# KogarashiNetwork/Kogarashi

Hardware: AMD Instinct MI355X
Metric: bn254_g1_msm_pairs_per_sec (higher is better)
Workload: dtype u32x9 (29-bit limbs)

## Files before the change

### kogarashi_amd/csrc/common.h

```cpp
#pragma once
#include <hip/hip_runtime.h>
#include <cstdint>
#include <atomic>
#include <future>
#include <cstdio>
#include <string>
#include <memory>
#include <map>
#include <unordered_map>
#include <vector>
#include <thread>
#include <new>
#include "../../include/kogarashi_amd.h"
#include "curve.h"
#include "tuning.h"
#include "worker_pool.h"

struct kg_tw_cache;

struct kg_ctx {
  int device = 0;
  hipStream_t own_stream = nullptr;
  hipStream_t stream = nullptr;
  std::string last_error;
  kg_tuning tune;
  int msm_window = 0;
  bool sort_alone = false;
  int msm_groups = 0;
  void* ws_sort[2] = {nullptr, nullptr};
  size_t ws_sort_bytes[2] = {0, 0};
  unsigned sort_seq = 0;
  bool queues_placed = false, sort_events = false;
  int placement = 0;
  hipStream_t sort_stream = nullptr;
  static constexpr int MAX_GROUPS = 4;
  hipEvent_t ev_sorted[2][MAX_GROUPS] = {};
  hipStream_t acc_stream[MAX_GROUPS] = {};
  void* ws_pb = nullptr;
  size_t ws_pb_bytes = 0;
  hipEvent_t ev_pb = nullptr;
  hipEvent_t ev_prep = nullptr;
  static constexpr int IDLE_EVS = 8;
  hipEvent_t ev_ws_idle[2][IDLE_EVS] = {};
  int ws_idle_n[2] = {0, 0};
  hipEvent_t ev_bases = nullptr;
  hipEvent_t ev_order = nullptr;
  unsigned small_glv_off = 0;
  bool inputs_complete = false;

  std::multimap<size_t, void*> pool_free;
  size_t pool_cached = 0;
  void* ws_vec = nullptr;
  size_t ws_vec_bytes = 0;
  void* ws2 = nullptr;
  size_t ws2_bytes = 0;
  void* ws3[2] = {nullptr, nullptr};
  size_t ws3_bytes[2] = {0, 0};
  static constexpr int RUN_SETS = 8;
  void* ws_run[RUN_SETS] = {};
  size_t ws_run_bytes[RUN_SETS] = {};
  hipStream_t side_stream = nullptr;
  hipStream_t side2_stream = nullptr;
  hipEvent_t ev_fork = nullptr, ev_join[3] = {nullptr, nullptr, nullptr};
  hipEvent_t ev_acc[RUN_SETS] = {};
  hipEvent_t ev_info[MAX_GROUPS] = {};
  struct Slot { void* host = nullptr; void* host_dev = nullptr; size_t bytes = 0; hipEvent_t done = nullptr; int W = 0, c = 0, w0 = 0; bool busy = false;
                bool combined = false; };
  static constexpr int NSLOTS = 24;
  Slot slots[NSLOTS];
  void* ws_small[NSLOTS] = {};
  size_t ws_small_bytes[NSLOTS] = {};
  std::unique_ptr<kg::WorkerPool> workers;
  std::shared_ptr<void> prover_jobs;
  size_t ticket_n[4] = {0, 0, 0, 0};
  std::future<int> ticket_fut[4];
  uint64_t ticket_out[4][24] = {};
  struct Registered { const uint64_t* base; const uint8_t* inf; size_t n; int curve; uint32_t* packed; uint32_t* table = nullptr; int table_c = 0, table_W = 0; bool fmt64 = false, table64 = false; };
  std::vector<Registered> registered;
  void* up_buf[3] = {nullptr, nullptr, nullptr};
  size_t up_bytes[3] = {0, 0, 0};
  hipStream_t up_stream = nullptr;
  static constexpr int UP_SLICES = 8;
  hipEvent_t ev_up_s[UP_SLICES] = {}, ev_up_b[UP_SLICES] = {};
  void* ws_points = nullptr;
  void* fb_tmp = nullptr;
  size_t fb_tmp_bytes = 0;
  uint32_t* fb_table[3] = {nullptr, nullptr, nullptr};
  void* h_pinned = nullptr;
  void* h_pinned_dev = nullptr;
  size_t h_pinned_bytes = 0;
  std::vector<kg_tw_cache*> tw;
  bool tw_fresh = false;
  bool prof = false;
  struct Phase { const char* name; hipEvent_t e0, e1; };
  std::vector<Phase> phases;
  std::vector<hipEvent_t> event_pool;
  size_t event_next = 0;
  std::atomic<long long> host_finish_us{0};
  std::atomic<int> host_finish_calls{0};
};

namespace kg {

inline WorkerPool& pool(kg_ctx* c) {
  if (!c->workers) c->workers.reset(new WorkerPool(c->tune.pool_max_threads));
  return *c->workers;
}
inline int set_err(kg_ctx* c, int code, const char* what, hipError_t e = hipSuccess) {
  if (c) {
    c->last_error = what;
    if (e != hipSuccess) { c->last_error += ": "; c->last_error += hipGetErrorString(e); }
  }
  if (e != hipSuccess) (void)hipGetLastError();
  return code;
}
template <class Fn>
inline int kg_guarded(kg_ctx* c, Fn&& fn) noexcept {
  try { return fn(); }
  catch (const std::bad_alloc&) { return set_err(c, KG_ERR_OOM, "host allocation failed"); }
  catch (...) { return set_err(c, KG_ERR_HIP, "host runtime failure (a worker thread could not be started?)"); }
}
struct JoinGuard {
  std::thread& t;
  ~JoinGuard() { if (t.joinable()) t.join(); }
};
#define KG_HIP(ctx, call)                                                        \
  do {                                                                           \
    hipError_t e__ = (call);                                                     \
    if (e__ != hipSuccess) return kg::set_err(ctx, e__ == hipErrorOutOfMemory ? KG_ERR_OOM : KG_ERR_HIP, #call, e__); \
  } while (0)
#define KG_TRY(call)            \
  do {                          \
    int s__ = (call);           \
    if (s__ != KG_OK) return s__; \
  } while (0)

hipError_t dev_alloc(kg_ctx* c, void** p, size_t bytes);
void pool_trim(kg_ctx* c);
int ensure_ws_sort(kg_ctx* c, int set, size_t bytes);
int make_sort_stream(kg_ctx* c);
hipError_t create_stream(kg_ctx* c, hipStream_t* out, bool service);
int ensure_ws2(kg_ctx* c, size_t bytes);
int ensure_ws_vec(kg_ctx* c, size_t bytes);
int ensure_ws3(kg_ctx* c, int which, size_t bytes);
int ensure_ws_run(kg_ctx* c, int which, size_t bytes);
int ensure_slot(kg_ctx* c, int slot, size_t bytes);
int ensure_pinned(kg_ctx* c, size_t bytes);
int make_side_stream(kg_ctx* c);
int slice_table_window(const kg_ctx* ctx, int curve, const uint64_t* d_bases, const uint8_t* d_inf, size_t cnt);
void sync_all(kg_ctx* c);

struct PhaseScope {
  kg_ctx* c; int idx = -1; hipStream_t s;
  PhaseScope(kg_ctx* ctx, const char* name, hipStream_t stream = nullptr);
  void end();
};
void prof_reset(kg_ctx* c);

#if defined(__HIP_DEVICE_COMPILE__)
#ifndef KG_PRIO_LEVEL
#define KG_PRIO_LEVEL 3
#endif
#define KG_SERVICE_PRIO() __builtin_amdgcn_s_setprio(KG_PRIO_LEVEL)
#ifndef KG_REDUCE_LEVEL
#define KG_REDUCE_LEVEL 1
#endif
#define KG_REDUCE_PRIO() __builtin_amdgcn_s_setprio(KG_REDUCE_LEVEL)
#else
#define KG_SERVICE_PRIO() ((void)0)
#define KG_REDUCE_PRIO() ((void)0)
#endif

struct alignas(16) Words8 { uint32_t w[8]; };

__device__ __forceinline__ void load_words(const uint64_t* base, size_t elem, uint32_t w[8]) {
  const uint4* p = reinterpret_cast<const uint4*>(base) + 2 * elem;
  uint4 a = p[0], b = p[1];
  w[0] = a.x; w[1] = a.y; w[2] = a.z; w[3] = a.w; w[4] = b.x; w[5] = b.y; w[6] = b.z; w[7] = b.w;
}
__device__ __forceinline__ void store_words(uint64_t* base, size_t elem, const uint32_t w[8]) {
  uint4* p = reinterpret_cast<uint4*>(base) + 2 * elem;
  p[0] = make_uint4(w[0], w[1], w[2], w[3]);
  p[1] = make_uint4(w[4], w[5], w[6], w[7]);
}

template <class F> struct RawIO;
template <class P> struct RawIO<Fp<P>> {
  static constexpr int NW = 9;
  static __device__ __forceinline__ Fp<P> load(const uint32_t* base, size_t stride, size_t i) {
    Fp<P> r;
#pragma unroll
    for (int k = 0; k < 9; ++k) r.l[k] = base[(size_t)k * stride + i];
    return r;
  }
  static __device__ __forceinline__ void store(uint32_t* base, size_t stride, size_t i, const Fp<P>& a) {
#pragma unroll
    for (int k = 0; k < 9; ++k) base[(size_t)k * stride + i] = a.l[k];
  }
};
template <class F> struct RawIO<Fp2<F>> {
  static constexpr int NW = 18;
  static __device__ __forceinline__ Fp2<F> load(const uint32_t* base, size_t stride, size_t i) {
    return {RawIO<F>::load(base, stride, i), RawIO<F>::load(base + 9 * stride, stride, i)};
  }
  static __device__ __forceinline__ void store(uint32_t* base, size_t stride, size_t i, const Fp2<F>& a) {
    RawIO<F>::store(base, stride, i, a.c0);
    RawIO<F>::store(base + 9 * stride, stride, i, a.c1);
  }
};
template <class F>
struct PointIO {
  static constexpr int NW = 4 * RawIO<F>::NW;
  static __device__ __forceinline__ XYZZ<F> load(const uint32_t* base, size_t stride, size_t i) {
    constexpr int E = RawIO<F>::NW;
    return {RawIO<F>::load(base, stride, i), RawIO<F>::load(base + (size_t)E * stride, stride, i),
            RawIO<F>::load(base + (size_t)2 * E * stride, stride, i), RawIO<F>::load(base + (size_t)3 * E * stride, stride, i)};
  }
  static __device__ __forceinline__ void store(uint32_t* base, size_t stride, size_t i, const XYZZ<F>& p) {
    constexpr int E = RawIO<F>::NW;
    RawIO<F>::store(base, stride, i, p.x);
    RawIO<F>::store(base + (size_t)E * stride, stride, i, p.y);
    RawIO<F>::store(base + (size_t)2 * E * stride, stride, i, p.zz);
    RawIO<F>::store(base + (size_t)3 * E * stride, stride, i, p.zzz);
  }
};

template <class F> struct RefIO;
template <class P> struct RefIO<Fp<P>> {
  static constexpr int W64 = 4;
  static __device__ __forceinline__ Fp<P> load(const uint64_t* p) {
    uint32_t w[8];
    load_words(p, 0, w);
    return from_ref<P>(w);
  }
};
template <class F> struct RefIO<Fp2<F>> {
  static constexpr int W64 = 8;
  static __device__ __forceinline__ Fp2<F> load(const uint64_t* p) { return {RefIO<F>::load(p), RefIO<F>::load(p + 4)}; }
};


struct MsmSorted {
  size_t n = 0;
  int c = 0, W = 0, B = 0;
  uint32_t T = 0, T2 = 16, T_top = 0, nhot = 0;
  int top_w = -1;
  uint32_t* hot_list = nullptr;
  size_t npts = 0, part_cap = 0;
  uint32_t ntasks = 0, max_cnt = 0;
  uint32_t *sorted = nullptr, *bsize = nullptr, *bstart = nullptr, *lcnt = nullptr, *lrel = nullptr, *lbase = nullptr;
  uint32_t *task_bkt = nullptr, *task_id = nullptr;
  int set = 0;
  hipEvent_t ready = nullptr;
  int w0 = 0, group = 0;
  hipStream_t acc_stream = nullptr;
  bool reduce_inline = false;
  bool tail_alone = false;
  hipStream_t sorted_on = nullptr;
  int merged_shift = 0, windows = 0;
};
int r1cs_prod_enqueue(kg_ctx* c, hipStream_t st, int field, const uint64_t* row_ptr, const uint64_t* col, const uint64_t* val, size_t m,
                      const uint64_t* z, uint64_t* out, uint32_t* scratch);
int ntt_prepare(kg_ctx* ctx, uint32_t log_n, int inverse);
int ntt_enqueue(kg_ctx* ctx, hipStream_t st, uint64_t* tmp, uint64_t* d_data, uint32_t log_n, int inverse, int coset);
struct NttTables;
int ntt_tables(kg_ctx* ctx, uint32_t log_n, int inverse, NttTables* out, const uint32_t** zinv);
int msm_sort(kg_ctx* ctx, int scalar_field, const uint64_t* d_scalars, size_t n, MsmSorted* S, bool ordered = false, int merged_c = 0, int lane_mult = 1,
             bool wait_info = true, int info_idx = 0);
int msm_sort_wait(kg_ctx* ctx, MsmSorted* S);
struct MsmSortPlan {
  size_t n = 0, chunk_len = 0, nv = 0;
  int c = 0, W = 0, B = 0, Wb = 0, G = 0, nch = 0, maxseg = 0, mshift = 0, set = 0, ngroups = 1, info_base = 0, fb = 7;
  bool alone = false;
  bool merged = false, two_pass = false;
  uint32_t T = 0, T_top = 0;
  int gw0[kg_ctx::MAX_GROUPS] = {}, gW[kg_ctx::MAX_GROUPS] = {};
  char* ws = nullptr;
  size_t o_kt = 0, o_cnt = 0, o_bsize = 0, o_bstart = 0, o_tmp = 0, o_gsize = 0, o_gstart = 0, o_segbase = 0, o_segcnt = 0, o_segoff = 0, o_sorted = 0,
         o_lcnt = 0, o_lrel = 0, o_rowtot = 0, o_bpart = 0, o_woff = 0, o_gsize_m = 0, o_gstart_m = 0, o_segbase_m = 0;
  size_t o_lbase[kg_ctx::MAX_GROUPS] = {}, o_misc[kg_ctx::MAX_GROUPS] = {}, o_lenh[kg_ctx::MAX_GROUPS] = {}, o_tbkt[kg_ctx::MAX_GROUPS] = {},
         o_tid[kg_ctx::MAX_GROUPS] = {}, o_hot[kg_ctx::MAX_GROUPS] = {}, part_cap[kg_ctx::MAX_GROUPS] = {};
};
int msm_sort_begin(kg_ctx* ctx, int scalar_field, const uint64_t* d_scalars, size_t n, MsmSortPlan* P, bool ordered, int merged_c, int lane_mult,
                   int ngroups = 1, const int* gw = nullptr, bool on_main = false);
int msm_sort_group(kg_ctx* ctx, const MsmSortPlan& P, int g, MsmSorted* S, bool on_main = false);
int msm_group_plan(const kg_ctx* ctx, size_t n, int* gw);
int merged_window(const kg_ctx* ctx, size_t n);
bool has_window_table(const kg_ctx* ctx, int curve, const uint64_t* d_bases, const uint8_t* d_inf, size_t nbases, size_t msm_len);
int scalar_queue(kg_ctx* ctx, hipStream_t* out);
struct MsmRunJob { const uint64_t* d_bases; const uint8_t* d_inf; size_t nbases; uint32_t idx_off; int slot; bool bases_complete = false;
                   const uint32_t* packed = nullptr; bool packed64 = false; };
int msm_run_multi(kg_ctx* ctx, const MsmSorted& S, int curve, const MsmRunJob* jobs, int njobs);
int msm_run(kg_ctx* ctx, const MsmSorted& S, int curve, const uint64_t* d_bases, const uint8_t* d_inf, size_t nbases, uint32_t idx_off, int slot);
int msm_finish(kg_ctx* ctx, int curve, int slot, uint64_t* out_xyz);
bool msm_small_plan(const kg_ctx* ctx, int curve, size_t n, int* c, int* r);
bool msm_small_glv(const kg_ctx* ctx, int curve, size_t n);
bool msm_small_kt(const kg_ctx* ctx, size_t n);
int msm_small_enqueue(kg_ctx* ctx, hipStream_t st, int curve, const uint64_t* d_bases, const uint8_t* d_inf, const uint64_t* d_scalars, size_t n, int slot,
                      int c, int r);
int msm_finish_groups(kg_ctx* ctx, int curve, const int* slots, int nslots, uint64_t* out_xyz);
void msm_identity(int curve, uint64_t* out_xyz);

}
```

### kogarashi_amd/csrc/msm_bases.h

```cpp
#pragma once
#include "msm_common.h"

namespace kg {
namespace msm {
namespace {

template <class F> struct FieldOf;
template <class Q> struct FieldOf<Fp<Q>> { using P = Q; };
template <class G> struct FieldOf<Fp2<G>> { using P = typename G::Params; };
template <class F> struct BaseIO;
template <class P> struct BaseIO<Fp<P>> {
  static constexpr int W = 8;
  static constexpr int PE = 9;
  static __device__ __forceinline__ void convert(const uint64_t* src, uint32_t* dst) {
    uint32_t w[8];
    load_words(src, 0, w);
    const Fp<P> v = from_ref<P>(w);
#pragma unroll
    for (int j = 0; j < 9; ++j) dst[j] = v.l[j];
  }
  static __device__ __forceinline__ Fp<P> from_words(const uint32_t* w) {
    Fp<P> r;
#pragma unroll
    for (int j = 0; j < 9; ++j) r.l[j] = w[j];
    return r;
  }
  static constexpr int PK = 8;
  static __device__ __forceinline__ void pack(const Fp<P>& v, uint32_t* dst) { words_from_limbs(v, dst); }
  static __device__ __forceinline__ bool load_point64(const uint32_t* src, Fp<P>& x, Fp<P>& y) {
    uint32_t w[16];
    const uint4* p = reinterpret_cast<const uint4*>(src);
#pragma unroll
    for (int j = 0; j < 4; ++j) { const uint4 v = p[j]; w[4 * j] = v.x; w[4 * j + 1] = v.y; w[4 * j + 2] = v.z; w[4 * j + 3] = v.w; }
    const bool inf = (w[7] & INF_BIT) != 0;
    w[7] &= ~INF_BIT;
    x = limbs_from_words<P>(w); y = limbs_from_words<P>(w + 8);
    return inf;
  }
  static __device__ __forceinline__ bool point64_from_words(uint32_t (&w)[16], Fp<P>& x, Fp<P>& y) {
    const bool inf = (w[7] & INF_BIT) != 0;
    w[7] &= ~INF_BIT;
    x = limbs_from_words<P>(w); y = limbs_from_words<P>(w + 8);
    return inf;
  }
  static __device__ __forceinline__ bool load_point(const uint32_t* src, Fp<P>& x, Fp<P>& y) {
    uint32_t w[18];
    const uint2* p = reinterpret_cast<const uint2*>(src);
#pragma unroll
    for (int j = 0; j < 9; ++j) { const uint2 v = p[j]; w[2 * j] = v.x; w[2 * j + 1] = v.y; }
    const bool inf = (w[8] & INF_BIT) != 0;
    w[8] &= ~INF_BIT;
    x = from_words(w); y = from_words(w + 9);
    return inf;
  }
};
template <class F> struct BaseIO<Fp2<F>> {
  static constexpr int W = 16;
  static constexpr int PE = 18;
  static __device__ __forceinline__ void convert(const uint64_t* src, uint32_t* dst) {
    BaseIO<F>::convert(src, dst);
    BaseIO<F>::convert(src + 4, dst + 9);
  }
  static constexpr int PK = 16;
  static __device__ __forceinline__ void pack(const Fp2<F>& v, uint32_t* dst) { BaseIO<F>::pack(v.c0, dst); BaseIO<F>::pack(v.c1, dst + 8); }
  static __device__ __forceinline__ bool load_point64(const uint32_t* src, Fp2<F>& x, Fp2<F>& y) {
    uint32_t w[32];
    const uint4* p = reinterpret_cast<const uint4*>(src);
#pragma unroll
    for (int j = 0; j < 8; ++j) { const uint4 v = p[j]; w[4 * j] = v.x; w[4 * j + 1] = v.y; w[4 * j + 2] = v.z; w[4 * j + 3] = v.w; }
    const bool inf = (w[7] & INF_BIT) != 0;
    w[7] &= ~INF_BIT;
    using P = typename F::Params;
    x = {limbs_from_words<P>(w), limbs_from_words<P>(w + 8)};
    y = {limbs_from_words<P>(w + 16), limbs_from_words<P>(w + 24)};
    return inf;
  }
  static __device__ __forceinline__ bool load_point(const uint32_t* src, Fp2<F>& x, Fp2<F>& y) {
    uint32_t w[36];
    const uint4* p = reinterpret_cast<const uint4*>(src);
#pragma unroll
    for (int j = 0; j < 9; ++j) { const uint4 v = p[j]; w[4 * j] = v.x; w[4 * j + 1] = v.y; w[4 * j + 2] = v.z; w[4 * j + 3] = v.w; }
    const bool inf = (w[8] & INF_BIT) != 0;
    w[8] &= ~INF_BIT;
    x = {BaseIO<F>::from_words(w), BaseIO<F>::from_words(w + 9)};
    y = {BaseIO<F>::from_words(w + 18), BaseIO<F>::from_words(w + 27)};
    return inf;
  }
};


}
}
template <class F> struct RawIO<Fp2S<F>> {
  static constexpr int NW = 18;
  static __device__ __forceinline__ Fp2S<F> load(const uint32_t* base, size_t stride, size_t i) {
    return {RawIO<F>::load(base + (size_t)(9 * Fp2S<F>::half()) * stride, stride, i)};
  }
  static __device__ __forceinline__ void store(uint32_t* base, size_t stride, size_t i, const Fp2S<F>& a) {
    RawIO<F>::store(base + (size_t)(9 * Fp2S<F>::half()) * stride, stride, i, a.v);
  }
};
namespace msm {
namespace {

template <class G> struct BaseIO<Fp2S<G>> {
  static constexpr int W = 16, PE = 18, PK = 16;
  using P = typename G::Params;
  static __device__ __forceinline__ bool load_point64(const uint32_t* src, Fp2S<G>& x, Fp2S<G>& y) {
    const int h = Fp2S<G>::half();
    const uint4* p = reinterpret_cast<const uint4*>(src);
    uint32_t w[16];
    const uint4 a0 = p[2 * h], a1 = p[2 * h + 1], b0 = p[4 + 2 * h], b1 = p[5 + 2 * h];
    w[0] = a0.x; w[1] = a0.y; w[2] = a0.z; w[3] = a0.w; w[4] = a1.x; w[5] = a1.y; w[6] = a1.z; w[7] = a1.w;
    w[8] = b0.x; w[9] = b0.y; w[10] = b0.z; w[11] = b0.w; w[12] = b1.x; w[13] = b1.y; w[14] = b1.z; w[15] = b1.w;
    int flag = (h == 0 && (w[7] & INF_BIT) != 0) ? 1 : 0;
    flag |= __shfl_xor(flag, 1);
    if (h == 0) w[7] &= ~INF_BIT;
    x.v = limbs_from_words<P>(w); y.v = limbs_from_words<P>(w + 8);
    return flag != 0;
  }
  static __device__ __forceinline__ bool load_point(const uint32_t* src, Fp2S<G>& x, Fp2S<G>& y) {
    const int h = Fp2S<G>::half();
    uint32_t wx[9], wy[9];
#pragma unroll
    for (int k = 0; k < 9; ++k) { wx[k] = src[9 * h + k]; wy[k] = src[18 + 9 * h + k]; }
    int flag = (h == 0 && (wx[8] & INF_BIT) != 0) ? 1 : 0;
    flag |= __shfl_xor(flag, 1);
    if (h == 0) wx[8] &= ~INF_BIT;
    x.v = BaseIO<G>::from_words(wx); y.v = BaseIO<G>::from_words(wy);
    return flag != 0;
  }
};

template <class F>
__device__ __forceinline__ void store_resident(uint32_t* out, size_t i, uint32_t* buf , int fmt64) {
  constexpr int PE = BaseIO<F>::PE, PK = BaseIO<F>::PK;
  if (fmt64) {
    const bool inf = (buf[8] & INF_BIT) != 0;
    buf[8] &= ~INF_BIT;
    uint32_t pk[2 * PK];
#pragma unroll
    for (int e = 0; e < PE / 9; ++e) {
      Fp<typename FieldOf<F>::P> vx, vy;
#pragma unroll
      for (int k = 0; k < 9; ++k) { vx.l[k] = buf[9 * e + k]; vy.l[k] = buf[PE + 9 * e + k]; }
      words_from_limbs(vx, pk + 8 * e);
      words_from_limbs(vy, pk + PK + 8 * e);
    }
    if (inf) pk[7] |= INF_BIT;
    uint4* dst = reinterpret_cast<uint4*>(out + i * 2 * PK);
#pragma unroll
    for (int j = 0; j < PK / 2; ++j) dst[j] = make_uint4(pk[4 * j], pk[4 * j + 1], pk[4 * j + 2], pk[4 * j + 3]);
    return;
  }
  uint2* dst = reinterpret_cast<uint2*>(out + i * 2 * PE);
#pragma unroll
  for (int j = 0; j < PE; ++j) dst[j] = make_uint2(buf[2 * j], buf[2 * j + 1]);
}
template <class F, bool P64>
__global__ void __launch_bounds__(256) k_prep_bases(const uint64_t* __restrict__ bases, const uint8_t* __restrict__ inf, size_t n,
                                                    uint32_t* __restrict__ out) {
  KG_SERVICE_PRIO();
  size_t i = (size_t)blockIdx.x * blockDim.x + threadIdx.x;
  if (i >= n) return;
  constexpr int W = BaseIO<F>::W, PE = BaseIO<F>::PE;
  uint32_t buf[2 * PE];
  BaseIO<F>::convert(bases + (size_t)i * W, buf);
  BaseIO<F>::convert(bases + (size_t)i * W + W / 2, buf + PE);
  if (inf && inf[i]) buf[8] |= INF_BIT;
  store_resident<F>(out, i, buf, P64 ? 1 : 0);
}

template <class F>
static void launch_prep_bases(hipStream_t st, const uint64_t* bases, const uint8_t* inf, size_t n, uint32_t* out, bool fmt64) {
  const dim3 grid((unsigned)((n + 255) / 256));
  if (fmt64) hipLaunchKernelGGL((k_prep_bases<F, true>), grid, dim3(256), 0, st, bases, inf, n, out);
  else hipLaunchKernelGGL((k_prep_bases<F, false>), grid, dim3(256), 0, st, bases, inf, n, out);
}

template <class P> __device__ __forceinline__ void put_limbs(const Fp<P>& a, uint32_t* w) {
#pragma unroll
  for (int j = 0; j < 9; ++j) w[j] = a.l[j];
}
template <class F> __device__ __forceinline__ void put_limbs(const Fp2<F>& a, uint32_t* w) { put_limbs(a.c0, w); put_limbs(a.c1, w + 9); }
template <class F>
__global__ void __launch_bounds__(64) k_table_next(const uint32_t* __restrict__ prev, size_t n, int c, uint32_t* __restrict__ next, int fmt64) {
  const size_t i = (size_t)blockIdx.x * blockDim.x + threadIdx.x;
  if (i >= n) return;
  constexpr int PE = BaseIO<F>::PE, PK = BaseIO<F>::PK;
  Affine<F> a;
  bool inf = fmt64 ? BaseIO<F>::load_point64(prev + i * 2 * PK, a.x, a.y) : BaseIO<F>::load_point(prev + i * 2 * PE, a.x, a.y);
  uint32_t buf[2 * PE];
#pragma unroll
  for (int j = 0; j < 2 * PE; ++j) buf[j] = 0;
  if (!inf) {
    XYZZ<F> p = double_affine(a);
    for (int k = 1; k < c; ++k) p = double_xyzz(p);
    Affine<F> o;
    inf = !to_affine(p, o);
    if (!inf) { put_limbs(reduce(o.x), buf); put_limbs(reduce(o.y), buf + PE); }
  }
  if (inf) buf[8] |= INF_BIT;
  store_resident<F>(next, i, buf, fmt64);
}


}
}
}
```

### kogarashi_amd/csrc/msm_digits.h

```cpp
#pragma once
#include <cstdint>
#include "fp29.h"
#include "glv_consts.h"

namespace kg {

KG_HD void small_bias(int c, int W, uint32_t H[8]) {
  for (int j = 0; j < 8; ++j) H[j] = 0;
  for (int w = 0; w < W - 1; ++w) {
    const int bit = w * c + c - 1;
    H[bit >> 5] |= 1u << (bit & 31);
  }
}

KG_HD uint32_t small_window_digit(const uint32_t kb[8], int w, int c, int W, bool& negative) {
  const int o = w * c;
  const int j = o >> 5, sh = o & 31;
  uint64_t v = kb[j];
  if (j + 1 < 8) v |= (uint64_t)kb[j + 1] << 32;
  const uint32_t e = (uint32_t)(v >> sh);
  if (w == W - 1) {
    negative = false;
    return e;
  }
  const int32_t d = (int32_t)(e & ((1u << c) - 1u)) - (int32_t)(1u << (c - 1));
  negative = d < 0;
  return (uint32_t)(d < 0 ? -d : d);
}

template <int NA, int NB, int LO, int NR>
KG_HD void glv_mul_words(const uint32_t* a, const uint32_t* b, uint32_t* r) {
  uint64_t carry = 0;
  uint64_t carry_hi = 0;
#pragma unroll
  for (int col = 0; col < LO + NR; ++col) {
    uint64_t lo = carry, hi = carry_hi;
#pragma unroll
    for (int i = 0; i < NA; ++i) {
      const int j = col - i;
      if (j < 0 || j >= NB) continue;
      const uint64_t pr = (uint64_t)a[i] * b[j];
      lo += pr & 0xffffffffu;
      hi += pr >> 32;
    }
    if (col >= LO) r[col - LO] = (uint32_t)lo;
    carry = (lo >> 32) + (hi & 0xffffffffu);
    carry_hi = hi >> 32;
  }
}
template <class L>
KG_HD void glv_decompose_with(const uint32_t k[8], uint32_t k1[4], bool& neg1, uint32_t k2[4], bool& neg2) {
  uint32_t c1[3], c2[5];
  {
    uint32_t t[6];
    glv_mul_words<8, 3, 7, 4>(k, L::G1, t);
    uint64_t cy = ((uint64_t)t[0] + 0x80000000u) >> 32;
#pragma unroll
    for (int i = 0; i < 3; ++i) { const uint64_t v = (uint64_t)t[1 + i] + cy; c1[i] = (uint32_t)v; cy = v >> 32; }
    glv_mul_words<8, 5, 7, 6>(k, L::G2, t);
    cy = ((uint64_t)t[0] + 0x80000000u) >> 32;
#pragma unroll
    for (int i = 0; i < 5; ++i) { const uint64_t v = (uint64_t)t[1 + i] + cy; c2[i] = (uint32_t)v; cy = v >> 32; }
  }
  uint32_t t1[5], t2[5], r1[5], r2[5];
  glv_mul_words<3, 5, 0, 5>(c1, L::A1, t1);
  glv_mul_words<5, 5, 0, 5>(c2, L::A2, t2);
  {
    int64_t br = 0;
#pragma unroll
    for (int i = 0; i < 5; ++i) {
      const int64_t d = (int64_t)k[i] - (int64_t)t1[i] - (int64_t)t2[i] + br;
      r1[i] = (uint32_t)d;
      br = d >> 32;
    }
  }
  glv_mul_words<3, 5, 0, 5>(c1, L::B1, t1);
  glv_mul_words<5, 5, 0, 5>(c2, L::B2, t2);
  {
    int64_t br = 0;
#pragma unroll
    for (int i = 0; i < 5; ++i) {
      const int64_t d = -(int64_t)t1[i] - (int64_t)t2[i] + br;
      r2[i] = (uint32_t)d;
      br = d >> 32;
    }
  }
  neg1 = (r1[4] >> 31) != 0;
  neg2 = (r2[4] >> 31) != 0;
  uint64_t cy1 = neg1 ? 1 : 0, cy2 = neg2 ? 1 : 0;
#pragma unroll
  for (int i = 0; i < 4; ++i) {
    const uint64_t s1 = (uint64_t)(neg1 ? ~r1[i] : r1[i]) + cy1;
    k1[i] = (uint32_t)s1; cy1 = s1 >> 32;
    const uint64_t s2 = (uint64_t)(neg2 ? ~r2[i] : r2[i]) + cy2;
    k2[i] = (uint32_t)s2; cy2 = s2 >> 32;
  }
}

}
```

### kogarashi_amd/csrc/msm_host.cpp

```cpp
#include "common.h"
#include "host_fp.h"
#include "msm_internal.h"
#include <algorithm>
#include <chrono>
#include <cstdlib>
#include <cstring>
#include <condition_variable>
#include <mutex>
#include <thread>

using namespace kg;

namespace {

struct G1Cfg { using HF = HostFq; static constexpr int E64 = 4; static constexpr int ID = KG_G1; };
struct GkCfg { using HF = HostFr; static constexpr int E64 = 4; static constexpr int ID = KG_GRUMPKIN; };
struct G2Cfg { using HF = HostFq2; static constexpr int E64 = 8; static constexpr int ID = KG_G2; };

template <class HF> struct HostIO;
template <class P> struct HostIO<HostFp<P>> {
  static HostFp<P> load(const uint64_t* w) { return HostFp<P>::from_words(w); }
  static void store(const HostFp<P>& a, uint64_t* w) { a.to_words(w); }
};
template <class F> struct HostIO<Fp2<F>> {
  static Fp2<F> load(const uint64_t* w) { return {HostIO<F>::load(w), HostIO<F>::load(w + 4)}; }
  static void store(const Fp2<F>& a, uint64_t* w) { HostIO<F>::store(a.c0, w); HostIO<F>::store(a.c1, w + 4); }
};

template <class Cfg>
XYZZ<typename Cfg::HF> host_load_point(const uint64_t* p) {
  using HF = typename Cfg::HF;
  constexpr int E = Cfg::E64;
  return {HostIO<HF>::load(p), HostIO<HF>::load(p + E), HostIO<HF>::load(p + 2 * E), HostIO<HF>::load(p + 3 * E)};
}

template <class Cfg>
void store_projective(const XYZZ<typename Cfg::HF>& p, uint64_t* out_xyz) {
  using HF = typename Cfg::HF;
  constexpr int E = Cfg::E64;
  Affine<HF> a;
  if (!to_affine(p, a)) {
    HostIO<HF>::store(HF::zero(), out_xyz);
    HostIO<HF>::store(HF::one(), out_xyz + E);
    HostIO<HF>::store(HF::zero(), out_xyz + 2 * E);
    return;
  }
  HostIO<HF>::store(a.x, out_xyz);
  HostIO<HF>::store(a.y, out_xyz + E);
  HostIO<HF>::store(HF::one(), out_xyz + 2 * E);
}

}

namespace kg {

template <class Cfg>
int msm_finish_t(kg_ctx* ctx, const int* slots, int nslots, uint64_t* out_xyz) {
  using HF = typename Cfg::HF;
  hipSetDevice(ctx->device);
  host_trace("finish: enter");
  constexpr int PE = 4 * Cfg::E64;
  XYZZ<HF> acc = XYZZ<HF>::identity();
  long long busy_us = 0;
  for (int s = 0; s < nslots; ++s) {
    kg_ctx::Slot& sl = ctx->slots[slots[s]];
    if (hipEventSynchronize(sl.done) != hipSuccess) return KG_ERR_HIP;
    host_trace("finish: slot ready");
    const auto t0 = std::chrono::steady_clock::now();
    const uint64_t* hp = (const uint64_t*)sl.host;
    const int W = sl.W, c = sl.c, w0 = sl.w0;
    if (sl.combined) {
      for (int w = W - 1; w >= 0; --w) {
        for (int l = 0; l < c; ++l) acc = double_xyzz(acc);
        acc = add_xyzz(acc, host_load_point<Cfg>(hp + (size_t)w * PE));
      }
    } else
    for (int bit = (w0 + W) * c - 1; bit >= w0 * c; --bit) {
      acc = double_xyzz(acc);
      const int w = bit / c - w0, l = bit % c;
      if (c > 1 && l < c - 1) acc = add_xyzz(acc, host_load_point<Cfg>(hp + ((size_t)w * c + 1 + l) * PE));
      if (l == 0) acc = add_xyzz(acc, host_load_point<Cfg>(hp + ((size_t)w * c) * PE));
    }
    if (s == nslots - 1) store_projective<Cfg>(acc, out_xyz);
    busy_us += std::chrono::duration_cast<std::chrono::microseconds>(std::chrono::steady_clock::now() - t0).count();
  }
  host_trace("finish: done");
  if (ctx->prof) {
    ctx->host_finish_us += busy_us;
    ctx->host_finish_calls += 1;
  }
  return KG_OK;
}

int msm_finish_groups(kg_ctx* ctx, int curve, const int* slots, int nslots, uint64_t* out_xyz) {
  if (nslots < 1) return KG_ERR_BAD_ARG;
  switch (curve) {
    case KG_G1: return msm_finish_t<G1Cfg>(ctx, slots, nslots, out_xyz);
    case KG_GRUMPKIN: return msm_finish_t<GkCfg>(ctx, slots, nslots, out_xyz);
    case KG_G2: return msm_finish_t<G2Cfg>(ctx, slots, nslots, out_xyz);
    default: return KG_ERR_BAD_ARG;
  }
}
int msm_finish(kg_ctx* ctx, int curve, int slot, uint64_t* out_xyz) { return msm_finish_groups(ctx, curve, &slot, 1, out_xyz); }
void msm_identity(int curve, uint64_t* out_xyz) {
  if (curve == KG_G2) store_projective<G2Cfg>(XYZZ<HostFq2>::identity(), out_xyz);
  else if (curve == KG_GRUMPKIN) store_projective<GkCfg>(XYZZ<HostFr>::identity(), out_xyz);
  else store_projective<G1Cfg>(XYZZ<HostFq>::identity(), out_xyz);
}

}

namespace {

template <class Cfg>
int sum_affine_impl(const uint64_t* pts, const uint8_t* inf, size_t count, uint64_t* out_xy, uint8_t* out_inf) {
  using HF = typename Cfg::HF;
  constexpr int E = Cfg::E64;
  XYZZ<HF> acc = XYZZ<HF>::identity();
  for (size_t i = 0; i < count; ++i) {
    if (inf && inf[i]) continue;
    Affine<HF> a{HostIO<HF>::load(pts + i * 2 * E), HostIO<HF>::load(pts + i * 2 * E + E)};
    acc = add_mixed(acc, a);
  }
  uint64_t xyz[3 * 8];
  store_projective<Cfg>(acc, xyz);
  std::memcpy(out_xy, xyz, 2 * E * 8);
  *out_inf = is_identity(acc) ? 1 : 0;
  return KG_OK;
}

}

extern "C" {

static int sum_slices(kg_ctx* ctx, int curve, const uint64_t (*part)[24], int K, uint64_t* out_xyz) {
  const int E = curve == KG_G2 ? 8 : 4;
  if (K == 1) { std::memcpy(out_xyz, part[0], (size_t)3 * E * 8); return KG_OK; }
  uint64_t pts[kg_ctx::UP_SLICES * 16];
  uint8_t pinf[kg_ctx::UP_SLICES];
  for (int j = 0; j < K; ++j) {
    bool z0 = true;
    for (int k = 0; k < E; ++k) z0 = z0 && part[j][2 * E + k] == 0;
    pinf[j] = z0 ? 1 : 0;
    std::memcpy(pts + (size_t)j * 2 * E, part[j], (size_t)2 * E * 8);
  }
  uint64_t xy[16];
  uint8_t inf = 0;
  KG_TRY(kg_points_sum_affine(ctx, curve, pts, pinf, (size_t)K, xy, &inf));
  kg::msm_identity(curve, out_xyz);
  if (!inf) {
    for (int k = 0; k < E; ++k) out_xyz[2 * E + k] = out_xyz[E + k];
    std::memcpy(out_xyz, xy, (size_t)2 * E * 8);
  }
  return KG_OK;
}

static int msm_sliced(kg_ctx* ctx, int curve, const uint64_t* d_bases, const uint8_t* d_inf, const uint64_t* d_scalars, size_t n, uint64_t* out_xyz) {
  constexpr int K = 4;
  const size_t pw = curve == KG_G2 ? 16 : 8;
  size_t lo[K + 1];
  for (int j = 0; j <= K; ++j) lo[j] = n / K * j + (j == K ? n % K : 0);
  const int saved_window = ctx->msm_window;
  struct Restore { kg_ctx* c; int w; ~Restore() { c->msm_window = w; } } restore_window{ctx, saved_window};
  if (!saved_window) { const int cw = pick_window(n, 0), cs = pick_window(n / K, 0); ctx->msm_window = cw > cs ? cw : cs; }
  uint64_t part[K][24];
  std::future<int> fin[K];
  kg::WaitAll fin_done{fin, K};
  int rc = KG_OK;
  const int sfield = curve == KG_GRUMPKIN ? KG_FQ : KG_FR;
  for (int j = 0; j < K && rc == KG_OK; ++j) {
    const size_t a = lo[j], cnt = lo[j + 1] - lo[j];
    kg::MsmSorted S;
    rc = kg::msm_sort(ctx, sfield, d_scalars + 4 * a, cnt, &S, j > 0);
    if (rc != KG_OK) break;
    rc = kg::msm_run(ctx, S, curve, d_bases + a * pw, d_inf ? d_inf + a : nullptr, cnt, 0, 16 + j);
    if (rc != KG_OK) break;
    uint64_t* out = part[j];
    fin[j] = kg::pool(ctx).submit([ctx, curve, j, out] { return kg::msm_finish(ctx, curve, 16 + j, out); });
  }
  ctx->msm_window = saved_window;
  for (int j = 0; j < K; ++j)
    if (fin[j].valid()) { const int r2 = fin[j].get(); if (rc == KG_OK) rc = r2; }
  if (rc != KG_OK) { kg_ctx_sync(ctx); return rc; }
  return sum_slices(ctx, curve, part, K, out_xyz);
}

static int msm_grouped(kg_ctx* ctx, int curve, const uint64_t* d_bases, const uint8_t* d_inf, const uint64_t* d_scalars, size_t n, const int* gw, int NG,
                       uint64_t* out_xyz) {
  KG_HIP(ctx, hipSetDevice(ctx->device));
  if (!ctx->side_stream) KG_TRY(make_side_stream(ctx));
  KG_TRY(make_sort_stream(ctx));
  for (int g = 1; g < NG && g < ctx->tune.group_accq; ++g)
    if (!ctx->acc_stream[g]) KG_HIP(ctx, create_stream(ctx, &ctx->acc_stream[g], false));
  kg::MsmSortPlan Q;
  const int main_first = ctx->tune.group_main_first;
  KG_TRY(kg::msm_sort_begin(ctx, curve == KG_GRUMPKIN ? KG_FQ : KG_FR, d_scalars, n, &Q, false, 0, 1, NG, gw, main_first != 0));
  if (main_first == 1) {
    KG_HIP(ctx, hipEventRecord(ctx->ev_prep, ctx->stream));
    KG_HIP(ctx, hipStreamWaitEvent(ctx->sort_stream, ctx->ev_prep, 0));
  }
  const size_t pw64 = curve == KG_G2 ? 16 : 8;
  bool resident = false;
  for (const auto& r : ctx->registered) {
    if (r.curve != curve || d_bases < r.base) continue;
    const size_t off64 = (size_t)(d_bases - r.base);
    if (off64 % pw64 != 0 || off64 / pw64 + n > r.n) continue;
    if (d_inf != (r.inf ? r.inf + off64 / pw64 : nullptr)) continue;
    resident = true;
    break;
  }
  const bool f64 = resident_fmt64(n);
  if (!resident) {
    const size_t bytes = n * (f64 ? (curve == KG_G2 ? 128 : 64) : (curve == KG_G2 ? 144 : 72));
    if (bytes > ctx->ws_pb_bytes) {
      if (ctx->ws_pb) { sync_all(ctx); hipFree(ctx->ws_pb); ctx->ws_pb = nullptr; ctx->ws_pb_bytes = 0; }
      const hipError_t e = dev_alloc(ctx, &ctx->ws_pb, bytes + bytes / 8);
      if (e != hipSuccess) return set_err(ctx, KG_ERR_OOM, "resident-bases allocation", e);
      ctx->ws_pb_bytes = bytes + bytes / 8;
    }
    hipStream_t cq = ctx->side_stream;
    if (!ctx->inputs_complete) {
      KG_HIP(ctx, hipEventRecord(ctx->ev_order, ctx->stream));
      KG_HIP(ctx, hipStreamWaitEvent(cq, ctx->ev_order, 0));
    }
    PhaseScope ph(ctx, "prep_bases", cq);
    prep_bases_enqueue(curve, cq, d_bases, d_inf, n, (uint32_t*)ctx->ws_pb, f64);
    ph.end();
    KG_HIP(ctx, hipGetLastError());
    KG_HIP(ctx, hipEventRecord(ctx->ev_pb, cq));
  }
  kg::MsmSorted S[kg_ctx::MAX_GROUPS];
  int slots[kg_ctx::MAX_GROUPS];
  int rc = kg::msm_sort_group(ctx, Q, 0, &S[0], main_first != 0);
  if (rc == KG_OK && main_first == 2) KG_HIP(ctx, hipStreamWaitEvent(ctx->sort_stream, S[0].ready, 0));
  if (rc == KG_OK && NG > 1) rc = kg::msm_sort_group(ctx, Q, 1, &S[1]);
  int launched = 0;
  for (int g = 0; g < NG && rc == KG_OK; ++g) {
    rc = kg::msm_sort_wait(ctx, &S[g]);
    if (rc != KG_OK) break;
    const int accq = ctx->tune.group_accq;
    S[g].acc_stream = (accq > 1 && g % accq) ? ctx->acc_stream[g % accq] : nullptr;
    const int rinl = ctx->tune.group_reduce_inline;
    S[g].reduce_inline = rinl && g == NG - 1;
    S[g].tail_alone = g == NG - 1;
    const int one_side = ctx->tune.group_one_side;
    slots[g] = one_side ? 16 + 2 * g : 16 + g;
    kg::MsmRunJob job{d_bases, d_inf, n, 0u, slots[g], false, resident ? nullptr : (const uint32_t*)ctx->ws_pb, f64};
    rc = kg::msm_run_multi(ctx, S[g], curve, &job, 1);
    if (rc != KG_OK) break;
    ++launched;
    if (g + 2 < NG) rc = kg::msm_sort_group(ctx, Q, g + 2, &S[g + 2]);
  }
  if (rc != KG_OK) { sync_all(ctx); return rc; }
  (void)launched;
  return kg::msm_finish_groups(ctx, curve, slots, NG, out_xyz);
}

static int msm_blocking(kg_ctx* ctx, int curve, const uint64_t* d_bases, const uint8_t* d_inf, const uint64_t* d_scalars, size_t n, uint64_t* out_xyz);

int kg_msm(kg_ctx* ctx, int curve, const uint64_t* d_bases, const uint8_t* d_inf, const uint64_t* d_scalars, size_t n, uint64_t* out_xyz) {
  return kg::kg_guarded(ctx, [&]() -> int {
  if (!ctx || !out_xyz || (n && (!d_bases || !d_scalars)) || curve < 0 || curve > KG_G2) return KG_ERR_BAD_ARG;
  if (n == 0) { kg::msm_identity(curve, out_xyz); return KG_OK; }
  return msm_blocking(ctx, curve, d_bases, d_inf, d_scalars, n, out_xyz);
  });
}

static int msm_blocking(kg_ctx* ctx, int curve, const uint64_t* d_bases, const uint8_t* d_inf, const uint64_t* d_scalars, size_t n, uint64_t* out_xyz) {
  int sc = 0, sr = 0;
  if (kg::msm_small_plan(ctx, curve, n, &sc, &sr)) {
    KG_TRY(kg::msm_small_enqueue(ctx, ctx->stream, curve, d_bases, d_inf, d_scalars, n, 0, sc, sr));
    return kg::msm_finish(ctx, curve, 0, out_xyz);
  }
  const bool sliced_ok = ctx->tune.msm_sliced != 0;
  if (n >= ((size_t)1 << 23) && sliced_ok && pick_window(n, ctx->msm_window) < 19) return msm_sliced(ctx, curve, d_bases, d_inf, d_scalars, n, out_xyz);
  kg::MsmSorted S;
  const bool tables_ok = n <= ((size_t)1 << ctx->tune.blocking_tables_log);
  const int mc = tables_ok && kg::has_window_table(ctx, curve, d_bases, d_inf, n, n) ? kg::merged_window(ctx, n) : 0;
  if (!mc) {
    int gw[kg_ctx::MAX_GROUPS];
    const int NG = kg::msm_group_plan(ctx, n, gw);
    if (NG > 1) return msm_grouped(ctx, curve, d_bases, d_inf, d_scalars, n, gw, NG, out_xyz);
  }
  ctx->sort_alone = true;
  const int rs = kg::msm_sort(ctx, curve == KG_GRUMPKIN ? KG_FQ : KG_FR, d_scalars, n, &S, false, mc);
  ctx->sort_alone = false;
  KG_TRY(rs);
  S.tail_alone = true;
  S.reduce_inline = ctx->tune.blocking_reduce_inline != 0;
  KG_TRY(kg::msm_run(ctx, S, curve, d_bases, d_inf, n, 0, 0));
  return kg::msm_finish(ctx, curve, 0, out_xyz);
}

int kg_msm_pick_window(size_t n) { return pick_window(n ? n : 1, 0); }
int kg_msm_table_window(size_t msm_len) { return kg::merged_window(nullptr, msm_len); }

int kg_bases_register(kg_ctx* ctx, int curve, const uint64_t* d_bases, const uint8_t* d_inf, size_t n) {
  return kg::kg_guarded(ctx, [&]() -> int {
  if (!ctx || curve < 0 || curve > KG_G2) return KG_ERR_BAD_ARG;
  if (n == 0) return KG_OK;
  if (!d_bases) return KG_ERR_BAD_ARG;
  KG_HIP(ctx, hipSetDevice(ctx->device));
  kg_bases_unregister(ctx, d_bases);
  const bool fmt64 = resident_fmt64(n);
  const size_t pw = fmt64 ? (curve == KG_G2 ? 32 : 16) : (curve == KG_G2 ? 36 : 18);
  uint32_t* packed = nullptr;
  KG_HIP(ctx, dev_alloc(ctx, (void**)&packed, n * pw * 4));
  prep_bases_enqueue(curve, ctx->stream, d_bases, d_inf, n, packed, fmt64);
  if (hipError_t e = hipGetLastError(); e != hipSuccess) {
    hipFree(packed);
    return set_err(ctx, KG_ERR_HIP, "k_prep_bases launch", e);
  }
  kg_ctx::Registered reg{d_bases, d_inf, n, curve, packed};
  reg.fmt64 = fmt64;
  ctx->registered.push_back(reg);
  return KG_OK;
  });
}

int kg_bases_unregister(kg_ctx* ctx, const uint64_t* d_bases) {
  return kg::kg_guarded(ctx, [&]() -> int {
  if (!ctx) return KG_ERR_BAD_ARG;
  for (size_t i = 0; i < ctx->registered.size(); ++i) {
    if (ctx->registered[i].base == d_bases) {
      kg_ctx_sync(ctx);
      hipFree(ctx->registered[i].packed);
      if (ctx->registered[i].table) hipFree(ctx->registered[i].table);
      ctx->registered.erase(ctx->registered.begin() + i);
      return KG_OK;
    }
  }
  return KG_OK;
  });
}

int kg_bases_precompute(kg_ctx* ctx, const uint64_t* d_bases, size_t msm_len) {
  return kg::kg_guarded(ctx, [&]() -> int {
  if (!ctx || !d_bases) return KG_ERR_BAD_ARG;
  KG_HIP(ctx, hipSetDevice(ctx->device));
  kg_ctx::Registered* r = nullptr;
  for (auto& e : ctx->registered) if (e.base == d_bases) r = &e;
  if (!r) return set_err(ctx, KG_ERR_BAD_ARG, "kg_bases_precompute: the array is not registered");
  if (msm_len == 0) msm_len = r->n;
  if (msm_len < r->n) return set_err(ctx, KG_ERR_BAD_ARG, "kg_bases_precompute: msm_len is shorter than the array");
  const int c = kg::merged_window(ctx, msm_len);
  if (!c) return set_err(ctx, KG_ERR_BAD_ARG, "kg_bases_precompute: window tables are offered for MSMs of 2^16 .. 2^20 scalars");
  if (r->table && r->table_c == c) return KG_OK;
  if (r->table) { kg_ctx_sync(ctx); hipFree(r->table); r->table = nullptr; r->table_c = r->table_W = 0; }
  const int W = (255 + c - 1) / c;
  const bool t64 = table_fmt64();
  const size_t pw = t64 ? (r->curve == KG_G2 ? 32 : 16) : (r->curve == KG_G2 ? 36 : 18), row = r->n * pw;
  uint32_t* table = nullptr;
  if (hipError_t e = dev_alloc(ctx, (void**)&table, (size_t)W * row * 4); e != hipSuccess) {
    (void)hipGetLastError();
    return set_err(ctx, KG_ERR_OOM, "window table allocation", e);
  }
  hipStream_t st = ctx->stream;
  prep_bases_enqueue(r->curve, st, r->base, r->inf, r->n, table, t64);
  hipError_t e = hipGetLastError();
  for (int w = 1; w < W && e == hipSuccess; ++w) {
    table_next_enqueue(r->curve, st, table + (size_t)(w - 1) * row, r->n, c, table + (size_t)w * row, t64);
    e = hipGetLastError();
  }
  if (e != hipSuccess) { hipFree(table); return set_err(ctx, KG_ERR_HIP, "window table build", e); }
  r->table = table; r->table_c = c; r->table_W = W; r->table64 = t64;
  return KG_OK;
  });
}

int kg_msm_begin(kg_ctx* ctx, int curve, const uint64_t* d_bases, const uint8_t* d_inf, const uint64_t* d_scalars, size_t n, int ticket) {
  return kg::kg_guarded(ctx, [&]() -> int {
  if (!ctx || (n && (!d_bases || !d_scalars)) || curve < 0 || curve > KG_G2 || ticket < 0 || ticket > 3) return KG_ERR_BAD_ARG;
  ctx->ticket_n[ticket] = n;
  if (n == 0) return KG_OK;
  int sc = 0, sr = 0;
  struct GlvGuard { kg_ctx* c; unsigned old; ~GlvGuard() { c->small_glv_off = old; } } glv_guard{ctx, ctx->small_glv_off};
  ctx->small_glv_off |= (1u << KG_G1) | (1u << KG_GRUMPKIN);
  if (n <= (size_t)(curve == KG_G2 ? ctx->tune.small_max_flight / 2 : ctx->tune.small_max_flight) && kg::msm_small_plan(ctx, curve, n, &sc, &sr)) {
    if (ctx->ticket_fut[ticket].valid()) ctx->ticket_fut[ticket].wait();
    KG_TRY(kg::msm_small_enqueue(ctx, ctx->stream, curve, d_bases, d_inf, d_scalars, n, 1 + ticket, sc, sr));
    uint64_t* out = ctx->ticket_out[ticket];
    ctx->ticket_fut[ticket] = kg::pool(ctx).submit([ctx, curve, ticket, out] { return kg::msm_finish(ctx, curve, 1 + ticket, out); });
    return KG_OK;
  }
  kg::MsmSorted S;
  const int mc = kg::has_window_table(ctx, curve, d_bases, d_inf, n, n) ? kg::merged_window(ctx, n) : 0;
  KG_TRY(kg::msm_sort(ctx, curve == KG_GRUMPKIN ? KG_FQ : KG_FR, d_scalars, n, &S, false, mc));
  const int pipe_accq = ctx->tune.pipe_accq;
  if (pipe_accq > 1 && (ticket & 1) && ctx->acc_stream[1]) S.acc_stream = ctx->acc_stream[1];
  if (ctx->ticket_fut[ticket].valid()) ctx->ticket_fut[ticket].wait();
  KG_TRY(kg::msm_run(ctx, S, curve, d_bases, d_inf, n, 0, 1 + ticket));
  uint64_t* out = ctx->ticket_out[ticket];
  ctx->ticket_fut[ticket] = kg::pool(ctx).submit([ctx, curve, ticket, out] { return kg::msm_finish(ctx, curve, 1 + ticket, out); });
  return KG_OK;
  });
}

int kg_msm_end(kg_ctx* ctx, int curve, int ticket, uint64_t* out_xyz) {
  return kg::kg_guarded(ctx, [&]() -> int {
  if (!ctx || !out_xyz || curve < 0 || curve > KG_G2 || ticket < 0 || ticket > 3) return KG_ERR_BAD_ARG;
  if (ctx->ticket_n[ticket] == 0) { kg::msm_identity(curve, out_xyz); return KG_OK; }
  if (!ctx->ticket_fut[ticket].valid()) return kg::set_err(ctx, KG_ERR_BAD_ARG, "kg_msm_end without a matching kg_msm_begin");
  const int rc = ctx->ticket_fut[ticket].get();
  if (rc != KG_OK) return rc;
  std::memcpy(out_xyz, ctx->ticket_out[ticket], (curve == KG_G2 ? 24 : 12) * 8);
  return KG_OK;
  });
}

static int grow_device(kg_ctx* ctx, int which, size_t bytes) {
  if (bytes <= ctx->up_bytes[which]) return KG_OK;
  if (ctx->up_buf[which]) { sync_all(ctx); hipFree(ctx->up_buf[which]); ctx->up_buf[which] = nullptr; ctx->up_bytes[which] = 0; }
  const hipError_t e = dev_alloc(ctx, &ctx->up_buf[which], bytes + bytes / 8);
  if (e != hipSuccess) { (void)hipGetLastError(); return set_err(ctx, KG_ERR_OOM, "upload buffer allocation", e); }
  ctx->up_bytes[which] = bytes + bytes / 8;
  return KG_OK;
}

static int msm_host_plan(const kg_tuning& tune, size_t n, bool scalars_only, size_t* lo) {
  int K = n >= ((size_t)1 << 20) ? 4 : (n >= ((size_t)1 << 18) ? 2 : 1);
  int first_div = 1;
  if (scalars_only) {
    int lg = 0;
    while (((size_t)1 << (lg + 1)) <= n) ++lg;
    K = lg >= 24 ? 8 : (lg == 23 ? 6 : (lg == 22 ? 4 : (lg == 21 ? 3 : (lg >= 19 ? 2 : 1))));
    first_div = K > 1 ? 2 : 1;
  }
  if (tune.host_slices >= 1 && tune.host_slices <= kg_ctx::UP_SLICES) K = tune.host_slices;
  if (tune.host_first_div >= 1 && tune.host_first_div <= 16) first_div = tune.host_first_div;
  if ((size_t)K > n) K = (int)n;
  if (K <= 1) { lo[0] = 0; lo[1] = n; return 1; }
  const size_t units = 1 + (size_t)(K - 1) * first_div;
  size_t first = n / units;
  if (first < 1) first = 1;
  first &= ~(size_t)255;
  if (first == 0) first = n / units ? n / units : 1;
  lo[0] = 0; lo[1] = first;
  const size_t rest = n - first;
  for (int j = 2; j <= K; ++j) lo[j] = first + rest / (K - 1) * (j - 1) + (j == K ? rest % (K - 1) : 0);
  return K;
}

static int msm_host_impl(kg_ctx* ctx, int curve, const uint64_t* bases, const uint8_t* inf, bool bases_on_device, const uint64_t* h_scalars, size_t n,
                         uint64_t* out_xyz) {
  KG_HIP(ctx, hipSetDevice(ctx->device));
  host_trace("host: enter");
  const size_t pb = curve == KG_G2 ? 128 : 64;
  if (!bases_on_device) {
    KG_TRY(grow_device(ctx, 0, n * pb));
    if (inf) KG_TRY(grow_device(ctx, 2, n));
  }
  KG_TRY(grow_device(ctx, 1, n * 32));
  if (!ctx->ev_up_s[0]) {
    KG_TRY(make_sort_stream(ctx));
    if (!ctx->up_stream) KG_HIP(ctx, hipStreamCreateWithFlags(&ctx->up_stream, hipStreamNonBlocking));
    for (int i = 0; i < kg_ctx::UP_SLICES; ++i) {
      KG_HIP(ctx, hipEventCreateWithFlags(&ctx->ev_up_s[i], hipEventDisableTiming));
      KG_HIP(ctx, hipEventCreateWithFlags(&ctx->ev_up_b[i], hipEventDisableTiming));
    }
  }
  hipStream_t sq;
  KG_TRY(kg::scalar_queue(ctx, &sq));
  if (bases_on_device && !ctx->inputs_complete) {
    KG_HIP(ctx, hipEventRecord(ctx->ev_order, ctx->stream));
    KG_HIP(ctx, hipStreamWaitEvent(sq, ctx->ev_order, 0));
  }
  const char* d_b = bases_on_device ? (const char*)bases : (const char*)ctx->up_buf[0];
  uint64_t* d_s = (uint64_t*)ctx->up_buf[1];
  const uint8_t* d_i = bases_on_device ? inf : (inf ? (const uint8_t*)ctx->up_buf[2] : nullptr);
  int sc = 0, sr = 0;
  if (kg::msm_small_plan(ctx, curve, n, &sc, &sr)) {
    KG_HIP(ctx, hipMemcpyAsync(d_s, h_scalars, n * 32, hipMemcpyHostToDevice, ctx->stream));
    if (!bases_on_device) {
      KG_HIP(ctx, hipMemcpyAsync(ctx->up_buf[0], bases, n * pb, hipMemcpyHostToDevice, ctx->stream));
      if (inf) KG_HIP(ctx, hipMemcpyAsync(ctx->up_buf[2], inf, n, hipMemcpyHostToDevice, ctx->stream));
    }
    KG_TRY(kg::msm_small_enqueue(ctx, ctx->stream, curve, (const uint64_t*)d_b, d_i, d_s, n, 0, sc, sr));
    return kg::msm_finish(ctx, curve, 0, out_xyz);
  }
  size_t lo[kg_ctx::UP_SLICES + 1];
  const int K = msm_host_plan(ctx->tune, n, bases_on_device, lo);
  std::atomic<int> up_s{0}, up_b{0}, up_rc{(int)hipSuccess};
  std::mutex up_mu;
  std::condition_variable up_cv;
  auto upload_scalars = [&](int j) {
    const size_t a = lo[j], cnt = lo[j + 1] - lo[j];
    hipError_t e = hipMemcpyAsync(d_s + 4 * a, h_scalars + 4 * a, cnt * 32, hipMemcpyHostToDevice, ctx->up_stream);
    if (e == hipSuccess) e = hipEventRecord(ctx->ev_up_s[j], ctx->up_stream);
    if (e != hipSuccess) up_rc = (int)e;
    { std::lock_guard<std::mutex> lk(up_mu); up_s = j + 1; }
    up_cv.notify_all();
    host_trace("upload: scalars");
  };
  auto upload_bases = [&](int j) {
    if (!bases_on_device) {
      const size_t a = lo[j], cnt = lo[j + 1] - lo[j];
      hipError_t e = hipMemcpyAsync((char*)ctx->up_buf[0] + a * pb, (const char*)bases + a * pb, cnt * pb, hipMemcpyHostToDevice, ctx->up_stream);
      if (e == hipSuccess && inf) e = hipMemcpyAsync((uint8_t*)ctx->up_buf[2] + a, inf + a, cnt, hipMemcpyHostToDevice, ctx->up_stream);
      if (e == hipSuccess) e = hipEventRecord(ctx->ev_up_b[j], ctx->up_stream);
      if (e != hipSuccess) up_rc = (int)e;
      host_trace("upload: bases");
    }
    { std::lock_guard<std::mutex> lk(up_mu); up_b = j + 1; }
    up_cv.notify_all();
  };
  upload_scalars(0);
  if (K == 1 && bases_on_device) {
    if (up_rc != (int)hipSuccess) return set_err(ctx, KG_ERR_HIP, "host-to-device upload", (hipError_t)up_rc.load());
    KG_HIP(ctx, hipStreamWaitEvent(ctx->stream, ctx->ev_up_s[0], 0));
    KG_HIP(ctx, hipStreamWaitEvent(sq, ctx->ev_up_s[0], 0));
    return msm_blocking(ctx, curve, bases, inf, d_s, n, out_xyz);
  }
  if (K > 1 && !ctx->acc_stream[1]) { if (create_stream(ctx, &ctx->acc_stream[1], false) != hipSuccess) return set_err(ctx, KG_ERR_HIP, "queue creation"); }
  std::future<int> uploader = kg::pool(ctx).submit([&]() -> int {
    hipSetDevice(ctx->device);
    upload_bases(0);
    for (int j = 1; j < K; ++j) { upload_scalars(j); upload_bases(j); }
    return KG_OK;
  });
  struct WaitGuard { std::future<int>& f; ~WaitGuard() { if (f.valid()) f.wait(); } } uploader_done{uploader};
  uint64_t part[kg_ctx::UP_SLICES][24];
  std::future<int> fin[kg_ctx::UP_SLICES];
  kg::WaitAll fin_done{fin, kg_ctx::UP_SLICES};
  int rc = KG_OK;
  const int sfield = curve == KG_GRUMPKIN ? KG_FQ : KG_FR;
  const bool was_alone = ctx->sort_alone;
  for (int j = 0; j < K && rc == KG_OK; ++j) {
    const size_t a = lo[j], cnt = lo[j + 1] - lo[j];
    { std::unique_lock<std::mutex> lk(up_mu); up_cv.wait(lk, [&] { return up_s.load() > j; }); }
    if (up_rc != (int)hipSuccess) { rc = set_err(ctx, KG_ERR_HIP, "host-to-device upload", (hipError_t)up_rc.load()); break; }
    if (hipStreamWaitEvent(sq, ctx->ev_up_s[j], 0) != hipSuccess) { rc = KG_ERR_HIP; break; }
    kg::MsmSorted S;
    ctx->sort_alone = j == 0;
    const int mc = (bases_on_device && ctx->tune.host_slice_tables) ? kg::slice_table_window(ctx, curve, (const uint64_t*)(d_b + a * pb), d_i ? d_i + a : nullptr, cnt) : 0;
    rc = kg::msm_sort(ctx, sfield, d_s + 4 * a, cnt, &S, true, mc);
    ctx->sort_alone = was_alone;
    if (rc != KG_OK) break;
    if (bases_on_device) {
      if (ctx->tune.host_accq > 1 && (j & 1)) S.acc_stream = ctx->acc_stream[1];
      S.reduce_inline = ctx->tune.group_reduce_inline && K > 1 && j == K - 1;
      S.tail_alone = j == K - 1;
    }
    if (!bases_on_device) {
      { std::unique_lock<std::mutex> lk(up_mu); up_cv.wait(lk, [&] { return up_b.load() > j; }); }
      if (up_rc != (int)hipSuccess) { rc = set_err(ctx, KG_ERR_HIP, "host-to-device upload", (hipError_t)up_rc.load()); break; }
      if (hipStreamWaitEvent(sq, ctx->ev_up_b[j], 0) != hipSuccess) { rc = KG_ERR_HIP; break; }
    }
    const kg::MsmRunJob job{(const uint64_t*)(d_b + a * pb), d_i ? d_i + a : nullptr, cnt, 0u, 16 + j, true};
    rc = kg::msm_run_multi(ctx, S, curve, &job, 1);
    if (rc != KG_OK) break;
    uint64_t* out = part[j];
    fin[j] = kg::pool(ctx).submit([ctx, curve, j, out] { return kg::msm_finish(ctx, curve, 16 + j, out); });
  }
  if (uploader.valid()) uploader.wait();
  hipStreamSynchronize(ctx->up_stream);
  host_trace("host: uploads synced");
  for (int j = 0; j < K; ++j)
    if (fin[j].valid()) { const int r2 = fin[j].get(); if (rc == KG_OK) rc = r2; }
  if (rc != KG_OK) { kg_ctx_sync(ctx); return rc; }
  return sum_slices(ctx, curve, part, K, out_xyz);
}

int kg_msm_host_slices(size_t n, int scalars_only, size_t* lo) {
  if (!lo) return KG_ERR_BAD_ARG;
  if (n == 0) { lo[0] = 0; return 0; }
  return msm_host_plan(tuning(), n, scalars_only != 0, lo);
}

int kg_msm_host(kg_ctx* ctx, int curve, const uint64_t* h_bases, const uint8_t* h_inf, const uint64_t* h_scalars, size_t n, uint64_t* out_xyz) {
  return kg::kg_guarded(ctx, [&]() -> int {
  if (!ctx || !out_xyz || (n && (!h_bases || !h_scalars)) || curve < 0 || curve > KG_G2) return KG_ERR_BAD_ARG;
  if (n == 0) return kg_msm(ctx, curve, nullptr, nullptr, nullptr, 0, out_xyz);
  return msm_host_impl(ctx, curve, h_bases, h_inf, false, h_scalars, n, out_xyz);
  });
}

int kg_msm_host_scalars(kg_ctx* ctx, int curve, const uint64_t* d_bases, const uint8_t* d_inf, const uint64_t* h_scalars, size_t n, uint64_t* out_xyz) {
  return kg::kg_guarded(ctx, [&]() -> int {
  if (!ctx || !out_xyz || (n && (!d_bases || !h_scalars)) || curve < 0 || curve > KG_G2) return KG_ERR_BAD_ARG;
  if (n == 0) return kg_msm(ctx, curve, nullptr, nullptr, nullptr, 0, out_xyz);
  return msm_host_impl(ctx, curve, d_bases, d_inf, true, h_scalars, n, out_xyz);
  });
}

static void xyz_to_commit(int curve, const uint64_t* xyz, uint64_t* out_xy, uint8_t* out_inf) {
  const int E = curve == KG_G2 ? 8 : 4;
  std::memcpy(out_xy, xyz, 2 * E * 8);
  bool z0 = true;
  for (int i = 0; i < E; ++i) z0 = z0 && xyz[2 * E + i] == 0;
  *out_inf = z0 ? 1 : 0;
}

int kg_commit_host_scalars(kg_ctx* ctx, int curve, const uint64_t* d_bases, const uint8_t* d_inf, const uint64_t* h_scalars, size_t n,
                           uint64_t* out_xy, uint8_t* out_inf) {
  return kg::kg_guarded(ctx, [&]() -> int {
  if (!ctx || !out_xy || !out_inf || curve < 0 || curve > KG_G2) return KG_ERR_BAD_ARG;
  uint64_t xyz[24];
  KG_TRY(kg_msm_host_scalars(ctx, curve, d_bases, d_inf, h_scalars, n, xyz));
  xyz_to_commit(curve, xyz, out_xy, out_inf);
  return KG_OK;
  });
}

int kg_commit(kg_ctx* ctx, int curve, const uint64_t* d_bases, const uint8_t* d_inf, const uint64_t* d_scalars, size_t n,
              uint64_t* out_xy, uint8_t* out_inf) {
  return kg::kg_guarded(ctx, [&]() -> int {
  if (!ctx || !out_xy || !out_inf || curve < 0 || curve > KG_G2) return KG_ERR_BAD_ARG;
  uint64_t xyz[24];
  KG_TRY(kg_msm(ctx, curve, d_bases, d_inf, d_scalars, n, xyz));
  xyz_to_commit(curve, xyz, out_xy, out_inf);
  return KG_OK;
  });
}

int kg_points_sum_affine(kg_ctx* ctx, int curve, const uint64_t* pts, const uint8_t* inf, size_t count, uint64_t* out_xy, uint8_t* out_inf) {
  (void)ctx;
  if (!out_xy || !out_inf || (count && !pts)) return KG_ERR_BAD_ARG;
  switch (curve) {
    case KG_G1: return sum_affine_impl<G1Cfg>(pts, inf, count, out_xy, out_inf);
    case KG_GRUMPKIN: return sum_affine_impl<GkCfg>(pts, inf, count, out_xy, out_inf);
    case KG_G2: return sum_affine_impl<G2Cfg>(pts, inf, count, out_xy, out_inf);
    default: return KG_ERR_BAD_ARG;
  }
}

}
```

### kogarashi_amd/csrc/msm_internal.h

```cpp
#pragma once
#include "common.h"

namespace kg {

int pick_window(size_t n, int forced);
bool resident_fmt64(size_t n);
bool table_fmt64();
void prep_bases_enqueue(int curve, hipStream_t st, const uint64_t* d_bases, const uint8_t* d_inf, size_t n, uint32_t* out, bool fmt64);
void table_next_enqueue(int curve, hipStream_t st, const uint32_t* prev, size_t n, int c, uint32_t* next, bool fmt64);
void host_trace(const char* what);

}
```

### kogarashi_amd/csrc/msm_run.hip

```cpp
#include "msm_reduce_kernels.h"
#include <cstdlib>
#include <cstring>

using namespace kg;
using namespace kg::msm;

namespace kg {
void prep_bases_enqueue(int curve, hipStream_t st, const uint64_t* d_bases, const uint8_t* d_inf, size_t n, uint32_t* out, bool fmt64) {
  if (curve == KG_G1) launch_prep_bases<Fq>(st, d_bases, d_inf, n, out, fmt64);
  else if (curve == KG_GRUMPKIN) launch_prep_bases<Fr>(st, d_bases, d_inf, n, out, fmt64);
  else launch_prep_bases<Fq2>(st, d_bases, d_inf, n, out, fmt64);
}
void table_next_enqueue(int curve, hipStream_t st, const uint32_t* prev, size_t n, int c, uint32_t* next, bool fmt64) {
  const dim3 grid((unsigned)((n + 63) / 64));
  if (curve == KG_G1) hipLaunchKernelGGL(k_table_next<Fq>, grid, dim3(64), 0, st, prev, n, c, next, fmt64 ? 1 : 0);
  else if (curve == KG_GRUMPKIN) hipLaunchKernelGGL(k_table_next<Fr>, grid, dim3(64), 0, st, prev, n, c, next, fmt64 ? 1 : 0);
  else hipLaunchKernelGGL(k_table_next<Fq2>, grid, dim3(64), 0, st, prev, n, c, next, fmt64 ? 1 : 0);
}
}

namespace kg {

struct RunJob { const uint64_t* d_bases; const uint8_t* d_inf; size_t nbases; uint32_t idx_off; int slot; bool bases_complete; const uint32_t* packed; bool packed64; };

template <class Cfg>
int msm_run_multi_t(kg_ctx* ctx, const MsmSorted& S, const RunJob* jobs, int njobs) {
  using F = typename Cfg::F;
  using KF = typename Cfg::KF;
  constexpr unsigned LPT = Lanes<KF>::N;
  constexpr int PW = 2 * BaseIO<F>::PE;
  constexpr int NW = PointIO<F>::NW;
  if (njobs < 1 || njobs > MAX_FUSED) return set_err(ctx, KG_ERR_BAD_ARG, "bad number of fused base arrays");
  const int W = S.W, B = S.B, c = S.c;
  const size_t npts = S.npts, part_cap = S.part_cap, nexp = (size_t)W * c;
  const size_t exp_bytes = nexp * 4 * Cfg::E64 * 8;
  hipStream_t st = S.acc_stream ? S.acc_stream : ctx->stream, sq;
  KG_TRY(scalar_queue(ctx, &sq));
  bool ordered_bases = false, converted = false, shared_pb = false;
  if (!ctx->side_stream) KG_TRY(make_side_stream(ctx));
  if (st != ctx->stream && !ctx->inputs_complete) {
    KG_HIP(ctx, hipEventRecord(ctx->ev_order, ctx->stream));
    KG_HIP(ctx, hipStreamWaitEvent(st, ctx->ev_order, 0));
  }
  struct Lay { size_t o_pb, o_lc[2], o_lr[2], o_lb[2], o_part[2], o_pbuf[2], o_rowtot, o_misc, o_hot; char* ws; const uint32_t* pb; int set; };
  Lay lay[MAX_FUSED];
  AccSets A;
  A.nsets = njobs;
  for (int k = 0; k < MAX_FUSED; ++k) { A.pb[k] = nullptr; A.idx_off[k] = 0; A.partial[k] = nullptr; A.tab_n[k] = 0; A.fmt64[k] = 0; }
  for (int k = 0; k < njobs; ++k) {
    const RunJob& J = jobs[k];
    Lay& Y = lay[k];
    Carver cv;
    const uint32_t* reg_pb = nullptr;
    if (J.packed) {
      if (S.merged_shift) return set_err(ctx, KG_ERR_BAD_ARG, "merged sort against caller-converted bases");
      reg_pb = J.packed; A.fmt64[k] = J.packed64 ? 1 : 0; shared_pb = true;
    }
    for (const auto& r : ctx->registered) {
      if (reg_pb) break;
      if (r.curve != Cfg::ID || J.d_bases < r.base) continue;
      const size_t off64 = (size_t)(J.d_bases - r.base);
      if (off64 % (size_t)BaseIO<F>::W != 0 || off64 / BaseIO<F>::W + J.nbases > r.n) continue;
      const size_t off = off64 / BaseIO<F>::W;
      if (J.d_inf != (r.inf ? r.inf + off : nullptr)) continue;
      if (S.merged_shift) {
        if (!r.table || r.table_c != c || r.table_W != S.windows) continue;
        reg_pb = r.table + off * (r.table64 ? 2 * BaseIO<F>::PK : PW);
        A.tab_n[k] = (uint32_t)r.n;
        A.fmt64[k] = r.table64 ? 1 : 0;
      } else {
        reg_pb = r.packed + off * (r.fmt64 ? 2 * BaseIO<F>::PK : PW);
        A.fmt64[k] = r.fmt64 ? 1 : 0;
      }
      break;
    }
    if (S.merged_shift && !reg_pb) return set_err(ctx, KG_ERR_BAD_ARG, "merged sort against bases without a matching window table");
    const bool conv64 = !reg_pb && resident_fmt64(J.nbases);
    if (conv64) A.fmt64[k] = 1;
    Y.o_pb = cv.take(reg_pb ? 256 : J.nbases * (conv64 ? 2 * BaseIO<F>::PK : PW) * 4);
    for (int i = 0; i < 2; ++i) {
      Y.o_lc[i] = cv.take(npts * 4); Y.o_lr[i] = cv.take(npts * 4); Y.o_lb[i] = cv.take((size_t)(W + 1) * 4);
      Y.o_part[i] = cv.take(part_cap * NW * 4); Y.o_pbuf[i] = cv.take(npts * NW * 4);
    }
    Y.o_rowtot = cv.take((size_t)W * 4); Y.o_misc = cv.take(64);
    Y.o_hot = cv.take(S.nhot ? (size_t)(S.nhot < HOT_MAX ? S.nhot : HOT_MAX) * hot_split<KF>(S.max_cnt) * NW * 4 : 0);
    Y.set = J.slot % kg_ctx::RUN_SETS;
    for (int k2 = 0; k2 < k; ++k2)
      if (lay[k2].set == Y.set) return set_err(ctx, KG_ERR_BAD_ARG, "fused MSMs need result slots in different run-space sets");
    KG_TRY(ensure_ws_run(ctx, Y.set, cv.off));
    KG_TRY(ensure_slot(ctx, J.slot, exp_bytes));
    if (!ctx->ev_acc[Y.set]) KG_HIP(ctx, hipEventCreateWithFlags(&ctx->ev_acc[Y.set], hipEventDisableTiming));
    Y.ws = (char*)ctx->ws_run[Y.set];
    Y.pb = reg_pb ? reg_pb : (uint32_t*)(Y.ws + Y.o_pb);
    for (int s2 = 0; s2 < kg_ctx::NSLOTS; ++s2)
      if (s2 % kg_ctx::RUN_SETS == Y.set && ctx->slots[s2].done && ctx->slots[s2].busy) {
        KG_HIP(ctx, hipStreamWaitEvent(st, ctx->slots[s2].done, 0));
        if (!reg_pb) KG_HIP(ctx, hipStreamWaitEvent(sq, ctx->slots[s2].done, 0));
        ctx->slots[s2].busy = false;
      }
    if (!reg_pb) {
      if (!ctx->inputs_complete && !ordered_bases && !J.bases_complete) {
        KG_HIP(ctx, hipEventRecord(ctx->ev_order, st));
        KG_HIP(ctx, hipStreamWaitEvent(sq, ctx->ev_order, 0));
        ordered_bases = true;
      }
      PhaseScope ph(ctx, "prep_bases", sq);
      launch_prep_bases<F>(sq, J.d_bases, J.d_inf, J.nbases, (uint32_t*)(Y.ws + Y.o_pb), conv64);
      ph.end();
      converted = true;
    }
    A.pb[k] = Y.pb; A.idx_off[k] = J.idx_off; A.partial[k] = (uint32_t*)(Y.ws + Y.o_part[0]);
  }
  const Level L0{S.lcnt, S.lrel, S.lbase};
  if (converted) {
    KG_HIP(ctx, hipEventRecord(ctx->ev_bases, sq));
    KG_HIP(ctx, hipStreamWaitEvent(st, ctx->ev_bases, 0));
  } else if (S.ready && S.sorted_on != st) KG_HIP(ctx, hipStreamWaitEvent(st, S.ready, 0));
  if (shared_pb) KG_HIP(ctx, hipStreamWaitEvent(st, ctx->ev_pb, 0));
  if (S.ntasks) {
    PhaseScope ph(ctx, "accumulate", st);
#ifdef KG_EXPERIMENTS
    if (LPT > 1 && ctx->tune.g2_pair_acc)
      hipLaunchKernelGGL(k_acc_tasks<KF>, dim3((unsigned)(((size_t)S.ntasks * LPT + 63) / 64) * (unsigned)njobs), dim3(64), 0, st, A, S.sorted, S.bstart, S.bsize, L0,
                         S.task_bkt, S.task_id, S.n, W, B, S.T, part_cap, S.merged_shift, S.T_top, S.top_w);
    else if (acc_prefetch<F>(A, njobs, jobs[0].nbases))
      hipLaunchKernelGGL(k_acc_tasks_q<typename PfField<F>::T>, dim3(((S.ntasks + 63) / 64) * (unsigned)njobs), dim3(64), 0, st, A, S.sorted, S.bstart, S.bsize, L0, S.task_bkt,
                         S.task_id, S.n, W, B, S.T, part_cap, S.merged_shift, S.T_top, S.top_w);
    else
#endif
    hipLaunchKernelGGL(k_acc_tasks<F>, dim3(((S.ntasks + 63) / 64) * (unsigned)njobs), dim3(64), 0, st, A, S.sorted, S.bstart, S.bsize, L0, S.task_bkt, S.task_id,
                       S.n, W, B, S.T, part_cap, S.merged_shift, S.T_top, S.top_w);
    ph.end();
  }
  for (int k = 0; k < njobs; ++k) {
    const RunJob& J = jobs[k];
    const Lay& Y = lay[k];
    const int slot = J.slot, set = Y.set;
    char* ws = Y.ws;
    const size_t* o_lc = Y.o_lc; const size_t* o_lr = Y.o_lr; const size_t* o_lb = Y.o_lb;
    uint32_t* part[2] = {(uint32_t*)(ws + Y.o_part[0]), (uint32_t*)(ws + Y.o_part[1])};
    uint32_t* pbuf[2] = {(uint32_t*)(ws + Y.o_pbuf[0]), (uint32_t*)(ws + Y.o_pbuf[1])};
    uint32_t* rowtot = (uint32_t*)(ws + Y.o_rowtot);
    uint32_t* misc = (uint32_t*)(ws + Y.o_misc);
    kg_ctx::Slot& sl = ctx->slots[slot];
    hipStream_t side = S.reduce_inline ? st : ((slot & 1) ? ctx->side2_stream : ctx->side_stream);
    if (side != st) {
      KG_HIP(ctx, hipEventRecord(ctx->ev_acc[set], st));
      KG_HIP(ctx, hipStreamWaitEvent(side, ctx->ev_acc[set], 0));
    }
    Level L = L0;
    int pcur = 0;
    bool fused_first = false;
    {
      PhaseScope ph(ctx, "partial_sums", side);
      uint32_t max_cnt = S.max_cnt;
      int lv = -1;
      const unsigned g1024 = (unsigned)((npts + 1023) / 1024);
      const bool hot_ok = ctx->tune.hot_sum != 0;
      if (max_cnt > GATHER_SUM_MAX && hot_ok && S.nhot >= 1 && S.nhot <= HOT_MAX && (size_t)part_cap * NW * 4 < ((size_t)1 << 32)) {
        PhaseScope ph2(ctx, "hot_sum", side);
        uint32_t* hot_scratch = (uint32_t*)(ws + Y.o_hot);
        const uint32_t split = hot_split<KF>(S.max_cnt);
        hipLaunchKernelGGL(k_hot_sum<KF>, dim3(S.nhot, split), dim3(256), 36 * 256 * 4, side, part[pcur], L, B, S.hot_list, hot_scratch, split);
        hipLaunchKernelGGL(k_hot_fold<KF>, dim3(S.nhot), dim3(256), 36 * 256 * 4, side, part[pcur], L, B, S.hot_list, hot_scratch, split);
        ph2.end();
        max_cnt = GATHER_SUM_MAX;
      }
      while (max_cnt > GATHER_SUM_MAX) {
        const int nx = lv < 0 ? 0 : (lv ^ 1);
        PhaseScope pr(ctx, "partial_round", side);
        uint32_t* ncnt = (uint32_t*)(ws + o_lc[nx]);
        uint32_t* nrel = (uint32_t*)(ws + o_lr[nx]);
        uint32_t* nbase = (uint32_t*)(ws + o_lb[nx]);
        KG_HIP(ctx, hipMemsetAsync(misc, 0, 64, side));
        hipLaunchKernelGGL(k_task_count, dim3(g1024), dim3(1024), 0, side, L.cnt, npts, S.T2, ncnt, misc + 8);
        hipLaunchKernelGGL(k_scan_rows, dim3(W), dim3(1024), 0, side, ncnt, B, nrel, rowtot);
        hipLaunchKernelGGL(k_row_bases, dim3(1), dim3(64), 0, side, rowtot, W, nbase, (const uint32_t*)nullptr, misc + 4);
        Level Lout{ncnt, nrel, nbase};
        const uint32_t bound = lv < 0 ? S.ntasks : (uint32_t)part_cap;
        hipLaunchKernelGGL(k_sum_tasks<KF>, dim3((unsigned)(((size_t)bound * LPT + 63) / 64)), dim3(64), 0, side, part[pcur], L, Lout, W, B, S.T2, part[pcur ^ 1]);
        pr.end();
        pcur ^= 1;
        L = Lout;
        lv = nx;
        max_cnt = (max_cnt + S.T2 - 1) / S.T2;
      }
      ph.end();
      PhaseScope pg(ctx, "gather", side);
      const bool fuse_ok = ctx->tune.gather_fuse != 0;
      fused_first = fuse_ok && max_cnt <= 1 && (uint32_t)B > (uint32_t)TailCfg<KF>::L && (size_t)part_cap * NW * 4 < ((size_t)1 << 32);
      if (max_cnt > 1)
        hipLaunchKernelGGL((k_gather_sum<F, KF>), dim3((unsigned)((npts * LPT + 63) / 64)), dim3(64), 0, side, part[pcur], L, W, B, pbuf[0]);
      else if (fused_first)
        hipLaunchKernelGGL(k_gather_halve<KF>, dim3((unsigned)((npts / 2 * LPT + 63) / 64)), dim3(64), 0, side, part[pcur], L, W, B, pbuf[0], (size_t)W * 2 * (B / 2));
      else
        hipLaunchKernelGGL(k_gather_buckets<F>, dim3((unsigned)((npts + 255) / 256)), dim3(256), 0, side, part[pcur], part_cap, L, W, B, pbuf[0]);
      pg.end();
    }
    if (ctx->ws_idle_n[S.set] < kg_ctx::IDLE_EVS) {
      KG_HIP(ctx, hipEventRecord(ctx->ev_ws_idle[S.set][ctx->ws_idle_n[S.set]], side));
      ctx->ws_idle_n[S.set] += 1;
    } else KG_HIP(ctx, hipStreamSynchronize(side));
    int cur = 0;
    {
      PhaseScope ph(ctx, "reduce", side);
      size_t in_stride = npts;
      int narr = 1;
      uint32_t len = (uint32_t)B;
      if (fused_first) { narr = 2; len = (uint32_t)B / 2; in_stride = (size_t)W * 2 * len; }
      constexpr uint32_t TL = (uint32_t)TailCfg<KF>::L;
      for (; len > TL; len /= 2) {
        const uint32_t n_out = len / 2;
        const size_t tasks = (size_t)W * narr * n_out;
        const size_t out_stride = (size_t)W * (narr + 1) * n_out;
        hipLaunchKernelGGL(k_halve<KF>, dim3((unsigned)((tasks * LPT + 63) / 64)), dim3(64), 0, side, pbuf[cur], in_stride, pbuf[cur ^ 1], out_stride,
                           W, narr, n_out);
        cur ^= 1;
        in_stride = out_stride;
        ++narr;
      }
      const size_t tail_lds = tail_lds_bytes(len, (int)LPT);
      const unsigned tail_threads = (unsigned)(len / 2 * LPT) < 64u ? 64u : (unsigned)(len / 2 * LPT);
      if (S.tail_alone && ctx->tune.coop_tail && len >= 2) {
        const size_t lds = tail_coop_lds_bytes<F>(len);
        static std::atomic<uint64_t> attr_devs{0};
        const uint64_t bit = (uint64_t)1 << (ctx->device & 63);
        if (!(attr_devs.load() & bit)) { KG_HIP(ctx, hipFuncSetAttribute((const void*)(k_reduce_tail_coop<F, Cfg::E64>), hipFuncAttributeMaxDynamicSharedMemorySize, 160 * 1024)); attr_devs |= bit; }
        hipLaunchKernelGGL((k_reduce_tail_coop<F, Cfg::E64>), dim3((unsigned)(W * narr)), dim3(TailCoopNT<F>::NT), lds, side, pbuf[cur], in_stride, narr, len, c, (uint64_t*)sl.host_dev);
      } else
      if (len == TL) {
        KG_HIP(ctx, hipFuncSetAttribute((const void*)(k_reduce_tail<KF, Cfg::E64, (int)TL>), hipFuncAttributeMaxDynamicSharedMemorySize, (int)tail_lds));
        hipLaunchKernelGGL((k_reduce_tail<KF, Cfg::E64, (int)TL>), dim3((unsigned)(W * narr)), dim3(tail_threads), tail_lds, side, pbuf[cur], in_stride, narr, len, c, (uint64_t*)sl.host_dev);
      } else {
        if (len > TL / 2) return set_err(ctx, KG_ERR_UNSUPPORTED, "reduction tail: array length");
        const size_t lds0 = tail_lds_bytes(TL / 2, (int)LPT);
        KG_HIP(ctx, hipFuncSetAttribute((const void*)(k_reduce_tail<KF, Cfg::E64, 0>), hipFuncAttributeMaxDynamicSharedMemorySize, (int)lds0));
        hipLaunchKernelGGL((k_reduce_tail<KF, Cfg::E64, 0>), dim3((unsigned)(W * narr)), dim3(tail_threads), lds0, side, pbuf[cur], in_stride, narr, len, c, (uint64_t*)sl.host_dev);
      }
      ph.end();
    }
    KG_HIP(ctx, hipGetLastError());
    KG_HIP(ctx, hipEventRecord(sl.done, side));
    sl.W = W; sl.c = c; sl.w0 = S.w0; sl.busy = true; sl.combined = false;
  }
  host_trace("run: enqueued");
  return KG_OK;
}

bool has_window_table(const kg_ctx* ctx, int curve, const uint64_t* d_bases, const uint8_t* d_inf, size_t nbases, size_t msm_len) {
  const int c = merged_window(ctx, msm_len);
  if (!c) return false;
  for (const auto& r : ctx->registered)
    if (r.base == d_bases && r.curve == curve && r.n == nbases && r.inf == d_inf && r.table && r.table_c == c) return true;
  return false;
}

int slice_table_window(const kg_ctx* ctx, int curve, const uint64_t* d_bases, const uint8_t* d_inf, size_t cnt) {
  const size_t pw64 = curve == KG_G2 ? 16 : 8;
  if (cnt < ((size_t)1 << 16)) return 0;
  int s = 0;
// ... 37 lines not shown
```

### kogarashi_amd/csrc/msm_sort.hip

```cpp
#include "msm_sort_kernels.h"
#include "msm_task_kernels.h"
#include <chrono>
#include <cstdlib>
#include <cstring>

using namespace kg;
using namespace kg::msm;

namespace kg {
void host_trace(const char* what) {
  if (!tuning().trace_host) return;
  static const auto t0 = std::chrono::steady_clock::now();
  fprintf(stderr, "[host] %-18s %10.1f us\n", what, std::chrono::duration<double, std::micro>(std::chrono::steady_clock::now() - t0).count());
}

int pick_window(size_t n, int forced) {
  const int wide_from = tuning().wide_window;
  if (forced) return forced;
  int lg = 0;
  while (((size_t)1 << (lg + 1)) <= n) ++lg;
  if (wide_from > 0 && lg >= wide_from && n <= ((size_t)1 << 24)) return 20;
  if (lg >= 21 && n <= ((size_t)1 << 24)) return 17;
  if (lg >= 19) return 16;
  if (lg >= 10) return 15;
  return lg >= 7 ? 8 : 5;
}

bool resident_fmt64(size_t n) { return n >= ((size_t)1 << tuning().fmt64_min_log); }
bool table_fmt64() { return tuning().table64 != 0; }
}

namespace kg {

int merged_window(const kg_ctx* ctx, size_t n) {
  if (n < ((size_t)1 << 16) || n > ((size_t)1 << 20)) return 0;
  int c = n >= ((size_t)1 << 17) ? 17 : 16;
  if (ctx && ctx->msm_window >= 15 && ctx->msm_window <= 18) c = ctx->msm_window;
  int s = 0;
  while (((size_t)1 << s) < n) ++s;
  const int W = (255 + c - 1) / c;
  if (((size_t)W << s) > ((size_t)1 << 24)) return 0;
  return c;
}

int msm_group_plan(const kg_ctx* ctx, size_t n, int* gw) {
  if (n < ((size_t)1 << 16) || n > ((size_t)1 << 24)) return 0;
  const int c = pick_window(n, ctx ? ctx->msm_window : 0);
  if (c - 1 < FINE_BITS + 4) return 0;
  const int W = (255 + c - 1) / c;
  int NG = n >= ((size_t)1 << 22) ? 3 : (n >= ((size_t)1 << 17) ? 2 : 0);
  if (c >= 19) NG = 4;
  if (ctx && ctx->msm_groups) NG = ctx->msm_groups;
  const kg_tuning& tn = ctx ? ctx->tune : tuning();
  if (!tn.msm_groups_list.empty() || tn.msm_groups >= 0) {
    if (!tn.msm_groups_list.empty()) {
      int k = 0, sum = 0;
      const char* p = tn.msm_groups_list.c_str();
      while (*p && k < kg_ctx::MAX_GROUPS) {
        const int v = atoi(p);
        if (v < 1) return 0;
        gw[k++] = v; sum += v;
        while (*p && *p != ',') ++p;
        if (*p == ',') ++p;
      }
      if (sum == W && !*p) return k;
    } else NG = tn.msm_groups;
  }
  if (NG > kg_ctx::MAX_GROUPS) NG = kg_ctx::MAX_GROUPS;
  if (NG > W) NG = W;
  if (NG < 2) return 0;
  for (int g = 0; g < NG; ++g) gw[g] = W / NG + (c >= 19 ? (g >= NG - W % NG ? 1 : 0) : (g < W % NG ? 1 : 0));
  return NG;
}

int msm_sort_begin(kg_ctx* ctx, int scalar_field, const uint64_t* d_scalars, size_t n, MsmSortPlan* P, bool ordered, int merged_c, int lane_mult,
                   int ngroups, const int* gw, bool on_main) {
  if (n == 0 || n >= ((size_t)1 << 31)) return set_err(ctx, KG_ERR_BAD_ARG, "msm length must be in [1, 2^31)");
  host_trace("sort: enter");
  KG_HIP(ctx, hipSetDevice(ctx->device));
  const bool merged = merged_c != 0;
  int c = merged ? merged_c : pick_window(n, ctx->msm_window);
  if (!merged && c > 16 && !(n >= ((size_t)1 << 16) && n <= ((size_t)1 << 24))) c = 16;
  const int W = (255 + c - 1) / c;
  const int B = 1 << (c - 1);
  int mshift = 0;
  if (merged) {
    while (((size_t)1 << mshift) < n) ++mshift;
    if (c < 15 || c > 18 || n < ((size_t)1 << 16) || ((size_t)W << mshift) > ((size_t)1 << 24))
      return set_err(ctx, KG_ERR_BAD_ARG, "merged sort not offered for this length / window");
  }
  const int Wb = merged ? 1 : W;
  const size_t nv = merged ? (size_t)W * n : n;
  int nch = (int)((n + 16383) / 16384);
  const int nch_cap = ctx->tune.sort_nch >= 1 && ctx->tune.sort_nch <= 1024 ? ctx->tune.sort_nch : 64;
  if (nch > nch_cap) nch = nch_cap;
  if (nch < 1) nch = 1;
  size_t chunk_len = (n + nch - 1) / nch;
  uint32_t T = (uint32_t)(2 * (n / B) + 16);
  if (ctx->tune.msm_t >= 4 && ctx->tune.msm_t <= 4096) T = (uint32_t)ctx->tune.msm_t;
  if (T < 32) T = 32;
  if (T > 2048) T = 2048;
  if (merged) {
    const size_t lanes = (size_t)(lane_mult < 1 ? 1 : lane_mult);
    size_t t = nv * lanes / ((size_t)4096 * 64);
    T = 16;
    while (T < 128 && 2 * (size_t)T <= t) T *= 2;
    if (ctx->tune.merged_t >= 4 && ctx->tune.merged_t <= 4096) T = (uint32_t)ctx->tune.merged_t;
  }
  const bool two_pass = merged || (c - 1 >= FINE_BITS + 4 && n >= ((size_t)1 << 16) && n <= ((size_t)1 << 24));
  const bool alone_ok = ctx->tune.sort_alone != 0;
  const bool alone = alone_ok && (ctx->sort_alone || ngroups > 1);
  if (c >= 19 && (!two_pass || merged)) return set_err(ctx, KG_ERR_BAD_ARG, "windows of 19 and 20 bits need the two-pass sort (2^16 .. 2^24 scalars)");
  const int fb = fine_bits_for(c);
  const uint32_t FINE = 1u << fb;
  const int G = two_pass ? B >> fb : 0;
  const uint32_t seg = seg_len_for(fb);
  const int maxseg = two_pass ? G + (int)((nv + seg - 1) / seg) : 0;
  if (two_pass) chunk_len = (chunk_len + PREP_CH - 1) / PREP_CH * PREP_CH;
  if (ngroups < 1 || ngroups > kg_ctx::MAX_GROUPS) return set_err(ctx, KG_ERR_BAD_ARG, "bad number of window groups");
  if (ngroups > 1 && (!two_pass || merged || !gw)) return set_err(ctx, KG_ERR_BAD_ARG, "window groups need the two-pass, unmerged sort");
  MsmSortPlan& Q = *P;
  Q = MsmSortPlan();
  {
    int top = Wb, sum = 0;
    for (int g = 0; g < ngroups; ++g) {
      const int wg = ngroups == 1 ? Wb : gw[g];
      if (wg < 1) return set_err(ctx, KG_ERR_BAD_ARG, "empty window group");
      top -= wg; sum += wg;
      Q.gw0[g] = top; Q.gW[g] = wg;
    }
    if (sum != Wb) return set_err(ctx, KG_ERR_BAD_ARG, "window groups do not add up to the window count");
  }
  Carver cv;
  Q.o_kt = cv.take(n * 32); Q.o_cnt = cv.take((size_t)W * nch * (two_pass ? G : B) * 4); Q.o_bsize = cv.take((size_t)W * B * 4);
  Q.o_bstart = cv.take((size_t)Wb * B * 4);
  Q.o_tmp = cv.take(two_pass ? (size_t)W * n * (fb == 9 ? 8 : 4) : 0); Q.o_gsize = cv.take((size_t)W * G * 4); Q.o_gstart = cv.take((size_t)W * G * 4);
  Q.o_segbase = cv.take((size_t)W * (G + 1) * 4); Q.o_segcnt = cv.take((size_t)Wb * maxseg * FINE * 4); Q.o_segoff = cv.take((size_t)Wb * maxseg * FINE * 4);
  Q.o_sorted = cv.take((size_t)W * n * 4); Q.o_lcnt = cv.take((size_t)Wb * B * 4); Q.o_lrel = cv.take((size_t)Wb * B * 4);
  Q.o_rowtot = cv.take((size_t)W * 4);
  Q.o_woff = cv.take(merged ? (size_t)W * G * 4 : 0); Q.o_gsize_m = cv.take(merged ? (size_t)G * 4 : 0); Q.o_gstart_m = cv.take(merged ? (size_t)G * 4 : 0);
  Q.o_segbase_m = cv.take(merged ? (size_t)(G + 1) * 4 : 0);
  Q.o_bpart = cv.take((size_t)W * (B / 4096 + 32) * 2 * 4);
  for (int g = 0; g < ngroups; ++g) {
    Q.part_cap[g] = (size_t)Q.gW[g] * (4 * ((nv + T - 1) / T)) + (size_t)Q.gW[g] * B;
    Q.o_lbase[g] = cv.take((size_t)(Q.gW[g] + 1) * 4);
    Q.o_misc[g] = cv.take(64); Q.o_lenh[g] = cv.take(2 * LEN_BINS * 4);
    Q.o_tbkt[g] = cv.take(Q.part_cap[g] * 4); Q.o_tid[g] = cv.take(Q.part_cap[g] * 4);
    Q.o_hot[g] = cv.take((size_t)HOT_MAX * 4);
  }
  const int set = (int)(ctx->sort_seq++ & 1u);
  KG_TRY(ensure_ws_sort(ctx, set, cv.off));
  KG_TRY(ensure_pinned(ctx, 4096));
  KG_TRY(make_sort_stream(ctx));
  char* ws = (char*)ctx->ws_sort[set];
  hipStream_t st = on_main ? ctx->stream : ctx->sort_stream;
  if (!on_main && !ordered && !ctx->inputs_complete) {
    KG_HIP(ctx, hipEventRecord(ctx->ev_order, ctx->stream));
    KG_HIP(ctx, hipStreamWaitEvent(st, ctx->ev_order, 0));
  }
  for (int j = 0; j < ctx->ws_idle_n[set]; ++j) KG_HIP(ctx, hipStreamWaitEvent(st, ctx->ev_ws_idle[set][j], 0));
  ctx->ws_idle_n[set] = 0;
  Q.n = n; Q.chunk_len = chunk_len; Q.nv = nv; Q.c = c; Q.W = W; Q.B = B; Q.Wb = Wb; Q.G = G; Q.nch = nch; Q.maxseg = maxseg; Q.mshift = mshift;
  Q.set = set; Q.ngroups = ngroups; Q.merged = merged; Q.two_pass = two_pass; Q.T = T; Q.ws = ws;
  Q.alone = alone;
  Q.T_top = merged ? T : 2 * T;
  Q.fb = fb;
  uint32_t* kt = (uint32_t*)(ws + Q.o_kt);
  uint32_t* cnt = (uint32_t*)(ws + Q.o_cnt);

  Words8 H;
  for (int j = 0; j < 8; ++j) H.w[j] = 0;
  for (int w = 0; w < W - 1; ++w) {
    int bit = w * c + c - 1;
    H.w[bit >> 5] |= 1u << (bit & 31);
  }
  {
    PhaseScope ph(ctx, "prep_scalars", st);
    if (two_pass) {
      const size_t hl = (size_t)W * G * 4;
      zero_fill(st, cnt, (size_t)W * nch * G * 4);
      const int per_wg = (alone && n < ((size_t)1 << 22) && fb == FINE_BITS) ? PREP_CH / 4 : PREP_CH;
      const dim3 grid((unsigned)((n + per_wg - 1) / per_wg));
      if (scalar_field == KG_FR) {
        if (hl > 48 * 1024) KG_HIP(ctx, hipFuncSetAttribute((const void*)k_prep_scalars_count<FrParams>, hipFuncAttributeMaxDynamicSharedMemorySize, (int)hl));
        hipLaunchKernelGGL(k_prep_scalars_count<FrParams>, grid, dim3(PREP_NT), hl, st, d_scalars, n, H, kt, c, W, fb, G, nch, chunk_len, cnt, per_wg);
      } else {
        if (hl > 48 * 1024) KG_HIP(ctx, hipFuncSetAttribute((const void*)k_prep_scalars_count<FqParams>, hipFuncAttributeMaxDynamicSharedMemorySize, (int)hl));
        hipLaunchKernelGGL(k_prep_scalars_count<FqParams>, grid, dim3(PREP_NT), hl, st, d_scalars, n, H, kt, c, W, fb, G, nch, chunk_len, cnt, per_wg);
      }
    } else if (scalar_field == KG_FR) hipLaunchKernelGGL(k_prep_scalars<FrParams>, dim3((unsigned)((n + 255) / 256)), dim3(256), 0, st, d_scalars, n, H, kt);
    else hipLaunchKernelGGL(k_prep_scalars<FqParams>, dim3((unsigned)((n + 255) / 256)), dim3(256), 0, st, d_scalars, n, H, kt);
    ph.end();
  }
  KG_HIP(ctx, hipGetLastError());
  return KG_OK;
}

int msm_sort_group(kg_ctx* ctx, const MsmSortPlan& Q, int g, MsmSorted* S, bool on_main) {
  if (g < 0 || g >= Q.ngroups) return set_err(ctx, KG_ERR_BAD_ARG, "bad window group");
  KG_HIP(ctx, hipSetDevice(ctx->device));
  const size_t n = Q.n, nv = Q.nv;
  const int c = Q.c, W = Q.W, B = Q.B, G = Q.G, nch = Q.nch, maxseg = Q.maxseg;
  const bool merged = Q.merged, two_pass = Q.two_pass;
  const int w0 = Q.gw0[g], Wg = Q.gW[g];
  const int sw0 = merged ? 0 : w0, sWg = merged ? W : Wg;
  const int hot_shift_env = ctx->tune.hot_shift;
  const uint32_t hot_shift = hot_shift_env >= 0 && hot_shift_env <= 2 ? (uint32_t)hot_shift_env : (Q.merged ? 0u : 2u);
  const uint32_t T = Q.T | (hot_shift << 30);
  char* ws = Q.ws;
  hipStream_t st = on_main ? ctx->stream : ctx->sort_stream;
  const size_t npts = (size_t)Wg * B;
  uint32_t* kt = (uint32_t*)(ws + Q.o_kt);
  uint32_t* cnt = (uint32_t*)(ws + Q.o_cnt);
  uint32_t* rowtot = (uint32_t*)(ws + Q.o_rowtot) + w0;
  uint32_t* misc = (uint32_t*)(ws + Q.o_misc[g]);
  uint32_t* lenh = (uint32_t*)(ws + Q.o_lenh[g]);
  S->set = Q.set; S->ready = ctx->ev_sorted[Q.set][g];
  S->n = n; S->c = c; S->W = Wg; S->B = B; S->T = T; S->npts = npts; S->part_cap = Q.part_cap[g];
  const int gi = Q.info_base + g;
  if (gi >= kg_ctx::MAX_GROUPS) return set_err(ctx, KG_ERR_BAD_ARG, "bad read-back index");
  S->merged_shift = Q.mshift; S->windows = W; S->w0 = w0; S->group = gi; S->acc_stream = nullptr; S->sorted_on = st;
  S->sorted = (uint32_t*)(ws + Q.o_sorted) + (size_t)w0 * n; S->bsize = (uint32_t*)(ws + Q.o_bsize) + (size_t)w0 * B;
  S->bstart = (uint32_t*)(ws + Q.o_bstart) + (size_t)w0 * B;
  S->lcnt = (uint32_t*)(ws + Q.o_lcnt) + (size_t)w0 * B; S->lrel = (uint32_t*)(ws + Q.o_lrel) + (size_t)w0 * B; S->lbase = (uint32_t*)(ws + Q.o_lbase[g]);
  S->task_bkt = (uint32_t*)(ws + Q.o_tbkt[g]); S->task_id = (uint32_t*)(ws + Q.o_tid[g]);
  S->hot_list = (uint32_t*)(ws + Q.o_hot[g]);
  S->T_top = Q.T_top | (hot_shift << 30);
  S->top_w = (!merged && w0 + Wg == W) ? Wg - 1 : -1;
  const uint32_t T_top = S->T_top;
  const int top_w = S->top_w;
  {
    PhaseScope ph(ctx, "sort", st);
    const size_t lds = (size_t)(two_pass ? G : B) * 4;
    if (lds > 48 * 1024) {
      KG_HIP(ctx, hipFuncSetAttribute((const void*)k_count, hipFuncAttributeMaxDynamicSharedMemorySize, (int)lds));
      KG_HIP(ctx, hipFuncSetAttribute((const void*)k_scatter, hipFuncAttributeMaxDynamicSharedMemorySize, (int)lds));
    }
    const int fb = Q.fb;
    const uint32_t FINE = 1u << fb;
    uint32_t* tmp = (uint32_t*)(ws + Q.o_tmp);
    uint64_t* tmp8 = (uint64_t*)(ws + Q.o_tmp);
    uint32_t* gsize = (uint32_t*)(ws + Q.o_gsize);
    uint32_t* gstart = (uint32_t*)(ws + Q.o_gstart);
    uint32_t* segbase = (uint32_t*)(ws + Q.o_segbase);
    uint32_t* segcnt = (uint32_t*)(ws + Q.o_segcnt) + (size_t)w0 * maxseg * FINE;
    uint32_t* segoff = (uint32_t*)(ws + Q.o_segoff) + (size_t)w0 * maxseg * FINE;
    const size_t zbytes = (Q.o_lenh[g] - Q.o_misc[g]) + 2 * LEN_BINS * 4;
    if (!two_pass) zero_fill(st, misc, zbytes);
    uint32_t* woff = merged ? (uint32_t*)(ws + Q.o_woff) : nullptr;
    const uint32_t* f_gstart = merged ? (uint32_t*)(ws + Q.o_gstart_m) : gstart + (size_t)w0 * G;
    const uint32_t* f_gsize = merged ? (uint32_t*)(ws + Q.o_gsize_m) : gsize + (size_t)w0 * G;
    const uint32_t* f_segbase = merged ? (uint32_t*)(ws + Q.o_segbase_m) : segbase + (size_t)w0 * (G + 1);
    const uint32_t* f_tmp = merged ? tmp : tmp + (size_t)w0 * n;
    const uint64_t* f_tmp8 = tmp8 + (size_t)w0 * n;
    const int gs_tile_env = ctx->tune.gs_tile;
    const int gs_nt_set = ctx->tune.gs_nt;
    const int gs_nt_env = gs_nt_set ? gs_nt_set : (fb == 9 ? 512 : 256);
    const int gs_nt0_env = ctx->tune.gs_nt0;
#ifdef KG_EXPERIMENTS
    const int gs_tile = gs_tile_env >= 0 ? gs_tile_env : (fb == 9 ? 8192 : 4096);
#else
    const int gs_tile = gs_tile_env > 0 ? gs_tile_env : (fb == 9 ? 8192 : 4096);
#endif
    const int gs_nt = (Q.alone && g == 0) ? gs_nt0_env : gs_nt_env;
    if (two_pass) {
      hipLaunchKernelGGL(k_group_scan, dim3(sWg), dim3(G > 256 ? 512 : GS_NT), 0, st, cnt + (size_t)sw0 * nch * G, nch, G, B, gsize + (size_t)sw0 * G, gstart + (size_t)sw0 * G,
                         segbase + (size_t)sw0 * (G + 1), (uint32_t*)(ws + Q.o_bsize) + (size_t)sw0 * B, misc, (int)(zbytes / 4), seg_len_for(fb));
      if (merged)
        hipLaunchKernelGGL(k_merge_groups, dim3(1), dim3(GS_NT), 0, st, gsize, W, G, woff, (uint32_t*)(ws + Q.o_gsize_m), (uint32_t*)(ws + Q.o_gstart_m),
                           (uint32_t*)(ws + Q.o_segbase_m));
      if (fb == 9) {
#ifdef KG_EXPERIMENTS
        if (!gs_tile) hipLaunchKernelGGL(k_group_scatter<9>, dim3(sWg, nch), dim3(GS_NT), 0, st, kt, n, c, W, Q.chunk_len, G, cnt, gstart, tmp8, woff, Q.mshift, sw0);
        else
#endif
        KG_HIP(ctx, launch_gs_big_any<9>(gs_tile, gs_nt, dim3(sWg, nch), st, kt, n, c, W, Q.chunk_len, G, cnt, gstart, tmp8, woff, Q.mshift, sw0));
        KG_HIP(ctx, hipFuncSetAttribute((const void*)k_fine_local<9>, hipFuncAttributeMaxDynamicSharedMemorySize, (int)fine_local_lds<9>()));
        hipLaunchKernelGGL(k_fine_local<9>, dim3(Wg, maxseg), dim3(512), fine_local_lds<9>(), st, f_tmp8, n, G, B, maxseg, f_gstart, f_gsize, f_segbase, S->bsize, segcnt, segoff, S->sorted);
      } else {
#ifdef KG_EXPERIMENTS
        if (!gs_tile) hipLaunchKernelGGL(k_group_scatter<7>, dim3(sWg, nch), dim3(GS_NT), 0, st, kt, n, c, W, Q.chunk_len, G, cnt, merged ? f_gstart : gstart, tmp, woff, Q.mshift, sw0);
        else
#endif
        KG_HIP(ctx, launch_gs_big_any<7>(gs_tile, gs_nt, dim3(sWg, nch), st, kt, n, c, W, Q.chunk_len, G, cnt, merged ? f_gstart : gstart, tmp, woff, Q.mshift, sw0));
        hipLaunchKernelGGL(k_fine_local<7>, dim3(Wg, maxseg), dim3(512), fine_local_lds<7>(), st, f_tmp, n, G, B, maxseg, f_gstart, f_gsize, f_segbase, S->bsize, segcnt, segoff, S->sorted);
      }
    } else {
      hipLaunchKernelGGL(k_count, dim3(W, nch), dim3(1024), lds, st, kt, n, c, W, Q.chunk_len, 0, cnt);
      hipLaunchKernelGGL(k_scan_chunks, dim3((unsigned)((npts + 255) / 256)), dim3(256), 0, st, cnt, W, nch, B, S->bsize);
    }
    const unsigned g1024 = (unsigned)((npts + 1023) / 1024);
    if (B >= 8192) {
      const int nsplit = B / 4096;
      uint32_t* bpart = (uint32_t*)(ws + Q.o_bpart) + (size_t)w0 * nsplit * 2;
      hipLaunchKernelGGL(k_bucket_part, dim3(Wg, nsplit), dim3(BR_NT), 0, st, S->bsize, B, T, nsplit, bpart, misc, lenh, T_top, top_w, S->hot_list, HOT_MAX);
      hipLaunchKernelGGL(k_bucket_fill, dim3(Wg, nsplit), dim3(BR_NT), 0, st, S->bsize, B, T, nsplit, bpart, S->bstart, S->lcnt, S->lrel, rowtot, T_top, top_w);
    } else
      hipLaunchKernelGGL(k_bucket_rows, dim3(Wg), dim3(BR_NT), 0, st, S->bsize, B, T, S->bstart, S->lcnt, S->lrel, rowtot, misc, lenh, T_top, top_w, S->hot_list, HOT_MAX);
    hipLaunchKernelGGL(k_task_bases, dim3(1), dim3(64), 0, st, rowtot, Wg, S->lbase, misc, misc + 4, lenh, lenh + LEN_BINS, (uint32_t*)ctx->h_pinned_dev + 4 * gi);
    KG_HIP(ctx, hipEventRecord(ctx->ev_info[gi], st));
    hipLaunchKernelGGL(k_len_scatter, dim3(g1024), dim3(1024), 0, st, S->bsize, S->lcnt, S->lrel, S->lbase, npts, B, T, lenh + LEN_BINS, S->task_bkt, S->task_id, T_top, top_w);
    const int fs_rows = maxseg < FS_ROWS ? maxseg : FS_ROWS;
    const int fs_extra = top_w >= 0 ? 3 : 0;
    if (two_pass && fb == 9) {
      KG_HIP(ctx, hipFuncSetAttribute((const void*)k_fine_scatter<9>, hipFuncAttributeMaxDynamicSharedMemorySize, (int)fine_scatter_lds<9>()));
      hipLaunchKernelGGL(k_fine_scatter<9>, dim3(Wg + fs_extra, fs_rows), dim3(512), fine_scatter_lds<9>(), st, f_tmp8, n, G, B, maxseg, f_gstart, f_gsize, f_segbase, S->bstart, segcnt, segoff, S->sorted, Wg, fs_extra ? top_w : -1);
    } else if (two_pass) {
      KG_HIP(ctx, hipFuncSetAttribute((const void*)k_fine_scatter<7>, hipFuncAttributeMaxDynamicSharedMemorySize, (int)fine_scatter_lds<7>()));
      hipLaunchKernelGGL(k_fine_scatter<7>, dim3(Wg + fs_extra, fs_rows), dim3(512), fine_scatter_lds<7>(), st, f_tmp, n, G, B, maxseg, f_gstart, f_gsize, f_segbase, S->bstart, segcnt, segoff, S->sorted, Wg, fs_extra ? top_w : -1);
    } else
      hipLaunchKernelGGL(k_scatter, dim3(W, nch), dim3(1024), lds, st, kt, n, c, W, Q.chunk_len, 0, cnt, S->bstart, S->sorted);
    ph.end();
    KG_HIP(ctx, hipGetLastError());
    KG_HIP(ctx, hipEventRecord(S->ready, st));
    host_trace("sort: enqueued");
  }
  (void)nv;
  return KG_OK;
}

int msm_sort(kg_ctx* ctx, int scalar_field, const uint64_t* d_scalars, size_t n, MsmSorted* S, bool ordered, int merged_c, int lane_mult, bool wait_info, int info_idx) {
  MsmSortPlan Q;
  KG_TRY(msm_sort_begin(ctx, scalar_field, d_scalars, n, &Q, ordered, merged_c, lane_mult));
  Q.info_base = info_idx;
  KG_TRY(msm_sort_group(ctx, Q, 0, S));
  return wait_info ? msm_sort_wait(ctx, S) : KG_OK;
}

int msm_sort_wait(kg_ctx* ctx, MsmSorted* S) {
  KG_HIP(ctx, hipEventSynchronize(ctx->ev_info[S->group]));
  host_trace("sort: info back");
  const uint32_t* h_info = (const uint32_t*)ctx->h_pinned + 4 * S->group;
  S->ntasks = h_info[0];
  S->max_cnt = h_info[3];
  S->nhot = h_info[2];
  if (S->ntasks > S->part_cap) return set_err(ctx, KG_ERR_HIP, "task count exceeds its bound");
  return KG_OK;
}

}
```

### kogarashi_amd/csrc/msm_sort_kernels.h

```cpp
#pragma once
#include "msm_level_kernels.h"

namespace kg {
namespace msm {
namespace {

template <class SP>
__global__ void __launch_bounds__(256) k_prep_scalars(const uint64_t* __restrict__ scalars, size_t n, Words8 H,
                                                      uint32_t* __restrict__ kt) {
  KG_SERVICE_PRIO();
  size_t i = (size_t)blockIdx.x * blockDim.x + threadIdx.x;
  if (i >= n) return;
  uint32_t w[8], k[8];
  load_words(scalars, i, w);
  ref_to_int<SP>(w, k);
  uint64_t cy = 0;
#pragma unroll
  for (int j = 0; j < 8; ++j) {
    uint64_t s = (uint64_t)k[j] + H.w[j] + cy;
    kt[(size_t)j * n + i] = (uint32_t)s;
    cy = s >> 32;
  }
}

constexpr int PREP_CH = 4096;
constexpr int PREP_NT = 256;
template <class SP>
__global__ void __launch_bounds__(PREP_NT) k_prep_scalars_count(const uint64_t* __restrict__ scalars, size_t n, Words8 H, uint32_t* __restrict__ kt,
                                                             int c, int W, int shift, int G, int nch, size_t chunk_len, uint32_t* __restrict__ cnt, int per_wg) {
  KG_SERVICE_PRIO();
  extern __shared__ uint32_t hist[];
  for (int t = threadIdx.x; t < W * G; t += blockDim.x) hist[t] = 0;
  __syncthreads();
  const size_t lo = (size_t)blockIdx.x * per_wg;
  const uint32_t cmask = (1u << c) - 1u, half = 1u << (c - 1);
  for (int r = 0; r < per_wg / PREP_NT; ++r) {
    const size_t i = lo + (size_t)r * PREP_NT + threadIdx.x;
    if (i >= n) break;
    uint32_t w[8], k[8];
    load_words(scalars, i, w);
    ref_to_int<SP>(w, k);
    uint64_t cy = 0;
#pragma unroll
    for (int j = 0; j < 8; ++j) {
      uint64_t s = (uint64_t)k[j] + H.w[j] + cy;
      k[j] = (uint32_t)s;
      kt[(size_t)j * n + i] = k[j];
      cy = s >> 32;
    }
    for (int wd = 0; wd < W; ++wd) {
      uint32_t m;
      if (wd == W - 1) m = k[0] & 0x1ffffu;
      else {
        const int32_t d = (int32_t)(k[0] & cmask) - (int32_t)half;
        m = (uint32_t)(d < 0 ? -d : d);
      }
      if (m) atomicAdd(&hist[wd * G + ((m - 1) >> shift)], 1u);
#pragma unroll
      for (int j = 0; j < 7; ++j) k[j] = (k[j] >> c) | (k[j + 1] << (32 - c));
      k[7] >>= c;
    }
  }
  __syncthreads();
  const int ch = (int)(lo / chunk_len);
  for (int t = threadIdx.x; t < W * G; t += blockDim.x) {
    const uint32_t v = hist[t];
    if (v) atomicAdd(&cnt[((size_t)(t / G) * nch + ch) * G + (t % G)], v);
  }
}


__device__ __forceinline__ uint32_t window_digit(const uint32_t* __restrict__ kt, size_t n, size_t i, int w, int c, int W, bool& negative) {
  const int o = w * c;
  const int j = o >> 5, sh = o & 31;
  uint64_t v = kt[(size_t)j * n + i];
  if (j + 1 < 8 && sh + (w == W - 1 ? 17 : c) > 32) v |= (uint64_t)kt[(size_t)(j + 1) * n + i] << 32;
  uint32_t e = (uint32_t)(v >> sh);
  if (w == W - 1) {
    negative = false;
    return e & 0x1ffffu;
  }
  e &= (1u << c) - 1u;
  const int32_t d = (int32_t)e - (int32_t)(1u << (c - 1));
  negative = d < 0;
  return (uint32_t)(d < 0 ? -d : d);
}

__global__ void __launch_bounds__(1024) k_count(const uint32_t* __restrict__ kt, size_t n, int c, int W, size_t chunk_len,
                                                int shift, uint32_t* __restrict__ cnt) {
  KG_SERVICE_PRIO();
  extern __shared__ uint32_t hist[];
  const int B = (1 << (c - 1)) >> shift;
  const int w = blockIdx.x, ch = blockIdx.y, nch = gridDim.y;
  for (int b = threadIdx.x; b < B; b += blockDim.x) hist[b] = 0;
  __syncthreads();
  const size_t lo = (size_t)ch * chunk_len, hi = lo + chunk_len < n ? lo + chunk_len : n;
  for (size_t i = lo + threadIdx.x; i < hi; i += blockDim.x) {
    bool neg;
    uint32_t m = window_digit(kt, n, i, w, c, W, neg);
    if (m) atomicAdd(&hist[(m - 1) >> shift], 1u);
  }
  __syncthreads();
  uint32_t* dst = cnt + ((size_t)w * nch + ch) * B;
  for (int b = threadIdx.x; b < B; b += blockDim.x) dst[b] = hist[b];
}

__global__ void __launch_bounds__(256) k_zero(uint4* __restrict__ p, size_t quads) {
  KG_SERVICE_PRIO();
  for (size_t i = (size_t)blockIdx.x * blockDim.x + threadIdx.x; i < quads; i += (size_t)gridDim.x * blockDim.x) p[i] = make_uint4(0, 0, 0, 0);
}
static inline void zero_fill(hipStream_t st, void* p, size_t bytes) {
  const size_t quads = (bytes + 15) / 16;
  unsigned blocks = (unsigned)((quads + 255) / 256);
  if (blocks > 1024) blocks = 1024;
  if (blocks) hipLaunchKernelGGL(k_zero, dim3(blocks), dim3(256), 0, st, reinterpret_cast<uint4*>(p), quads);
}

__global__ void __launch_bounds__(256) k_scan_chunks(uint32_t* __restrict__ cnt, int W, int nch, int B, uint32_t* __restrict__ bsize) {
  KG_SERVICE_PRIO();
  size_t t = (size_t)blockIdx.x * blockDim.x + threadIdx.x;
  if (t >= (size_t)W * B) return;
  const int w = (int)(t / B), b = (int)(t % B);
  uint32_t run = 0;
  for (int ch = 0; ch < nch; ++ch) {
    uint32_t* p = cnt + ((size_t)w * nch + ch) * B + b;
    uint32_t v = *p;
    *p = run;
    run += v;
  }
  bsize[t] = run;
}

__global__ void __launch_bounds__(1024) k_scatter(const uint32_t* __restrict__ kt, size_t n, int c, int W, size_t chunk_len,
                                                  int shift, const uint32_t* __restrict__ cnt, const uint32_t* __restrict__ bstart,
                                                  uint32_t* __restrict__ sorted) {
  KG_SERVICE_PRIO();
  extern __shared__ uint32_t off[];
  const int B = (1 << (c - 1)) >> shift;
  const uint32_t fine_mask = (1u << shift) - 1u;
  const int w = blockIdx.x, ch = blockIdx.y, nch = gridDim.y;
  const uint32_t* src = cnt + ((size_t)w * nch + ch) * B;
  for (int b = threadIdx.x; b < B; b += blockDim.x) off[b] = src[b] + bstart[(size_t)w * B + b];
  __syncthreads();
  const size_t lo = (size_t)ch * chunk_len, hi = lo + chunk_len < n ? lo + chunk_len : n;
  uint32_t* dst = sorted + (size_t)w * n;
  for (size_t i = lo + threadIdx.x; i < hi; i += blockDim.x) {
    bool neg;
    uint32_t m = window_digit(kt, n, i, w, c, W, neg);
    if (m) {
      uint32_t pos = atomicAdd(&off[(m - 1) >> shift], 1u);
      dst[pos] = (uint32_t)i | (((m - 1) & fine_mask) << 24) | (neg ? 0x80000000u : 0u);
    }
  }
}

constexpr int FINE_BITS = 7, SEG = 8192;
template <int FB> struct Ent;
template <> struct Ent<7> {
  using T = uint32_t;
  static __device__ __forceinline__ T make(uint32_t idx_tag, uint32_t fine, bool neg) { return idx_tag | (fine << 24) | (neg ? 0x80000000u : 0u); }
  static __device__ __forceinline__ uint32_t fine(T e) { return (e >> 24) & 127u; }
  static __device__ __forceinline__ uint32_t out(T e) { return e & 0x80ffffffu; }
};
template <> struct Ent<9> {
  using T = uint64_t;
  static __device__ __forceinline__ T make(uint32_t idx_tag, uint32_t fine, bool neg) { return ((uint64_t)fine << 32) | idx_tag | (neg ? 0x80000000u : 0u); }
  static __device__ __forceinline__ uint32_t fine(T e) { return (uint32_t)(e >> 32); }
  static __device__ __forceinline__ uint32_t out(T e) { return (uint32_t)e; }
};
static inline int fine_bits_for(int c) { return c >= 19 ? 9 : FINE_BITS; }
template <int FB> struct SegLen { static constexpr uint32_t V = FB == 9 ? 20480u : (uint32_t)SEG; };
static inline uint32_t seg_len_for(int fb) { return fb == 9 ? SegLen<9>::V : SegLen<7>::V; }
constexpr uint32_t MULTI_SEG = 0x80000000u;

constexpr int GS_NT = 256, GS_TILE = 1024, GS_MAXG = 1024;
__device__ __forceinline__ uint32_t window_digit_buf(BufRsrc kt, uint32_t n4, uint32_t i4, int w, int c, int W, bool& negative) {
  const int o = w * c;
  const int j = o >> 5, sh = o & 31;
  uint64_t v = (uint32_t)__builtin_amdgcn_raw_buffer_load_b32(kt, i4, (uint32_t)j * n4, 0);
  if (j + 1 < 8 && sh + (w == W - 1 ? 17 : c) > 32) v |= (uint64_t)(uint32_t)__builtin_amdgcn_raw_buffer_load_b32(kt, i4, (uint32_t)(j + 1) * n4, 0) << 32;
  uint32_t e = (uint32_t)(v >> sh);
  if (w == W - 1) {
    negative = false;
    return e & 0x1ffffu;
  }
  e &= (1u << c) - 1u;
  const int32_t d = (int32_t)e - (int32_t)(1u << (c - 1));
  negative = d < 0;
  return (uint32_t)(d < 0 ? -d : d);
}
template <int FB> struct EntLoad;
template <> struct EntLoad<7> { static __device__ __forceinline__ uint32_t ld(BufRsrc r, uint32_t idx) { return (uint32_t)__builtin_amdgcn_raw_buffer_load_b32(r, idx * 4u, 0, 0); } };
template <> struct EntLoad<9> {
  static __device__ __forceinline__ uint64_t ld(BufRsrc r, uint32_t idx) {
    typedef uint32_t u2 __attribute__((ext_vector_type(2)));
    const u2 v = __builtin_amdgcn_raw_buffer_load_b64(r, idx * 8u, 0, 0);
    return ((uint64_t)v.y << 32) | v.x;
  }
};
template <int FB> struct EntStore;
template <> struct EntStore<7> { static __device__ __forceinline__ void st(BufRsrc r, uint32_t idx, uint32_t e) { __builtin_amdgcn_raw_buffer_store_b32(e, r, idx * 4u, 0, 0); } };
template <> struct EntStore<9> {
  static __device__ __forceinline__ void st(BufRsrc r, uint32_t idx, uint64_t e) {
    typedef uint32_t u2 __attribute__((ext_vector_type(2)));
    u2 v; v.x = (uint32_t)e; v.y = (uint32_t)(e >> 32);
    __builtin_amdgcn_raw_buffer_store_b64(v, r, idx * 8u, 0, 0);
  }
};
#ifdef KG_EXPERIMENTS
#ifndef KG_GS_ATTR
#define KG_GS_ATTR
#endif
template <int FB>
__global__ void __launch_bounds__(GS_NT) KG_GS_ATTR k_group_scatter(const uint32_t* __restrict__ kt, size_t n, int c, int W, size_t chunk_len, int G,
                                                         const uint32_t* __restrict__ cnt, const uint32_t* __restrict__ gstart,
                                                         typename Ent<FB>::T* __restrict__ tmp, const uint32_t* __restrict__ woff, int mshift, int w0) {
  KG_SERVICE_PRIO();
  using E = typename Ent<FB>::T;
  constexpr uint32_t FINE = 1u << FB;
  __shared__ uint32_t cursor[GS_MAXG], hist[GS_MAXG], lstart[GS_MAXG], sh[40];
  __shared__ E stage[GS_TILE];
  __shared__ uint16_t sg[GS_TILE];
  const int w = (int)blockIdx.x + w0, ch = blockIdx.y, nch = gridDim.y, tid = threadIdx.x;
  const int per = (G + GS_NT - 1) / GS_NT;
  if (woff) {
#pragma unroll 1
    for (int g = tid; g < G; g += GS_NT) cursor[g] = cnt[((size_t)w * nch + ch) * G + g] + woff[(size_t)w * G + g] + gstart[g];
  } else {
#pragma unroll 1
    for (int g = tid; g < G; g += GS_NT) cursor[g] = cnt[((size_t)w * nch + ch) * G + g] + gstart[(size_t)w * G + g];
  }
  const uint32_t lo = (uint32_t)((size_t)ch * chunk_len), hi = (size_t)lo + chunk_len < n ? lo + (uint32_t)chunk_len : (uint32_t)n;
  const BufRsrc rkt = soa_rsrc(kt), rdst = soa_rsrc(woff ? tmp : tmp + (size_t)w * n);
  const uint32_t n4 = (uint32_t)n * 4u;
  const uint32_t wtag = woff ? (uint32_t)w << mshift : 0u;
  for (uint32_t tile = lo; tile < hi; tile += GS_TILE) {
    for (int g = tid; g < G; g += GS_NT) hist[g] = 0;
    __syncthreads();
    E rec[GS_TILE / GS_NT];
    uint32_t key[GS_TILE / GS_NT];
#pragma unroll
    for (int r = 0; r < GS_TILE / GS_NT; ++r) {
      const uint32_t i = tile + (uint32_t)r * GS_NT + (uint32_t)tid;
      key[r] = 0xffffffffu;
      if (i < hi) {
        bool neg;
        const uint32_t m = window_digit_buf(rkt, n4, i * 4u, w, c, W, neg);
        if (m) {
          const uint32_t g = (m - 1) >> FB;
          rec[r] = Ent<FB>::make(i | wtag, (m - 1) & (FINE - 1), neg);
          key[r] = (g << 16) | atomicAdd(&hist[g], 1u);
        }
      }
    }
    __syncthreads();
    uint32_t v[4], vsum = 0;
#pragma unroll
    for (int j = 0; j < 4; ++j) { const int g = tid * per + j; v[j] = (j < per && g < G) ? hist[g] : 0u; vsum += v[j]; }
    uint32_t total;
    uint32_t ex = block_exclusive_scan_1024(vsum, sh, total);
#pragma unroll
    for (int j = 0; j < 4; ++j) {
      const int g = tid * per + j;
      if (j < per && g < G) {
        lstart[g] = ex;
        hist[g] = cursor[g] - ex;
        cursor[g] += v[j];
        ex += v[j];
      }
    }
    __syncthreads();
#pragma unroll
    for (int r = 0; r < GS_TILE / GS_NT; ++r) {
      if (key[r] != 0xffffffffu) {
        const uint32_t g = key[r] >> 16, p = lstart[g] + (key[r] & 0xffffu);
        stage[p] = rec[r];
        sg[p] = (uint16_t)g;
      }
    }
    __syncthreads();
    for (uint32_t p = tid; p < total; p += GS_NT) EntStore<FB>::st(rdst, p + hist[sg[p]], stage[p]);
    __syncthreads();
  }
}
#endif

template <int FB, int TILE> constexpr size_t gs_big_lds() { return (size_t)TILE * (sizeof(typename Ent<FB>::T) + 2); }
template <int FB, int TILE, int NT>
__global__ void __launch_bounds__(NT) k_group_scatter_big(const uint32_t* __restrict__ kt, size_t n, int c, int W, size_t chunk_len, int G,
                                                             const uint32_t* __restrict__ cnt, const uint32_t* __restrict__ gstart,
                                                             typename Ent<FB>::T* __restrict__ tmp, const uint32_t* __restrict__ woff, int mshift, int w0) {
  KG_SERVICE_PRIO();
  using E = typename Ent<FB>::T;
  constexpr uint32_t FINE = 1u << FB;
  constexpr int R = TILE / NT;
  __shared__ uint32_t cursor[GS_MAXG], delta[GS_MAXG], fill[GS_MAXG], sh[40];
  extern __shared__ __align__(8) unsigned char gs_dyn[];
  E* stage = reinterpret_cast<E*>(gs_dyn);
  uint16_t* sg = reinterpret_cast<uint16_t*>(gs_dyn + sizeof(E) * TILE);
  const int w = (int)blockIdx.x + w0, ch = blockIdx.y, nch = gridDim.y, tid = threadIdx.x;
  const int per = (G + NT - 1) / NT;
  if (woff) {
#pragma unroll 1
    for (int g = tid; g < G; g += NT) cursor[g] = cnt[((size_t)w * nch + ch) * G + g] + woff[(size_t)w * G + g] + gstart[g];
  } else {
#pragma unroll 1
    for (int g = tid; g < G; g += NT) cursor[g] = cnt[((size_t)w * nch + ch) * G + g] + gstart[(size_t)w * G + g];
  }
  const uint32_t lo = (uint32_t)((size_t)ch * chunk_len), hi = (size_t)lo + chunk_len < n ? lo + (uint32_t)chunk_len : (uint32_t)n;
  const BufRsrc rkt = soa_rsrc(kt), rdst = soa_rsrc(woff ? tmp : tmp + (size_t)w * n);
  const uint32_t n4 = (uint32_t)n * 4u;
  const uint32_t wtag = woff ? (uint32_t)w << mshift : 0u;
  for (uint32_t tile = lo; tile < hi; tile += TILE) {
    for (int g = tid; g < G; g += NT) fill[g] = 0;
    __syncthreads();
#pragma unroll 8
    for (int r = 0; r < R; ++r) {
      const uint32_t i = tile + (uint32_t)r * NT + (uint32_t)tid;
      if (i < hi) {
        bool neg;
        const uint32_t m = window_digit_buf(rkt, n4, i * 4u, w, c, W, neg);
        if (m) atomicAdd(&fill[(m - 1) >> FB], 1u);
      }
    }
    __syncthreads();
    uint32_t v[4], vsum = 0;
#pragma unroll
    for (int j = 0; j < 4; ++j) { const int g = tid * per + j; v[j] = (j < per && g < G) ? fill[g] : 0u; vsum += v[j]; }
    uint32_t total;
    uint32_t ex = block_exclusive_scan_1024(vsum, sh, total);
#pragma unroll
    for (int j = 0; j < 4; ++j) {
      const int g = tid * per + j;
      if (j < per && g < G) {
        fill[g] = ex;
        delta[g] = cursor[g] - ex;
        cursor[g] += v[j];
        ex += v[j];
      }
    }
    __syncthreads();
#pragma unroll 8
    for (int r = 0; r < R; ++r) {
      const uint32_t i = tile + (uint32_t)r * NT + (uint32_t)tid;
      if (i < hi) {
        bool neg;
        const uint32_t m = window_digit_buf(rkt, n4, i * 4u, w, c, W, neg);
        if (m) {
          const uint32_t g = (m - 1) >> FB;
          const uint32_t p = atomicAdd(&fill[g], 1u);
          stage[p] = Ent<FB>::make(i | wtag, (m - 1) & (FINE - 1), neg);
          sg[p] = (uint16_t)g;
        }
      }
    }
    __syncthreads();
    for (uint32_t p = tid; p < total; p += NT) EntStore<FB>::st(rdst, p + delta[sg[p]], stage[p]);
  }
}

template <int FB, int TILE, int NT>
static hipError_t launch_gs_big(dim3 grid, hipStream_t st, const uint32_t* kt, size_t n, int c, int W, size_t chunk_len, int G, const uint32_t* cnt,
                                const uint32_t* gstart, typename Ent<FB>::T* tmp, const uint32_t* woff, int mshift, int w0) {
  constexpr size_t lds = gs_big_lds<FB, TILE>();
  auto* kern = &k_group_scatter_big<FB, TILE, NT>;
  if (lds + 4 * (3 * GS_MAXG + 40) > 48 * 1024) {
    const hipError_t e = hipFuncSetAttribute((const void*)kern, hipFuncAttributeMaxDynamicSharedMemorySize, (int)lds);
    if (e != hipSuccess) return e;
  }
  hipLaunchKernelGGL(kern, grid, dim3(NT), lds, st, kt, n, c, W, chunk_len, G, cnt, gstart, tmp, woff, mshift, w0);
  return hipSuccess;
}

template <int FB>
static hipError_t launch_gs_big_any(int tile, int nt, dim3 grid, hipStream_t st, const uint32_t* kt, size_t n, int c, int W, size_t chunk_len, int G,
                                    const uint32_t* cnt, const uint32_t* gstart, typename Ent<FB>::T* tmp, const uint32_t* woff, int mshift, int w0) {
#define KG_GS_CASE(TILE, NT) \
  if (tile == TILE && nt == NT) return launch_gs_big<FB, TILE, NT>(grid, st, kt, n, c, W, chunk_len, G, cnt, gstart, tmp, woff, mshift, w0);
  KG_GS_CASE(4096, 256) KG_GS_CASE(4096, 512) KG_GS_CASE(4096, 1024)
  KG_GS_CASE(8192, 256) KG_GS_CASE(8192, 512) KG_GS_CASE(8192, 1024)
#undef KG_GS_CASE
  return hipErrorInvalidValue;
}

__global__ void __launch_bounds__(1024) k_group_scan(uint32_t* __restrict__ cnt, int nch, int G, int B, uint32_t* __restrict__ gsize,
                                                       uint32_t* __restrict__ gstart, uint32_t* __restrict__ segbase, uint32_t* __restrict__ bsize,
                                                       uint32_t* __restrict__ zero, int zwords, uint32_t seg) {
  KG_SERVICE_PRIO();
  __shared__ uint32_t sh[40];
  const int w = blockIdx.x, tid = threadIdx.x;
  const int NT = (int)blockDim.x;
  if (w == 0) for (int t = tid; t < zwords; t += NT) zero[t] = 0;
  const int per = (G + NT - 1) / NT;
  uint32_t run[4], ns[4], rsum = 0, nsum = 0;
#pragma unroll
  for (int j = 0; j < 4; ++j) {
    const int g = tid * per + j;
    run[j] = 0;
    if (j < per && g < G) {
      uint32_t* col = cnt + (size_t)w * nch * G + g;
      int ch = 0;
      for (; ch + 8 <= nch; ch += 8) {
        uint32_t v[8];
#pragma unroll
        for (int k = 0; k < 8; ++k) v[k] = col[(size_t)(ch + k) * G];
#pragma unroll
        for (int k = 0; k < 8; ++k) { col[(size_t)(ch + k) * G] = run[j]; run[j] += v[k]; }
      }
      for (; ch < nch; ++ch) {
        uint32_t* p = col + (size_t)ch * G;
        const uint32_t v = *p;
        *p = run[j];
        run[j] += v;
      }
      gsize[(size_t)w * G + g] = run[j];
    }
    ns[j] = (run[j] + seg - 1) / seg;
    rsum += run[j]; nsum += ns[j];
  }
  uint32_t total;
  uint32_t st = block_exclusive_scan_1024(rsum, sh, total);
  uint32_t ex = block_exclusive_scan_1024(nsum, sh, total);
#pragma unroll
  for (int j = 0; j < 4; ++j) {
    const int g = tid * per + j;
    if (j < per && g < G) {
      gstart[(size_t)w * G + g] = st;
      segbase[(size_t)w * (G + 1) + g] = ex;
      st += run[j]; ex += ns[j];
    }
  }
  const int any_multi = __syncthreads_or((ns[0] > 1) | (ns[1] > 1) | (ns[2] > 1) | (ns[3] > 1));
  if (tid == 0) segbase[(size_t)w * (G + 1) + G] = total | (any_multi ? MULTI_SEG : 0u);
  uint4* z = reinterpret_cast<uint4*>(bsize + (size_t)w * B);
  for (int b = threadIdx.x; b < B / 4; b += blockDim.x) z[b] = make_uint4(0, 0, 0, 0);
}

__global__ void __launch_bounds__(GS_NT) k_merge_groups(const uint32_t* __restrict__ gsize, int W, int G, uint32_t* __restrict__ woff,
                                                        uint32_t* __restrict__ gsize_m, uint32_t* __restrict__ gstart_m,
                                                        uint32_t* __restrict__ segbase_m) {
  KG_SERVICE_PRIO();
  __shared__ uint32_t sh[40];
  const int tid = threadIdx.x;
  const int per = (G + GS_NT - 1) / GS_NT;
  uint32_t run[4], ns[4], rsum = 0, nsum = 0;
#pragma unroll
  for (int j = 0; j < 4; ++j) {
    const int g = tid * per + j;
    run[j] = 0;
    if (j < per && g < G) {
      for (int w = 0; w < W; ++w) {
        woff[(size_t)w * G + g] = run[j];
        run[j] += gsize[(size_t)w * G + g];
      }
      gsize_m[g] = run[j];
    }
    ns[j] = (run[j] + SEG - 1) / SEG;
    rsum += run[j]; nsum += ns[j];
  }
  uint32_t total;
  uint32_t st = block_exclusive_scan_1024(rsum, sh, total);
  uint32_t ex = block_exclusive_scan_1024(nsum, sh, total);
#pragma unroll
  for (int j = 0; j < 4; ++j) {
    const int g = tid * per + j;
    if (j < per && g < G) {
      gstart_m[g] = st;
      segbase_m[g] = ex;
      st += run[j]; ex += ns[j];
    }
  }
  const int any_multi = __syncthreads_or((ns[0] > 1) | (ns[1] > 1) | (ns[2] > 1) | (ns[3] > 1));
  if (tid == 0) segbase_m[G] = total | (any_multi ? MULTI_SEG : 0u);
}

struct SegRange { int g; uint32_t lo, hi; };
__device__ __forceinline__ bool seg_locate(const uint32_t* sb, int G, uint32_t s, const uint32_t* __restrict__ gstart,
                                           const uint32_t* __restrict__ gsize, int w, SegRange& r, uint32_t seg = SEG) {
  if (s >= (sb[G] & ~MULTI_SEG)) return false;
  int lo = 0, hi = G;
  while (hi - lo > 1) { const int mid = (lo + hi) >> 1; if (sb[mid] <= s) lo = mid; else hi = mid; }
  r.g = lo;
  const uint32_t st = gstart[(size_t)w * G + lo], sz = gsize[(size_t)w * G + lo];
  r.lo = st + (s - sb[lo]) * seg;
  r.hi = r.lo + seg < st + sz ? r.lo + seg : st + sz;
  return true;
}

__device__ __forceinline__ uint32_t fine_exclusive(uint32_t v, uint32_t* wsum8) {
  const int lane = threadIdx.x & 63, wv = threadIdx.x >> 6;
  uint32_t inc = v;
#pragma unroll
  for (int d = 1; d < 64; d <<= 1) { uint32_t o2 = __shfl_up(inc, d); if (lane >= d) inc += o2; }
  if (lane == 63) wsum8[wv] = inc;
  __syncthreads();
  uint32_t before = 0;
  for (int k = 0; k < wv; ++k) before += wsum8[k];
  return inc - v + before;
}
#ifndef KG_FL_UNROLL
#define KG_FL_UNROLL 4
#endif
template <int FB>
__global__ void __launch_bounds__(512) k_fine_local(const typename Ent<FB>::T* __restrict__ tmp, size_t n, int G, int B, int maxseg, const uint32_t* __restrict__ gstart,
                                                    const uint32_t* __restrict__ gsize, const uint32_t* __restrict__ segbase,
                                                    uint32_t* __restrict__ bsize, uint32_t* __restrict__ segcnt, uint32_t* __restrict__ segoff,
                                                    uint32_t* __restrict__ sorted) {
  KG_SERVICE_PRIO();
  using E = typename Ent<FB>::T;
  constexpr uint32_t FINE = 1u << FB, SEGN = SegLen<FB>::V;
  extern __shared__ uint32_t fl_lds[];
  uint32_t* const sb = fl_lds;
  uint32_t* const hist = sb + 1028;
  uint32_t* const cursor = hist + FINE;
  uint32_t* const wsum8 = cursor + FINE;
  uint32_t* const stage = wsum8 + 8;
  const int w = blockIdx.x;
  const uint32_t s = blockIdx.y;
  for (int g = threadIdx.x; g <= G; g += blockDim.x) sb[g] = segbase[(size_t)w * (G + 1) + g];
  if (threadIdx.x < FINE) hist[threadIdx.x] = 0;
  __syncthreads();
  SegRange r;
  if (!seg_locate(sb, G, s, gstart, gsize, w, r, SEGN)) return;
  const E* src = tmp + (size_t)w * n;
  if (gsize[(size_t)w * G + r.g] > SEGN) {
    uint32_t i = r.lo + threadIdx.x;
    for (; i + 3u * blockDim.x < r.hi; i += 4u * blockDim.x) {
      E e[4];
#pragma unroll
      for (int k = 0; k < 4; ++k) e[k] = src[i + (uint32_t)k * blockDim.x];
#pragma unroll
// ... 153 lines not shown
```

### kogarashi_amd/csrc/sharded.cpp

```cpp
#include "common.h"
#include <future>
#include <thread>
#include <vector>

using namespace kg;

namespace {

void shard_range(size_t n, int rank, int world, size_t* lo, size_t* hi) {
  const size_t base = n / (size_t)world, extra = n % (size_t)world;
  const size_t r = (size_t)rank;
  *lo = r * base + (r < extra ? r : extra);
  *hi = *lo + base + (r < extra ? 1 : 0);
}

int words_of(int curve) { return curve == KG_G2 ? 16 : 8; }

template <class Fn>
int for_each_ctx(kg_ctx* const* ctxs, int n_ctx, Fn fn) {
  std::vector<int> rc((size_t)n_ctx, KG_OK);
  std::vector<std::future<int>> fut;
  fut.reserve((size_t)n_ctx);
  int started = 1;
  try {
    for (int i = 1; i < n_ctx; ++i, ++started) fut.push_back(kg::pool(ctxs[0]).submit([&fn, i]() -> int { return fn(i); }));
  } catch (...) {
  }
  rc[0] = fn(0);
  for (int i = started; i < n_ctx; ++i) rc[(size_t)i] = fn(i);
  for (size_t t = 0; t < fut.size(); ++t) rc[t + 1] = fut[t].get();
  for (int i = 0; i < n_ctx; ++i)
    if (rc[(size_t)i] != KG_OK) return rc[(size_t)i];
  return KG_OK;
}

int combine(kg_ctx* ctx0, int curve, const std::vector<uint64_t>& xyz, int n_ctx, uint64_t* out_xy, uint8_t* out_inf) {
  const int E2 = words_of(curve), E = E2 / 2;
  std::vector<uint64_t> pts((size_t)n_ctx * E2);
  std::vector<uint8_t> inf((size_t)n_ctx);
  for (int i = 0; i < n_ctx; ++i) {
    const uint64_t* p = xyz.data() + (size_t)i * 3 * E;
    bool z0 = true;
    for (int k = 0; k < E; ++k) z0 = z0 && p[2 * E + k] == 0;
    inf[(size_t)i] = z0 ? 1 : 0;
    for (int k = 0; k < E2; ++k) pts[(size_t)i * E2 + k] = p[k];
  }
  return kg_points_sum_affine(ctx0, curve, pts.data(), inf.data(), (size_t)n_ctx, out_xy, out_inf);
}

}

struct kg_sharded_key {
  std::vector<kg_ctx*> ctxs;
  int curve = 0;
  size_t n = 0;
  std::vector<size_t> lo, hi;
  std::vector<uint64_t*> d_bases;
  std::vector<uint8_t*> d_inf;
};

extern "C" {

int kg_shard_range(size_t n, int rank, int world, size_t* lo, size_t* hi) {
  if (!lo || !hi || world < 1 || rank < 0 || rank >= world) return KG_ERR_BAD_ARG;
  shard_range(n, rank, world, lo, hi);
  return KG_OK;
}

int kg_commit_sharded(kg_ctx* const* ctxs, int n_ctx, int curve, const uint64_t* const* d_bases, const uint8_t* const* d_inf,
                      const uint64_t* const* d_scalars, const size_t* n_local, uint64_t* out_xy, uint8_t* out_inf) {
  return kg::kg_guarded((ctxs && n_ctx > 0 ? ctxs[0] : nullptr), [&]() -> int {
  if (!ctxs || n_ctx < 1 || n_ctx > 64 || curve < 0 || curve > KG_G2 || !d_bases || !d_scalars || !n_local || !out_xy || !out_inf) return KG_ERR_BAD_ARG;
  for (int i = 0; i < n_ctx; ++i)
    if (!ctxs[i] || (n_local[i] && (!d_bases[i] || !d_scalars[i]))) return KG_ERR_BAD_ARG;
  const int E = words_of(curve) / 2;
  std::vector<uint64_t> xyz((size_t)n_ctx * 3 * E);
  const int rc = for_each_ctx(ctxs, n_ctx, [&](int i) {
    return kg_msm(ctxs[i], curve, d_bases[i], d_inf ? d_inf[i] : nullptr, d_scalars[i], n_local[i], xyz.data() + (size_t)i * 3 * E);
  });
  if (rc != KG_OK) return rc;
  return combine(ctxs[0], curve, xyz, n_ctx, out_xy, out_inf);
  });
}

int kg_msm_sharded(kg_ctx* const* ctxs, int n_ctx, int curve, const uint64_t* const* d_bases, const uint8_t* const* d_inf,
                   const uint64_t* const* d_scalars, const size_t* n_local, uint64_t* out_xyz) {
  return kg::kg_guarded((ctxs && n_ctx > 0 ? ctxs[0] : nullptr), [&]() -> int {
  if (!out_xyz || curve < 0 || curve > KG_G2) return KG_ERR_BAD_ARG;
  uint64_t xy[16];
  uint8_t inf = 0;
  KG_TRY(kg_commit_sharded(ctxs, n_ctx, curve, d_bases, d_inf, d_scalars, n_local, xy, &inf));
  if (inf) { msm_identity(curve, out_xyz); return KG_OK; }
  const int E = words_of(curve) / 2;
  uint64_t one[24];
  msm_identity(curve, one);
  for (int k = 0; k < 2 * E; ++k) out_xyz[k] = xy[k];
  for (int k = 0; k < E; ++k) out_xyz[2 * E + k] = one[E + k];
  return KG_OK;
  });
}

int kg_sharded_key_create(kg_ctx* const* ctxs, int n_ctx, int curve, const uint64_t* h_bases, const uint8_t* h_inf, size_t n,
                          kg_sharded_key** out) {
  return kg::kg_guarded((ctxs && n_ctx > 0 ? ctxs[0] : nullptr), [&]() -> int {
  if (!out) return KG_ERR_BAD_ARG;
  *out = nullptr;
  if (!ctxs || n_ctx < 1 || n_ctx > 64 || curve < 0 || curve > KG_G2 || (n && !h_bases)) return KG_ERR_BAD_ARG;
  for (int i = 0; i < n_ctx; ++i)
    if (!ctxs[i]) return KG_ERR_BAD_ARG;
  kg_sharded_key* K = new kg_sharded_key();
  K->ctxs.assign(ctxs, ctxs + n_ctx);
  K->curve = curve; K->n = n;
  K->lo.resize((size_t)n_ctx); K->hi.resize((size_t)n_ctx);
  K->d_bases.assign((size_t)n_ctx, nullptr); K->d_inf.assign((size_t)n_ctx, nullptr);
  const size_t wb = (size_t)words_of(curve) * 8;
  const int rc = for_each_ctx(ctxs, n_ctx, [&](int i) {
    size_t lo, hi;
    shard_range(n, i, n_ctx, &lo, &hi);
    K->lo[(size_t)i] = lo; K->hi[(size_t)i] = hi;
    const size_t cnt = hi - lo;
    if (!cnt) return (int)KG_OK;
    kg_ctx* c = K->ctxs[(size_t)i];
    KG_TRY(kg_malloc(c, cnt * wb, (void**)&K->d_bases[(size_t)i]));
    KG_TRY(kg_memcpy_h2d(c, K->d_bases[(size_t)i], (const char*)h_bases + lo * wb, cnt * wb));
    if (h_inf) {
      KG_TRY(kg_malloc(c, cnt, (void**)&K->d_inf[(size_t)i]));
      KG_TRY(kg_memcpy_h2d(c, K->d_inf[(size_t)i], h_inf + lo, cnt));
    }
    return kg_bases_register(c, curve, K->d_bases[(size_t)i], K->d_inf[(size_t)i], cnt);
  });
  if (rc != KG_OK) { kg_sharded_key_destroy(K); return rc; }
  *out = K;
  return KG_OK;
  });
}

void kg_sharded_key_destroy(kg_sharded_key* K) {
  if (!K) return;
  for (size_t i = 0; i < K->ctxs.size(); ++i) {
    kg_ctx* c = K->ctxs[i];
    if (K->d_bases[i]) kg_free(c, K->d_bases[i]);
    if (K->d_inf[i]) kg_free(c, K->d_inf[i]);
  }
  delete K;
}

size_t kg_sharded_key_len(const kg_sharded_key* K) { return K ? K->n : 0; }

int kg_sharded_key_commit(kg_sharded_key* K, const uint64_t* h_scalars, size_t n, uint64_t* out_xy, uint8_t* out_inf) {
  return kg::kg_guarded((kg_ctx*)nullptr, [&]() -> int {
  if (!K || !out_xy || !out_inf || (n && !h_scalars)) return KG_ERR_BAD_ARG;
  if (n > K->n) n = K->n;
  const int n_ctx = (int)K->ctxs.size();
  const int E = words_of(K->curve) / 2;
  std::vector<uint64_t> xyz((size_t)n_ctx * 3 * E);
  const int rc = for_each_ctx(K->ctxs.data(), n_ctx, [&](int i) {
    const size_t lo = K->lo[(size_t)i] < n ? K->lo[(size_t)i] : n, hi = K->hi[(size_t)i] < n ? K->hi[(size_t)i] : n;
    const size_t cnt = hi - lo;
    kg_ctx* c = K->ctxs[(size_t)i];
    uint64_t* part = xyz.data() + (size_t)i * 3 * E;
    if (!cnt) { msm_identity(K->curve, part); return (int)KG_OK; }
    return kg_msm_host_scalars(c, K->curve, K->d_bases[(size_t)i], K->d_inf[(size_t)i], h_scalars + 4 * lo, cnt, part);
  });
  if (rc != KG_OK) return rc;
  return combine(K->ctxs[0], K->curve, xyz, n_ctx, out_xy, out_inf);
  });
}

}
```

### kogarashi_amd/csrc/tuning.h

```cpp
#pragma once
#include <string>

#define KG_TUNING_TABLE(X)                                                                                                                   \
   \
  X(wide_window, "KG_WIDE_WINDOW", 23, "log2 of the length from which a blocking MSM takes the 20-bit window (13 windows, unsliced, window groups); 0 = never (index slices with c = 17)") \
  X(msm_groups, "KG_MSM_GROUPS", -1, "window groups of a blocking MSM: -1 automatic, 0/1 none, k = k equal groups; a list \"a,b,c\" names the groups' window counts from the top window down") \
  X(msm_sliced, "KG_MSM_SLICED", 1, "0 = a blocking MSM of 2^23 pairs or more runs in window groups instead of four index slices") \
  X(msm_t, "KG_MSM_T", -1, "task length of the accumulation (entries per lane): -1 = 2 n / B + 16") \
  X(merged_t, "KG_MERGED_T", -1, "task length of a merged (window-table) accumulation: -1 = one resident round of lanes") \
  X(hot_shift, "KG_HOT_SHIFT", -1, "hot buckets are cut 2^shift times finer: -1 = 2 (0 for a merged sort)") \
  X(hot_sum, "KG_HOT_SUM", 1, "0 = hot buckets go through the generic partial-sum rounds instead of the workgroup-wide trees") \
  X(gather_fuse, "KG_GATHER_FUSE", 1, "0 = the bucket gather writes the dense bucket array instead of fusing the first halving level") \
  X(fmt64_min_log, "KG_FMT64_MIN_LOG", 0, "log2 of the array length from which resident bases take the 64-byte point form (30 = always the 72-byte limb form)") \
  X(table64, "KG_TABLE64", 1, "0 = window tables in the 72-byte limb form") \
  X(pipe_accq, "KG_PIPE_ACCQ", 1, "2 = MSM tickets alternate between two accumulation queues (measured level; off)") \
  X(coop_tail, "KG_COOP_TAIL", 1, "0 = the last reduction of a blocking MSM runs the streamed tail kernel (96 VGPRs) instead of the lane-cooperative one") \
  X(small_max, "KG_SMALL_MAX", 32768, "longest MSM (pairs) that runs as the short-input kernel (msm_small.hip): 0 = never, at most 32768 (G2: 20480)") \
  X(small_max_flight, "KG_SMALL_MAX_FLIGHT", 8192, "longest MSM begun with kg_msm_begin that runs as the short-input kernel (a call in flight shares the chip with its neighbours, and the kernel's grid fills it at these lengths); G2: half of it") \
  X(small_glv, "KG_SMALL_GLV", 1, "short-input MSMs of up to 16384 pairs split every scalar into two 127-bit halves k1 + k2 lambda against P and (beta x, y): half the windows, half the host chain (0 = off, 1 = where it pays: G1 / Grumpkin up to 6144 pairs, G2 up to 16384, 2 = wherever the index field allows)") \
  X(small_kt_from, "KG_SMALL_KT_FROM", 2048, "short-input MSMs LONGER than this convert their scalars once, by a launch of their own, instead of in every workgroup (0 = always)") \
  X(small_c, "KG_SMALL_C", 0, "window width of the short-input kernel: 0 = by length, 2..10") \
  X(small_r, "KG_SMALL_R", -1, "log2 of the buckets a workgroup of the short-input kernel owns: -1 = by length, 0..7 (2^(c-1-r) workgroups per window)") \
   \
  X(sort_nch, "KG_SORT_NCH", 64, "cap on the scalar chunks (workgroups per window) of the first sort pass, 1..1024") \
  X(sort_alone, "KG_SORT_ALONE", 1, "0 = every sort is shaped for a busy device (a blocking call's first sort normally takes the whole chip)") \
  X(gs_tile, "KG_GS_TILE", -1, "entries per tile of the first sort pass: -1 = 4096 (8192 for the wide windows), 0 = the 1024-entry kernel (needs -DKG_EXPERIMENTS)") \
  X(gs_nt, "KG_GS_NT", 0, "threads per workgroup of the first sort pass beside an accumulation: 0 = 256 (512 for the wide windows)") \
  X(gs_nt0, "KG_GS_NT0", 1024, "threads per workgroup of the first sort pass on an idle device") \
   \
  X(group_main_first, "KG_GROUP_MAIN_FIRST", 0, "1 / 2 = conversion and first group's sort on the main queue (measured slower; off)") \
  X(group_accq, "KG_GROUP_ACCQ", 2, "accumulation queues the window groups rotate over") \
  X(group_reduce_inline, "KG_GROUP_REDUCE_INLINE", 1, "the last group's bucket reduction follows its accumulation on the same queue") \
  X(blocking_reduce_inline, "KG_BLOCKING_REDUCE_INLINE", 1, "an unsplit blocking MSM (8193 .. 2^17 pairs, window tables) runs its bucket reduction behind the accumulation on the main queue instead of handing it to a reduction queue") \
  X(group_one_side, "KG_GROUP_ONE_SIDE", 0, "1 = all groups reduce on one side queue") \
   \
  X(host_slices, "KG_HOST_SLICES", 0, "index slices a host-scalar MSM is uploaded and run in: 0 = automatic (by length), 1..8") \
  X(host_first_div, "KG_HOST_FIRST_DIV", 0, "the first slice (whose upload nothing hides) is 1/div of an equal share: 0 = automatic") \
  X(blocking_tables_log, "KG_BLOCKING_TABLES_LOG", 18, "longest blocking kg_msm (log2 pairs) that goes through the window tables of registered bases; longer ones run in window groups") \
  X(host_slice_tables, "KG_HOST_SLICE_TABLES", 1, "index slices of a host-scalar MSM go through the window tables of registered bases when they have them") \
  X(host_accq, "KG_HOST_ACCQ", 2, "accumulation queues the slices of a host-scalar MSM alternate over (1 = the main queue only)") \
   \
  X(small_stamps, "KG_SMALL_STAMPS", 0, "experiment: 1 = the short-input kernel stamps its phase boundaries; the previous call's phase times go to stderr (tools/dbg/small_stamps.py)") \
  X(acc_prefetch, "KG_ACC_PREFETCH", 0, "experiment: 1 = accumulation with the next base prefetched into LDS (k_acc_tasks_q; measured level)") \
  X(acc_prefetch_log, "KG_ACC_PREFETCH_LOG", 0, "experiment: log2 of the array length from which KG_ACC_PREFETCH applies") \
  X(g2_pair_acc, "KG_G2_PAIR_ACC", 0, "experiment: 1 = G2 accumulation on lane pairs (~150 VGPRs instead of 250; measured level)") \
   \
  X(g16_h_early, "KG_G16_H_EARLY", 1, "order of h's transform chain in a proof: 1 = before the fused G1 accumulation, 0 = last (the order up to round 3), 2 = in front of the G2 accumulation") \
  X(g16_h_early_pipe, "KG_G16_H_EARLY_PIPE", 1, "0 = the early-h order only for blocking proofs") \
  X(g16_g2_glv_max, "KG_G16_G2_GLV_MAX", 1100, "a proof's b_g2 MSM keeps the halved scalars (KG_SMALL_GLV) up to this many witness entries") \
  X(g16_blind_early, "KG_G16_BLIND_EARLY", 1, "a proof's blinding chains (prover.rs:75-77, three 255-step host chains) start when the proof is enqueued; 0 = when its assembly starts") \
  X(g16_small_h_first, "KG_G16_SMALL_H_FIRST", 4096, "a short proof (one-launch MSMs) with more witness entries than this issues h's whole chain before the three G1 witness MSMs") \
  X(g16_h_inline, "KG_G16_H_INLINE", 1, "a blocking proof runs h's reduction behind h's accumulation on the main queue") \
   \
  X(ntt_direct_max_log, "KG_NTT_DIRECT_MAX_LOG", 22, "largest log2 of a direct inter-step twiddle table, 0..22 (beyond it, and when the allocation fails: composed twiddles)") \
  X(ntt_steps, "KG_NTT_STEPS", 0, "force the number of steps (HBM round trips) of a transform, 1..3; 0 = by size") \
  X(ntt_tile, "KG_NTT_TILE", 0, "force log2 of the elements a workgroup holds in LDS; 0 = by size") \
   \
  X(pool_mb, "KG_POOL_MB", 1024, "MiB of released kg_malloc blocks a context keeps for the next request of the same size (0 = none: every kg_free is a hipFree): the per-call upload buffers of the hosts (a 2^24-scalar vector is 512 MiB); kept blocks are given back when ANY context of the device runs out, and by kg_ctx_trim") \
  X(pool_max_threads, "KG_POOL_MAX_THREADS", 64, "most host worker threads a context starts (host finishes, proof assemblies, uploaders; started on demand, kept until the context is destroyed); a task that needs one more fails with a status -- 0 makes every such call fail (tests)") \
   \
  X(queue_placement, "KG_QUEUE_PLACEMENT", 1, "0 = the context's queues in creation order instead of probed over the compute pipes") \
  X(trace_host, "KG_TRACE_HOST", 0, "1 = host-side timestamps of the MSM pipeline's calls on stderr") \
  X(profile_timeline, "KG_PROFILE_TIMELINE", 0, "1 = kg_profile_summary prints every phase's start / end on stderr")

struct kg_tuning {
#define KG_X(field, env, def, doc) int field = def;
  KG_TUNING_TABLE(KG_X)
#undef KG_X
  std::string msm_groups_list;
  std::string stream_pad;
};

namespace kg {
const kg_tuning& tuning();
}
```

Baseline: 764.9 million.

## Apply GLV scalar splitting to the long MSM pipeline for G1/Grumpkin

Extends the GLV endomorphism split, previously used only for short MSMs, to the long sort-and-accumulate pipeline. Each scalar is decomposed into two roughly 127-bit halves against P and (beta·x, y). This gives 2n points over half as many windows and half as many bucket sets to reduce. Prep-bases now writes a second endomorphism-mapped copy of each base, and the sort kernels flip digit signs per half. It is enabled by default only in selected size ranges, in exchange for twice the base storage and twice the points per window.

After: 734.2 million. 0.96x the previous value.

```diff
diff --git a/kogarashi_amd/csrc/common.h b/kogarashi_amd/csrc/common.h
--- a/kogarashi_amd/csrc/common.h
+++ b/kogarashi_amd/csrc/common.h
@@ -46,6 +46,7 @@
   hipEvent_t ev_bases = nullptr;
   hipEvent_t ev_order = nullptr;
   unsigned small_glv_off = 0;
+  bool long_glv_off = false;
   bool inputs_complete = false;
 
   std::multimap<size_t, void*> pool_free;
@@ -75,7 +76,7 @@
   size_t ticket_n[4] = {0, 0, 0, 0};
   std::future<int> ticket_fut[4];
   uint64_t ticket_out[4][24] = {};
-  struct Registered { const uint64_t* base; const uint8_t* inf; size_t n; int curve; uint32_t* packed; uint32_t* table = nullptr; int table_c = 0, table_W = 0; bool fmt64 = false, table64 = false; };
+  struct Registered { const uint64_t* base; const uint8_t* inf; size_t n; int curve; uint32_t* packed; uint32_t* table = nullptr; int table_c = 0, table_W = 0; bool fmt64 = false, table64 = false, glv2 = false; };
   std::vector<Registered> registered;
   void* up_buf[3] = {nullptr, nullptr, nullptr};
   size_t up_bytes[3] = {0, 0, 0};
@@ -258,6 +259,7 @@
   bool tail_alone = false;
   hipStream_t sorted_on = nullptr;
   int merged_shift = 0, windows = 0;
+  bool glv = false;
 };
 int r1cs_prod_enqueue(kg_ctx* c, hipStream_t st, int field, const uint64_t* row_ptr, const uint64_t* col, const uint64_t* val, size_t m,
                       const uint64_t* z, uint64_t* out, uint32_t* scratch);
@@ -266,13 +268,13 @@
 struct NttTables;
 int ntt_tables(kg_ctx* ctx, uint32_t log_n, int inverse, NttTables* out, const uint32_t** zinv);
 int msm_sort(kg_ctx* ctx, int scalar_field, const uint64_t* d_scalars, size_t n, MsmSorted* S, bool ordered = false, int merged_c = 0, int lane_mult = 1,
-             bool wait_info = true, int info_idx = 0);
+             bool wait_info = true, int info_idx = 0, int glv_c = 0);
 int msm_sort_wait(kg_ctx* ctx, MsmSorted* S);
 struct MsmSortPlan {
   size_t n = 0, chunk_len = 0, nv = 0;
   int c = 0, W = 0, B = 0, Wb = 0, G = 0, nch = 0, maxseg = 0, mshift = 0, set = 0, ngroups = 1, info_base = 0, fb = 7;
   bool alone = false;
-  bool merged = false, two_pass = false;
+  bool merged = false, two_pass = false, glv = false;
   uint32_t T = 0, T_top = 0;
   int gw0[kg_ctx::MAX_GROUPS] = {}, gW[kg_ctx::MAX_GROUPS] = {};
   char* ws = nullptr;
@@ -282,9 +284,10 @@
          o_tid[kg_ctx::MAX_GROUPS] = {}, o_hot[kg_ctx::MAX_GROUPS] = {}, part_cap[kg_ctx::MAX_GROUPS] = {};
 };
 int msm_sort_begin(kg_ctx* ctx, int scalar_field, const uint64_t* d_scalars, size_t n, MsmSortPlan* P, bool ordered, int merged_c, int lane_mult,
-                   int ngroups = 1, const int* gw = nullptr, bool on_main = false);
+                   int ngroups = 1, const int* gw = nullptr, bool on_main = false, int glv_c = 0);
+int long_glv(const kg_ctx* ctx, int curve, size_t n, bool merged, bool blocking, const uint64_t* d_bases, const uint8_t* d_inf, bool registering = false);
 int msm_sort_group(kg_ctx* ctx, const MsmSortPlan& P, int g, MsmSorted* S, bool on_main = false);
-int msm_group_plan(const kg_ctx* ctx, size_t n, int* gw);
+int msm_group_plan(const kg_ctx* ctx, size_t n, int* gw, int glv_c = 0);
 int merged_window(const kg_ctx* ctx, size_t n);
 bool has_window_table(const kg_ctx* ctx, int curve, const uint64_t* d_bases, const uint8_t* d_inf, size_t nbases, size_t msm_len);
 int scalar_queue(kg_ctx* ctx, hipStream_t* out);
diff --git a/kogarashi_amd/csrc/msm_bases.h b/kogarashi_amd/csrc/msm_bases.h
--- a/kogarashi_amd/csrc/msm_bases.h
+++ b/kogarashi_amd/csrc/msm_bases.h
@@ -1,5 +1,6 @@
 #pragma once
 #include "msm_common.h"
+#include "glv_consts.h"
 
 namespace kg {
 namespace msm {
@@ -157,7 +158,22 @@
 #pragma unroll
   for (int j = 0; j < PE; ++j) dst[j] = make_uint2(buf[2 * j], buf[2 * j + 1]);
 }
-template <class F, bool P64>
+template <class F> struct EndoX { static constexpr bool OK = false; static __device__ __forceinline__ void apply(uint32_t*) {} };
+template <class P> struct EndoBeta;
+template <> struct EndoBeta<FqParams> { using T = GlvBeta<FqParams, FrParams>; };
+template <> struct EndoBeta<FrParams> { using T = GlvBeta<FrParams, FqParams>; };
+template <class P> struct EndoX<Fp<P>> {
+  static constexpr bool OK = true;
+  static __device__ __forceinline__ void apply(uint32_t* xl ) {
+    Fp<P> x;
+#pragma unroll
+    for (int j = 0; j < 9; ++j) x.l[j] = xl[j];
+    const Fp<P> bx = mul(x, Fp<P>::from_const(EndoBeta<P>::T::BETA));
+#pragma unroll
+    for (int j = 0; j < 9; ++j) xl[j] = bx.l[j];
+  }
+};
+template <class F, bool P64, bool GLV = false>
 __global__ void __launch_bounds__(256) k_prep_bases(const uint64_t* __restrict__ bases, const uint8_t* __restrict__ inf, size_t n,
                                                     uint32_t* __restrict__ out) {
   KG_SERVICE_PRIO();
@@ -167,13 +183,28 @@
   uint32_t buf[2 * PE];
   BaseIO<F>::convert(bases + (size_t)i * W, buf);
   BaseIO<F>::convert(bases + (size_t)i * W + W / 2, buf + PE);
+  if constexpr (GLV) {
+    uint32_t buf2[2 * PE];
+#pragma unroll
+    for (int j = 0; j < 2 * PE; ++j) buf2[j] = buf[j];
+    EndoX<F>::apply(buf2);
+    if (inf && inf[i]) buf2[8] |= INF_BIT;
+    store_resident<F>(out, n + i, buf2, P64 ? 1 : 0);
+  }
   if (inf && inf[i]) buf[8] |= INF_BIT;
   store_resident<F>(out, i, buf, P64 ? 1 : 0);
 }
 
 template <class F>
-static void launch_prep_bases(hipStream_t st, const uint64_t* bases, const uint8_t* inf, size_t n, uint32_t* out, bool fmt64) {
+static void launch_prep_bases(hipStream_t st, const uint64_t* bases, const uint8_t* inf, size_t n, uint32_t* out, bool fmt64, bool glv = false) {
   const dim3 grid((unsigned)((n + 255) / 256));
+  if constexpr (EndoX<F>::OK) {
+    if (glv) {
+      if (fmt64) hipLaunchKernelGGL((k_prep_bases<F, true, true>), grid, dim3(256), 0, st, bases, inf, n, out);
+      else hipLaunchKernelGGL((k_prep_bases<F, false, true>), grid, dim3(256), 0, st, bases, inf, n, out);
+      return;
+    }
+  }
   if (fmt64) hipLaunchKernelGGL((k_prep_bases<F, true>), grid, dim3(256), 0, st, bases, inf, n, out);
   else hipLaunchKernelGGL((k_prep_bases<F, false>), grid, dim3(256), 0, st, bases, inf, n, out);
 }
diff --git a/kogarashi_amd/csrc/msm_digits.h b/kogarashi_amd/csrc/msm_digits.h
--- a/kogarashi_amd/csrc/msm_digits.h
+++ b/kogarashi_amd/csrc/msm_digits.h
@@ -97,4 +97,32 @@
   }
 }
 
+template <class L>
+KG_HD void glv_biased_halves(const uint32_t k[8], const uint32_t H[8], uint32_t kb[2][4], bool neg[2]) {
+  glv_decompose_with<L>(k, kb[0], neg[0], kb[1], neg[1]);
+#pragma unroll
+  for (int e = 0; e < 2; ++e) {
+    uint64_t cy = 0;
+#pragma unroll
+    for (int j = 0; j < 4; ++j) {
+      const uint64_t s = (uint64_t)kb[e][j] + H[j] + cy;
+      kb[e][j] = (uint32_t)s;
+      cy = s >> 32;
+    }
+  }
 }
+KG_HD uint32_t glv_peel_digit(uint32_t kb[4], int c, bool top, bool half_neg, bool& negative) {
+  uint32_t m;
+  if (top) { m = kb[0] & 0x1ffffu; negative = half_neg; }
+  else {
+    const int32_t d = (int32_t)(kb[0] & ((1u << c) - 1u)) - (int32_t)(1u << (c - 1));
+    m = (uint32_t)(d < 0 ? -d : d);
+    negative = (d < 0) != half_neg;
+  }
+#pragma unroll
+  for (int j = 0; j < 3; ++j) kb[j] = (kb[j] >> c) | (kb[j + 1] << (32 - c));
+  kb[3] >>= c;
+  return m;
+}
+
+}
diff --git a/kogarashi_amd/csrc/msm_host.cpp b/kogarashi_amd/csrc/msm_host.cpp
--- a/kogarashi_amd/csrc/msm_host.cpp
+++ b/kogarashi_amd/csrc/msm_host.cpp
@@ -160,6 +160,7 @@
   const size_t pw = curve == KG_G2 ? 16 : 8;
   size_t lo[K + 1];
   for (int j = 0; j <= K; ++j) lo[j] = n / K * j + (j == K ? n % K : 0);
+  const int gc = kg::long_glv(ctx, curve, n, false, true, d_bases, d_inf);
   const int saved_window = ctx->msm_window;
   struct Restore { kg_ctx* c; int w; ~Restore() { c->msm_window = w; } } restore_window{ctx, saved_window};
   if (!saved_window) { const int cw = pick_window(n, 0), cs = pick_window(n / K, 0); ctx->msm_window = cw > cs ? cw : cs; }
@@ -171,7 +172,7 @@
   for (int j = 0; j < K && rc == KG_OK; ++j) {
     const size_t a = lo[j], cnt = lo[j + 1] - lo[j];
     kg::MsmSorted S;
-    rc = kg::msm_sort(ctx, sfield, d_scalars + 4 * a, cnt, &S, j > 0);
+    rc = kg::msm_sort(ctx, sfield, d_scalars + 4 * a, cnt, &S, j > 0, 0, 1, true, 0, gc);
     if (rc != KG_OK) break;
     rc = kg::msm_run(ctx, S, curve, d_bases + a * pw, d_inf ? d_inf + a : nullptr, cnt, 0, 16 + j);
     if (rc != KG_OK) break;
@@ -186,7 +187,7 @@
 }
 
 static int msm_grouped(kg_ctx* ctx, int curve, const uint64_t* d_bases, const uint8_t* d_inf, const uint64_t* d_scalars, size_t n, const int* gw, int NG,
-                       uint64_t* out_xyz) {
+                       int gc, uint64_t* out_xyz) {
   KG_HIP(ctx, hipSetDevice(ctx->device));
   if (!ctx->side_stream) KG_TRY(make_side_stream(ctx));
   KG_TRY(make_sort_stream(ctx));
@@ -194,7 +195,7 @@
     if (!ctx->acc_stream[g]) KG_HIP(ctx, create_stream(ctx, &ctx->acc_stream[g], false));
   kg::MsmSortPlan Q;
   const int main_first = ctx->tune.group_main_first;
-  KG_TRY(kg::msm_sort_begin(ctx, curve == KG_GRUMPKIN ? KG_FQ : KG_FR, d_scalars, n, &Q, false, 0, 1, NG, gw, main_first != 0));
+  KG_TRY(kg::msm_sort_begin(ctx, curve == KG_GRUMPKIN ? KG_FQ : KG_FR, d_scalars, n, &Q, false, 0, 1, NG, gw, main_first != 0, gc));
   if (main_first == 1) {
     KG_HIP(ctx, hipEventRecord(ctx->ev_prep, ctx->stream));
     KG_HIP(ctx, hipStreamWaitEvent(ctx->sort_stream, ctx->ev_prep, 0));
@@ -206,12 +207,13 @@
     const size_t off64 = (size_t)(d_bases - r.base);
     if (off64 % pw64 != 0 || off64 / pw64 + n > r.n) continue;
     if (d_inf != (r.inf ? r.inf + off64 / pw64 : nullptr)) continue;
+    if (gc && (off64 != 0 || n != r.n || !r.glv2)) continue;
     resident = true;
     break;
   }
   const bool f64 = resident_fmt64(n);
   if (!resident) {
-    const size_t bytes = n * (f64 ? (curve == KG_G2 ? 128 : 64) : (curve == KG_G2 ? 144 : 72));
+    const size_t bytes = (gc ? 2 : 1) * n * (f64 ? (curve == KG_G2 ? 128 : 64) : (curve == KG_G2 ? 144 : 72));
     if (bytes > ctx->ws_pb_bytes) {
       if (ctx->ws_pb) { sync_all(ctx); hipFree(ctx->ws_pb); ctx->ws_pb = nullptr; ctx->ws_pb_bytes = 0; }
       const hipError_t e = dev_alloc(ctx, &ctx->ws_pb, bytes + bytes / 8);
@@ -224,7 +226,7 @@
       KG_HIP(ctx, hipStreamWaitEvent(cq, ctx->ev_order, 0));
     }
     PhaseScope ph(ctx, "prep_bases", cq);
-    prep_bases_enqueue(curve, cq, d_bases, d_inf, n, (uint32_t*)ctx->ws_pb, f64);
+    prep_bases_enqueue(curve, cq, d_bases, d_inf, n, (uint32_t*)ctx->ws_pb, f64, gc != 0);
     ph.end();
     KG_HIP(ctx, hipGetLastError());
     KG_HIP(ctx, hipEventRecord(ctx->ev_pb, cq));
@@ -256,7 +258,7 @@
   return kg::msm_finish_groups(ctx, curve, slots, NG, out_xyz);
 }
 
-static int msm_blocking(kg_ctx* ctx, int curve, const uint64_t* d_bases, const uint8_t* d_inf, const uint64_t* d_scalars, size_t n, uint64_t* out_xyz);
+static int msm_blocking(kg_ctx* ctx, int curve, const uint64_t* d_bases, const uint8_t* d_inf, const uint64_t* d_scalars, size_t n, uint64_t* out_xyz, bool may_split = true);
 
 int kg_msm(kg_ctx* ctx, int curve, const uint64_t* d_bases, const uint8_t* d_inf, const uint64_t* d_scalars, size_t n, uint64_t* out_xyz) {
   return kg::kg_guarded(ctx, [&]() -> int {
@@ -266,7 +268,7 @@
   });
 }
 
-static int msm_blocking(kg_ctx* ctx, int curve, const uint64_t* d_bases, const uint8_t* d_inf, const uint64_t* d_scalars, size_t n, uint64_t* out_xyz) {
+static int msm_blocking(kg_ctx* ctx, int curve, const uint64_t* d_bases, const uint8_t* d_inf, const uint64_t* d_scalars, size_t n, uint64_t* out_xyz, bool may_split) {
   int sc = 0, sr = 0;
   if (kg::msm_small_plan(ctx, curve, n, &sc, &sr)) {
     KG_TRY(kg::msm_small_enqueue(ctx, ctx->stream, curve, d_bases, d_inf, d_scalars, n, 0, sc, sr));
@@ -277,13 +279,14 @@
   kg::MsmSorted S;
   const bool tables_ok = n <= ((size_t)1 << ctx->tune.blocking_tables_log);
   const int mc = tables_ok && kg::has_window_table(ctx, curve, d_bases, d_inf, n, n) ? kg::merged_window(ctx, n) : 0;
+  const int gc = may_split ? kg::long_glv(ctx, curve, n, mc != 0, true, d_bases, d_inf) : 0;
   if (!mc) {
     int gw[kg_ctx::MAX_GROUPS];
-    const int NG = kg::msm_group_plan(ctx, n, gw);
-    if (NG > 1) return msm_grouped(ctx, curve, d_bases, d_inf, d_scalars, n, gw, NG, out_xyz);
+    const int NG = kg::msm_group_plan(ctx, n, gw, gc);
+    if (NG > 1) return msm_grouped(ctx, curve, d_bases, d_inf, d_scalars, n, gw, NG, gc, out_xyz);
   }
   ctx->sort_alone = true;
-  const int rs = kg::msm_sort(ctx, curve == KG_GRUMPKIN ? KG_FQ : KG_FR, d_scalars, n, &S, false, mc);
+  const int rs = kg::msm_sort(ctx, curve == KG_GRUMPKIN ? KG_FQ : KG_FR, d_scalars, n, &S, false, mc, 1, true, 0, gc);
   ctx->sort_alone = false;
   KG_TRY(rs);
   S.tail_alone = true;
@@ -304,15 +307,16 @@
   kg_bases_unregister(ctx, d_bases);
   const bool fmt64 = resident_fmt64(n);
   const size_t pw = fmt64 ? (curve == KG_G2 ? 32 : 16) : (curve == KG_G2 ? 36 : 18);
+  const bool glv2 = kg::long_glv(ctx, curve, n, false, true, d_bases, d_inf, true) != 0;
   uint32_t* packed = nullptr;
-  KG_HIP(ctx, dev_alloc(ctx, (void**)&packed, n * pw * 4));
-  prep_bases_enqueue(curve, ctx->stream, d_bases, d_inf, n, packed, fmt64);
+  KG_HIP(ctx, dev_alloc(ctx, (void**)&packed, (glv2 ? 2 : 1) * n * pw * 4));
+  prep_bases_enqueue(curve, ctx->stream, d_bases, d_inf, n, packed, fmt64, glv2);
   if (hipError_t e = hipGetLastError(); e != hipSuccess) {
     hipFree(packed);
     return set_err(ctx, KG_ERR_HIP, "k_prep_bases launch", e);
   }
   kg_ctx::Registered reg{d_bases, d_inf, n, curve, packed};
-  reg.fmt64 = fmt64;
+  reg.fmt64 = fmt64; reg.glv2 = glv2;
   ctx->registered.push_back(reg);
   return KG_OK;
   });
@@ -385,7 +389,7 @@
   }
   kg::MsmSorted S;
   const int mc = kg::has_window_table(ctx, curve, d_bases, d_inf, n, n) ? kg::merged_window(ctx, n) : 0;
-  KG_TRY(kg::msm_sort(ctx, curve == KG_GRUMPKIN ? KG_FQ : KG_FR, d_scalars, n, &S, false, mc));
+  KG_TRY(kg::msm_sort(ctx, curve == KG_GRUMPKIN ? KG_FQ : KG_FR, d_scalars, n, &S, false, mc, 1, true, 0, kg::long_glv(ctx, curve, n, mc != 0, false, d_bases, d_inf)));
   const int pipe_accq = ctx->tune.pipe_accq;
   if (pipe_accq > 1 && (ticket & 1) && ctx->acc_stream[1]) S.acc_stream = ctx->acc_stream[1];
   if (ctx->ticket_fut[ticket].valid()) ctx->ticket_fut[ticket].wait();
@@ -509,7 +513,7 @@
     if (up_rc != (int)hipSuccess) return set_err(ctx, KG_ERR_HIP, "host-to-device upload", (hipError_t)up_rc.load());
     KG_HIP(ctx, hipStreamWaitEvent(ctx->stream, ctx->ev_up_s[0], 0));
     KG_HIP(ctx, hipStreamWaitEvent(sq, ctx->ev_up_s[0], 0));
-    return msm_blocking(ctx, curve, bases, inf, d_s, n, out_xyz);
+    return msm_blocking(ctx, curve, bases, inf, d_s, n, out_xyz, false);
   }
   if (K > 1 && !ctx->acc_stream[1]) { if (create_stream(ctx, &ctx->acc_stream[1], false) != hipSuccess) return set_err(ctx, KG_ERR_HIP, "queue creation"); }
   std::future<int> uploader = kg::pool(ctx).submit([&]() -> int {
diff --git a/kogarashi_amd/csrc/msm_internal.h b/kogarashi_amd/csrc/msm_internal.h
--- a/kogarashi_amd/csrc/msm_internal.h
+++ b/kogarashi_amd/csrc/msm_internal.h
@@ -6,7 +6,7 @@
 int pick_window(size_t n, int forced);
 bool resident_fmt64(size_t n);
 bool table_fmt64();
-void prep_bases_enqueue(int curve, hipStream_t st, const uint64_t* d_bases, const uint8_t* d_inf, size_t n, uint32_t* out, bool fmt64);
+void prep_bases_enqueue(int curve, hipStream_t st, const uint64_t* d_bases, const uint8_t* d_inf, size_t n, uint32_t* out, bool fmt64, bool glv = false);
 void table_next_enqueue(int curve, hipStream_t st, const uint32_t* prev, size_t n, int c, uint32_t* next, bool fmt64);
 void host_trace(const char* what);
 
diff --git a/kogarashi_amd/csrc/msm_run.hip b/kogarashi_amd/csrc/msm_run.hip
--- a/kogarashi_amd/csrc/msm_run.hip
+++ b/kogarashi_amd/csrc/msm_run.hip
@@ -6,9 +6,9 @@
 using namespace kg::msm;
 
 namespace kg {
-void prep_bases_enqueue(int curve, hipStream_t st, const uint64_t* d_bases, const uint8_t* d_inf, size_t n, uint32_t* out, bool fmt64) {
-  if (curve == KG_G1) launch_prep_bases<Fq>(st, d_bases, d_inf, n, out, fmt64);
-  else if (curve == KG_GRUMPKIN) launch_prep_bases<Fr>(st, d_bases, d_inf, n, out, fmt64);
+void prep_bases_enqueue(int curve, hipStream_t st, const uint64_t* d_bases, const uint8_t* d_inf, size_t n, uint32_t* out, bool fmt64, bool glv) {
+  if (curve == KG_G1) launch_prep_bases<Fq>(st, d_bases, d_inf, n, out, fmt64, glv);
+  else if (curve == KG_GRUMPKIN) launch_prep_bases<Fr>(st, d_bases, d_inf, n, out, fmt64, glv);
   else launch_prep_bases<Fq2>(st, d_bases, d_inf, n, out, fmt64);
 }
 void table_next_enqueue(int curve, hipStream_t st, const uint32_t* prev, size_t n, int c, uint32_t* next, bool fmt64) {
@@ -31,6 +31,8 @@
   constexpr int PW = 2 * BaseIO<F>::PE;
   constexpr int NW = PointIO<F>::NW;
   if (njobs < 1 || njobs > MAX_FUSED) return set_err(ctx, KG_ERR_BAD_ARG, "bad number of fused base arrays");
+  if (S.glv && (!EndoX<F>::OK || njobs != 1 || S.merged_shift || jobs[0].idx_off || S.n != 2 * jobs[0].nbases))
+    return set_err(ctx, KG_ERR_BAD_ARG, "split scalars against this base job");
   const int W = S.W, B = S.B, c = S.c;
   const size_t npts = S.npts, part_cap = S.part_cap, nexp = (size_t)W * c;
   const size_t exp_bytes = nexp * 4 * Cfg::E64 * 8;
@@ -63,6 +65,7 @@
       if (off64 % (size_t)BaseIO<F>::W != 0 || off64 / BaseIO<F>::W + J.nbases > r.n) continue;
       const size_t off = off64 / BaseIO<F>::W;
       if (J.d_inf != (r.inf ? r.inf + off : nullptr)) continue;
+      if (S.glv && (off != 0 || J.nbases != r.n || !r.glv2)) continue;
       if (S.merged_shift) {
         if (!r.table || r.table_c != c || r.table_W != S.windows) continue;
         reg_pb = r.table + off * (r.table64 ? 2 * BaseIO<F>::PK : PW);
@@ -77,7 +80,7 @@
     if (S.merged_shift && !reg_pb) return set_err(ctx, KG_ERR_BAD_ARG, "merged sort against bases without a matching window table");
     const bool conv64 = !reg_pb && resident_fmt64(J.nbases);
     if (conv64) A.fmt64[k] = 1;
-    Y.o_pb = cv.take(reg_pb ? 256 : J.nbases * (conv64 ? 2 * BaseIO<F>::PK : PW) * 4);
+    Y.o_pb = cv.take(reg_pb ? 256 : (S.glv ? 2 : 1) * J.nbases * (conv64 ? 2 * BaseIO<F>::PK : PW) * 4);
     for (int i = 0; i < 2; ++i) {
       Y.o_lc[i] = cv.take(npts * 4); Y.o_lr[i] = cv.take(npts * 4); Y.o_lb[i] = cv.take((size_t)(W + 1) * 4);
       Y.o_part[i] = cv.take(part_cap * NW * 4); Y.o_pbuf[i] = cv.take(npts * NW * 4);
@@ -105,7 +108,7 @@
         ordered_bases = true;
       }
       PhaseScope ph(ctx, "prep_bases", sq);
-      launch_prep_bases<F>(sq, J.d_bases, J.d_inf, J.nbases, (uint32_t*)(Y.ws + Y.o_pb), conv64);
+      launch_prep_bases<F>(sq, J.d_bases, J.d_inf, J.nbases, (uint32_t*)(Y.ws + Y.o_pb), conv64, S.glv);
       ph.end();
       converted = true;
     }
diff --git a/kogarashi_amd/csrc/msm_sort.hip b/kogarashi_amd/csrc/msm_sort.hip
--- a/kogarashi_amd/csrc/msm_sort.hip
+++ b/kogarashi_amd/csrc/msm_sort.hip
@@ -43,11 +43,43 @@
   return c;
 }
 
-int msm_group_plan(const kg_ctx* ctx, size_t n, int* gw) {
+static bool long_glv_pays(size_t n, bool blocking) {
+  if (!blocking) return false;
+  return (n > ((size_t)1 << 15) && n < ((size_t)1 << 15) + ((size_t)1 << 14)) || (n >= ((size_t)1 << 20) && n < ((size_t)1 << 20) + ((size_t)1 << 19));
+}
+static int long_glv_width(const kg_ctx* ctx, size_t n) {
+  int c = ctx ? ctx->msm_window : 0;
+  if (!c) c = 2 * n >= ((size_t)1 << 15) ? 16 : (2 * n >= ((size_t)1 << 10) ? 13 : 8);
+  if (c > 16 && !(2 * n >= ((size_t)1 << 16) && 2 * n <= ((size_t)1 << 24))) c = 16;
+  return c;
+}
+int long_glv(const kg_ctx* ctx, int curve, size_t n, bool merged, bool blocking, const uint64_t* d_bases, const uint8_t* d_inf, bool registering) {
+  const kg_tuning& tn = ctx ? ctx->tune : tuning();
+  if (tn.long_glv == 0 || merged || n == 0 || (ctx && ctx->long_glv_off)) return 0;
+  if (curve != KG_G1 && curve != KG_GRUMPKIN) return 0;
+  if (2 * n >= ((size_t)1 << 31)) return 0;
+  const int c = long_glv_width(ctx, n);
+  if (c < 2 || c > 20) return 0;
+  if (tn.long_glv == 1 && !long_glv_pays(n, blocking || registering)) return 0;
+  if (ctx && !registering)
+    for (const auto& r : ctx->registered) {
+      if (r.curve != curve || d_bases < r.base) continue;
+      const size_t off64 = (size_t)(d_bases - r.base);
+      if (off64 % 8 != 0 || off64 / 8 + n > r.n) continue;
+      if (d_inf != (r.inf ? r.inf + off64 / 8 : nullptr)) continue;
+      if (off64 != 0 || n != r.n || !r.glv2) return 0;
+      break;
+    }
+  return c;
+}
+
+int msm_group_plan(const kg_ctx* ctx, size_t n, int* gw, int glv_c) {
+  if (glv_c) n *= 2;
   if (n < ((size_t)1 << 16) || n > ((size_t)1 << 24)) return 0;
-  const int c = pick_window(n, ctx ? ctx->msm_window : 0);
+  const int c = glv_c ? glv_c : pick_window(n, ctx ? ctx->msm_window : 0);
   if (c - 1 < FINE_BITS + 4) return 0;
-  const int W = (255 + c - 1) / c;
+  const int W = ((glv_c ? 128 : 255) + c - 1) / c;
+  if (glv_c) n /= 2;
   int NG = n >= ((size_t)1 << 22) ? 3 : (n >= ((size_t)1 << 17) ? 2 : 0);
   if (c >= 19) NG = 4;
   if (ctx && ctx->msm_groups) NG = ctx->msm_groups;
@@ -73,15 +105,22 @@
   return NG;
 }
 
+constexpr size_t ACC_ROUND_LANES = (size_t)4096 * 64;
 int msm_sort_begin(kg_ctx* ctx, int scalar_field, const uint64_t* d_scalars, size_t n, MsmSortPlan* P, bool ordered, int merged_c, int lane_mult,
-                   int ngroups, const int* gw, bool on_main) {
+                   int ngroups, const int* gw, bool on_main, int glv_c) {
   if (n == 0 || n >= ((size_t)1 << 31)) return set_err(ctx, KG_ERR_BAD_ARG, "msm length must be in [1, 2^31)");
   host_trace("sort: enter");
   KG_HIP(ctx, hipSetDevice(ctx->device));
   const bool merged = merged_c != 0;
-  int c = merged ? merged_c : pick_window(n, ctx->msm_window);
+  const bool glv = glv_c != 0;
+  const size_t n_in = n;
+  if (glv) {
+    if (merged || glv_c < 2 || glv_c > 20 || 2 * n_in >= ((size_t)1 << 31)) return set_err(ctx, KG_ERR_BAD_ARG, "split scalars not offered for this sort");
+    n = 2 * n_in;
+  }
+  int c = merged ? merged_c : (glv ? glv_c : pick_window(n, ctx->msm_window));
   if (!merged && c > 16 && !(n >= ((size_t)1 << 16) && n <= ((size_t)1 << 24))) c = 16;
-  const int W = (255 + c - 1) / c;
+  const int W = ((glv ? 128 : 255) + c - 1) / c;
   const int B = 1 << (c - 1);
   int mshift = 0;
   if (merged) {
@@ -92,11 +131,16 @@
   const int Wb = merged ? 1 : W;
   const size_t nv = merged ? (size_t)W * n : n;
   int nch = (int)((n + 16383) / 16384);
-  const int nch_cap = ctx->tune.sort_nch >= 1 && ctx->tune.sort_nch <= 1024 ? ctx->tune.sort_nch : 64;
+  int nch_cap = ctx->tune.sort_nch >= 1 && ctx->tune.sort_nch <= 1024 ? ctx->tune.sort_nch : 64;
+  if (glv && nch_cap <= 512) nch_cap *= 2;
   if (nch > nch_cap) nch = nch_cap;
   if (nch < 1) nch = 1;
   size_t chunk_len = (n + nch - 1) / nch;
   uint32_t T = (uint32_t)(2 * (n / B) + 16);
+  if (glv && (size_t)W * B < 2 * ACC_ROUND_LANES) {
+    const size_t k = (2 * ACC_ROUND_LANES + (size_t)W * B - 1) / ((size_t)W * B);
+    if ((n / B) / k + 4 >= 32) T = (uint32_t)((n / B) / k + 4);
+  }
   if (ctx->tune.msm_t >= 4 && ctx->tune.msm_t <= 4096) T = (uint32_t)ctx->tune.msm_t;
   if (T < 32) T = 32;
   if (T > 2048) T = 2048;
@@ -132,7 +176,7 @@
     if (sum != Wb) return set_err(ctx, KG_ERR_BAD_ARG, "window groups do not add up to the window count");
   }
   Carver cv;
-  Q.o_kt = cv.take(n * 32); Q.o_cnt = cv.take((size_t)W * nch * (two_pass ? G : B) * 4); Q.o_bsize = cv.take((size_t)W * B * 4);
+  Q.o_kt = cv.take(glv ? n * 20 : n * 32); Q.o_cnt = cv.take((size_t)W * nch * (two_pass ? G : B) * 4); Q.o_bsize = cv.take((size_t)W * B * 4);
   Q.o_bstart = cv.take((size_t)Wb * B * 4);
   Q.o_tmp = cv.take(two_pass ? (size_t)W * n * (fb == 9 ? 8 : 4) : 0); Q.o_gsize = cv.take((size_t)W * G * 4); Q.o_gstart = cv.take((size_t)W * G * 4);
   Q.o_segbase = cv.take((size_t)W * (G + 1) * 4); Q.o_segcnt = cv.take((size_t)Wb * maxseg * FINE * 4); Q.o_segoff = cv.take((size_t)Wb * maxseg * FINE * 4);
@@ -162,7 +206,7 @@
   ctx->ws_idle_n[set] = 0;
   Q.n = n; Q.chunk_len = chunk_len; Q.nv = nv; Q.c = c; Q.W = W; Q.B = B; Q.Wb = Wb; Q.G = G; Q.nch = nch; Q.maxseg = maxseg; Q.mshift = mshift;
   Q.set = set; Q.ngroups = ngroups; Q.merged = merged; Q.two_pass = two_pass; Q.T = T; Q.ws = ws;
-  Q.alone = alone;
+  Q.alone = alone; Q.glv = glv;
   Q.T_top = merged ? T : 2 * T;
   Q.fb = fb;
   uint32_t* kt = (uint32_t*)(ws + Q.o_kt);
@@ -177,18 +221,26 @@
   {
     PhaseScope ph(ctx, "prep_scalars", st);
     if (two_pass) {
-      const size_t hl = (size_t)W * G * 4;
+      const size_t hl = (size_t)W * G * 4 * (glv ? 3 : 1);
       zero_fill(st, cnt, (size_t)W * nch * G * 4);
       const int per_wg = (alone && n < ((size_t)1 << 22) && fb == FINE_BITS) ? PREP_CH / 4 : PREP_CH;
-      const dim3 grid((unsigned)((n + per_wg - 1) / per_wg));
-      if (scalar_field == KG_FR) {
+      const dim3 grid((unsigned)((n_in + per_wg - 1) / per_wg));
+      if (glv && scalar_field == KG_FR) {
+        if (hl > 48 * 1024) KG_HIP(ctx, hipFuncSetAttribute((const void*)k_prep_scalars_count_glv<FrParams>, hipFuncAttributeMaxDynamicSharedMemorySize, (int)hl));
+        hipLaunchKernelGGL(k_prep_scalars_count_glv<FrParams>, grid, dim3(PREP_NT), hl, st, d_scalars, n_in, H, kt, c, W, fb, G, nch, chunk_len, cnt, per_wg);
+      } else if (glv) {
+        if (hl > 48 * 1024) KG_HIP(ctx, hipFuncSetAttribute((const void*)k_prep_scalars_count_glv<FqParams>, hipFuncAttributeMaxDynamicSharedMemorySize, (int)hl));
+        hipLaunchKernelGGL(k_prep_scalars_count_glv<FqParams>, grid, dim3(PREP_NT), hl, st, d_scalars, n_in, H, kt, c, W, fb, G, nch, chunk_len, cnt, per_wg);
+      } else if (scalar_field == KG_FR) {
         if (hl > 48 * 1024) KG_HIP(ctx, hipFuncSetAttribute((const void*)k_prep_scalars_count<FrParams>, hipFuncAttributeMaxDynamicSharedMemorySize, (int)hl));
         hipLaunchKernelGGL(k_prep_scalars_count<FrParams>, grid, dim3(PREP_NT), hl, st, d_scalars, n, H, kt, c, W, fb, G, nch, chunk_len, cnt, per_wg);
       } else {
         if (hl > 48 * 1024) KG_HIP(ctx, hipFuncSetAttribute((const void*)k_prep_scalars_count<FqParams>, hipFuncAttributeMaxDynamicSharedMemorySize, (int)hl));
         hipLaunchKernelGGL(k_prep_scalars_count<FqParams>, grid, dim3(PREP_NT), hl, st, d_scalars, n, H, kt, c, W, fb, G, nch, chunk_len, cnt, per_wg);
       }
-    } else if (scalar_field == KG_FR) hipLaunchKernelGGL(k_prep_scalars<FrParams>, dim3((unsigned)((n + 255) / 256)), dim3(256), 0, st, d_scalars, n, H, kt);
+    } else if (glv && scalar_field == KG_FR) hipLaunchKernelGGL(k_prep_scalars_glv<FrParams>, dim3((unsigned)((n_in + 255) / 256)), dim3(256), 0, st, d_scalars, n_in, H, kt);
+    else if (glv) hipLaunchKernelGGL(k_prep_scalars_glv<FqParams>, dim3((unsigned)((n_in + 255) / 256)), dim3(256), 0, st, d_scalars, n_in, H, kt);
+    else if (scalar_field == KG_FR) hipLaunchKernelGGL(k_prep_scalars<FrParams>, dim3((unsigned)((n + 255) / 256)), dim3(256), 0, st, d_scalars, n, H, kt);
     else hipLaunchKernelGGL(k_prep_scalars<FqParams>, dim3((unsigned)((n + 255) / 256)), dim3(256), 0, st, d_scalars, n, H, kt);
     ph.end();
   }
@@ -216,7 +268,7 @@
   uint32_t* misc = (uint32_t*)(ws + Q.o_misc[g]);
   uint32_t* lenh = (uint32_t*)(ws + Q.o_lenh[g]);
   S->set = Q.set; S->ready = ctx->ev_sorted[Q.set][g];
-  S->n = n; S->c = c; S->W = Wg; S->B = B; S->T = T; S->npts = npts; S->part_cap = Q.part_cap[g];
+  S->n = n; S->glv = Q.glv; S->c = c; S->W = Wg; S->B = B; S->T = T; S->npts = npts; S->part_cap = Q.part_cap[g];
   const int gi = Q.info_base + g;
   if (gi >= kg_ctx::MAX_GROUPS) return set_err(ctx, KG_ERR_BAD_ARG, "bad read-back index");
   S->merged_shift = Q.mshift; S->windows = W; S->w0 = w0; S->group = gi; S->acc_stream = nullptr; S->sorted_on = st;
@@ -236,7 +288,7 @@
       KG_HIP(ctx, hipFuncSetAttribute((const void*)k_count, hipFuncAttributeMaxDynamicSharedMemorySize, (int)lds));
       KG_HIP(ctx, hipFuncSetAttribute((const void*)k_scatter, hipFuncAttributeMaxDynamicSharedMemorySize, (int)lds));
     }
-    const int fb = Q.fb;
+    const int fb = Q.fb, glv = Q.glv ? 1 : 0;
     const uint32_t FINE = 1u << fb;
     uint32_t* tmp = (uint32_t*)(ws + Q.o_tmp);
     uint64_t* tmp8 = (uint64_t*)(ws + Q.o_tmp);
@@ -271,18 +323,18 @@
                            (uint32_t*)(ws + Q.o_segbase_m));
       if (fb == 9) {
 #ifdef KG_EXPERIMENTS
-        if (!gs_tile) hipLaunchKernelGGL(k_group_scatter<9>, dim3(sWg, nch), dim3(GS_NT), 0, st, kt, n, c, W, Q.chunk_len, G, cnt, gstart, tmp8, woff, Q.mshift, sw0);
+        if (!gs_tile) hipLaunchKernelGGL(k_group_scatter<9>, dim3(sWg, nch), dim3(GS_NT), 0, st, kt, n, c, W, Q.chunk_len, G, cnt, gstart, tmp8, woff, Q.mshift, sw0, glv);
         else
 #endif
-        KG_HIP(ctx, launch_gs_big_any<9>(gs_tile, gs_nt, dim3(sWg, nch), st, kt, n, c, W, Q.chunk_len, G, cnt, gstart, tmp8, woff, Q.mshift, sw0));
+        KG_HIP(ctx, launch_gs_big_any<9>(gs_tile, gs_nt, dim3(sWg, nch), st, kt, n, c, W, Q.chunk_len, G, cnt, gstart, tmp8, woff, Q.mshift, sw0, glv));
         KG_HIP(ctx, hipFuncSetAttribute((const void*)k_fine_local<9>, hipFuncAttributeMaxDynamicSharedMemorySize, (int)fine_local_lds<9>()));
         hipLaunchKernelGGL(k_fine_local<9>, dim3(Wg, maxseg), dim3(512), fine_local_lds<9>(), st, f_tmp8, n, G, B, maxseg, f_gstart, f_gsize, f_segbase, S->bsize, segcnt, segoff, S->sorted);
       } else {
 #ifdef KG_EXPERIMENTS
-        if (!gs_tile) hipLaunchKernelGGL(k_group_scatter<7>, dim3(sWg, nch), dim3(GS_NT), 0, st, kt, n, c, W, Q.chunk_len, G, cnt, merged ? f_gstart : gstart, tmp, woff, Q.mshift, sw0);
+        if (!gs_tile) hipLaunchKernelGGL(k_group_scatter<7>, dim3(sWg, nch), dim3(GS_NT), 0, st, kt, n, c, W, Q.chunk_len, G, cnt, merged ? f_gstart : gstart, tmp, woff, Q.mshift, sw0, glv);
         else
 #endif
-        KG_HIP(ctx, launch_gs_big_any<7>(gs_tile, gs_nt, dim3(sWg, nch), st, kt, n, c, W, Q.chunk_len, G, cnt, merged ? f_gstart : gstart, tmp, woff, Q.mshift, sw0));
+        KG_HIP(ctx, launch_gs_big_any<7>(gs_tile, gs_nt, dim3(sWg, nch), st, kt, n, c, W, Q.chunk_len, G, cnt, merged ? f_gstart : gstart, tmp, woff, Q.mshift, sw0, glv));
         hipLaunchKernelGGL(k_fine_local<7>, dim3(Wg, maxseg), dim3(512), fine_local_lds<7>(), st, f_tmp, n, G, B, maxseg, f_gstart, f_gsize, f_segbase, S->bsize, segcnt, segoff, S->sorted);
       }
     } else {
@@ -309,7 +361,7 @@
       KG_HIP(ctx, hipFuncSetAttribute((const void*)k_fine_scatter<7>, hipFuncAttributeMaxDynamicSharedMemorySize, (int)fine_scatter_lds<7>()));
       hipLaunchKernelGGL(k_fine_scatter<7>, dim3(Wg + fs_extra, fs_rows), dim3(512), fine_scatter_lds<7>(), st, f_tmp, n, G, B, maxseg, f_gstart, f_gsize, f_segbase, S->bstart, segcnt, segoff, S->sorted, Wg, fs_extra ? top_w : -1);
     } else
-      hipLaunchKernelGGL(k_scatter, dim3(W, nch), dim3(1024), lds, st, kt, n, c, W, Q.chunk_len, 0, cnt, S->bstart, S->sorted);
+      hipLaunchKernelGGL(k_scatter, dim3(W, nch), dim3(1024), lds, st, kt, n, c, W, Q.chunk_len, 0, cnt, S->bstart, S->sorted, glv);
     ph.end();
     KG_HIP(ctx, hipGetLastError());
     KG_HIP(ctx, hipEventRecord(S->ready, st));
@@ -319,9 +371,10 @@
   return KG_OK;
 }
 
-int msm_sort(kg_ctx* ctx, int scalar_field, const uint64_t* d_scalars, size_t n, MsmSorted* S, bool ordered, int merged_c, int lane_mult, bool wait_info, int info_idx) {
+int msm_sort(kg_ctx* ctx, int scalar_field, const uint64_t* d_scalars, size_t n, MsmSorted* S, bool ordered, int merged_c, int lane_mult, bool wait_info, int info_idx,
+             int glv_c) {
   MsmSortPlan Q;
-  KG_TRY(msm_sort_begin(ctx, scalar_field, d_scalars, n, &Q, ordered, merged_c, lane_mult));
+  KG_TRY(msm_sort_begin(ctx, scalar_field, d_scalars, n, &Q, ordered, merged_c, lane_mult, 1, nullptr, false, glv_c));
   Q.info_base = info_idx;
   KG_TRY(msm_sort_group(ctx, Q, 0, S));
   return wait_info ? msm_sort_wait(ctx, S) : KG_OK;
diff --git a/kogarashi_amd/csrc/msm_sort_kernels.h b/kogarashi_amd/csrc/msm_sort_kernels.h
--- a/kogarashi_amd/csrc/msm_sort_kernels.h
+++ b/kogarashi_amd/csrc/msm_sort_kernels.h
@@ -1,5 +1,6 @@
 #pragma once
 #include "msm_level_kernels.h"
+#include "msm_digits.h"
 
 namespace kg {
 namespace msm {
@@ -69,20 +70,82 @@
   }
 }
 
-
-__device__ __forceinline__ uint32_t window_digit(const uint32_t* __restrict__ kt, size_t n, size_t i, int w, int c, int W, bool& negative) {
+template <class SP>
+__global__ void __launch_bounds__(256) k_prep_scalars_glv(const uint64_t* __restrict__ scalars, size_t n, Words8 H, uint32_t* __restrict__ kt) {
+  KG_SERVICE_PRIO();
+  const size_t i = (size_t)blockIdx.x * blockDim.x + threadIdx.x, nv = 2 * n;
+  if (i >= n) return;
+  uint32_t w[8], k[8], kb[2][4];
+  bool hneg[2];
+  load_words(scalars, i, w);
+  ref_to_int<SP>(w, k);
+  glv_biased_halves<GlvLattice<SP>>(k, H.w, kb, hneg);
+#pragma unroll
+  for (int e = 0; e < 2; ++e) {
+    const size_t v = e ? n + i : i;
+#pragma unroll
+    for (int j = 0; j < 4; ++j) kt[(size_t)j * nv + v] = kb[e][j];
+    kt[(size_t)4 * nv + v] = hneg[e] ? 0x80000000u : 0u;
+  }
+}
+
+template <class SP>
+__global__ void __launch_bounds__(PREP_NT) k_prep_scalars_count_glv(const uint64_t* __restrict__ scalars, size_t n, Words8 H, uint32_t* __restrict__ kt,
+                                                                 int c, int W, int shift, int G, int nch, size_t chunk_len, uint32_t* __restrict__ cnt, int per_wg) {
+  KG_SERVICE_PRIO();
+  extern __shared__ uint32_t hist[];
+  const int WG = W * G;
+  for (int t = threadIdx.x; t < 3 * WG; t += blockDim.x) hist[t] = 0;
+  __syncthreads();
+  const size_t lo = (size_t)blockIdx.x * per_wg, nv = 2 * n;
+  const int ch1 = (int)(lo / chunk_len), ch2 = (int)((n + lo) / chunk_len);
+  const size_t ch2_end = (size_t)(ch2 + 1) * chunk_len;
+  for (int r = 0; r < per_wg / PREP_NT; ++r) {
+    const size_t i = lo + (size_t)r * PREP_NT + threadIdx.x;
+    if (i >= n) break;
+    uint32_t w[8], k[8], kb[2][4];
+    bool hneg[2];
+    load_words(scalars, i, w);
+    ref_to_int<SP>(w, k);
+    glv_biased_halves<GlvLattice<SP>>(k, H.w, kb, hneg);
+#pragma unroll
+    for (int e = 0; e < 2; ++e) {
+      const size_t v = e ? n + i : i;
+#pragma unroll
+      for (int j = 0; j < 4; ++j) kt[(size_t)j * nv + v] = kb[e][j];
+      kt[(size_t)4 * nv + v] = hneg[e] ? 0x80000000u : 0u;
+      uint32_t* h = hist + (e ? (v >= ch2_end ? 2 : 1) * WG : 0);
+      for (int wd = 0; wd < W; ++wd) {
+        bool neg;
+        const uint32_t m = glv_peel_digit(kb[e], c, wd == W - 1, hneg[e], neg);
+        if (m) atomicAdd(&h[wd * G + ((m - 1) >> shift)], 1u);
+      }
+    }
+  }
+  __syncthreads();
+  for (int t = threadIdx.x; t < 3 * WG; t += blockDim.x) {
+    const uint32_t v = hist[t];
+    const int s = t / WG, u = t % WG;
+    const int ch = s == 0 ? ch1 : ch2 + s - 1;
+    if (v) atomicAdd(&cnt[((size_t)(u / G) * nch + ch) * G + (u % G)], v);
+  }
+}
+
+
+__device__ __forceinline__ uint32_t window_digit(const uint32_t* __restrict__ kt, size_t n, size_t i, int w, int c, int W, bool& negative, int glv = 0) {
+  const bool flip = glv && (kt[(size_t)4 * n + i] >> 31) != 0;
   const int o = w * c;
   const int j = o >> 5, sh = o & 31;
   uint64_t v = kt[(size_t)j * n + i];
   if (j + 1 < 8 && sh + (w == W - 1 ? 17 : c) > 32) v |= (uint64_t)kt[(size_t)(j + 1) * n + i] << 32;
   uint32_t e = (uint32_t)(v >> sh);
   if (w == W - 1) {
-    negative = false;
+    negative = flip;
     return e & 0x1ffffu;
   }
   e &= (1u << c) - 1u;
   const int32_t d = (int32_t)e - (int32_t)(1u << (c - 1));
-  negative = d < 0;
+  negative = (d < 0) != flip;
   return (uint32_t)(d < 0 ? -d : d);
 }
 
@@ -133,7 +196,7 @@
 
 __global__ void __launch_bounds__(1024) k_scatter(const uint32_t* __restrict__ kt, size_t n, int c, int W, size_t chunk_len,
                                                   int shift, const uint32_t* __restrict__ cnt, const uint32_t* __restrict__ bstart,
-                                                  uint32_t* __restrict__ sorted) {
+                                                  uint32_t* __restrict__ sorted, int glv) {
   KG_SERVICE_PRIO();
   extern __shared__ uint32_t off[];
   const int B = (1 << (c - 1)) >> shift;
@@ -146,7 +209,7 @@
   uint32_t* dst = sorted + (size_t)w * n;
   for (size_t i = lo + threadIdx.x; i < hi; i += blockDim.x) {
     bool neg;
-    uint32_t m = window_digit(kt, n, i, w, c, W, neg);
+    uint32_t m = window_digit(kt, n, i, w, c, W, neg, glv);
     if (m) {
       uint32_t pos = atomicAdd(&off[(m - 1) >> shift], 1u);
       dst[pos] = (uint32_t)i | (((m - 1) & fine_mask) << 24) | (neg ? 0x80000000u : 0u);
@@ -174,19 +237,20 @@
 constexpr uint32_t MULTI_SEG = 0x80000000u;
 
 constexpr int GS_NT = 256, GS_TILE = 1024, GS_MAXG = 1024;
-__device__ __forceinline__ uint32_t window_digit_buf(BufRsrc kt, uint32_t n4, uint32_t i4, int w, int c, int W, bool& negative) {
+__device__ __forceinline__ uint32_t window_digit_buf(BufRsrc kt, uint32_t n4, uint32_t i4, int w, int c, int W, bool& negative, int glv = 0) {
+  const bool flip = glv && ((uint32_t)__builtin_amdgcn_raw_buffer_load_b32(kt, i4, 4u * n4, 0) >> 31) != 0;
   const int o = w * c;
   const int j = o >> 5, sh = o & 31;
   uint64_t v = (uint32_t)__builtin_amdgcn_raw_buffer_load_b32(kt, i4, (uint32_t)j * n4, 0);
   if (j + 1 < 8 && sh + (w == W - 1 ? 17 : c) > 32) v |= (uint64_t)(uint32_t)__builtin_amdgcn_raw_buffer_load_b32(kt, i4, (uint32_t)(j + 1) * n4, 0) << 32;
   uint32_t e = (uint32_t)(v >> sh);
   if (w == W - 1) {
-    negative = false;
+    negative = flip;
     return e & 0x1ffffu;
   }
   e &= (1u << c) - 1u;
   const int32_t d = (int32_t)e - (int32_t)(1u << (c - 1));
-  negative = d < 0;
+  negative = (d < 0) != flip;
   return (uint32_t)(d < 0 ? -d : d);
 }
 template <int FB> struct EntLoad;
@@ -214,7 +278,7 @@
 template <int FB>
 __global__ void __launch_bounds__(GS_NT) KG_GS_ATTR k_group_scatter(const uint32_t* __restrict__ kt, size_t n, int c, int W, size_t chunk_len, int G,
                                                          const uint32_t* __restrict__ cnt, const uint32_t* __restrict__ gstart,
-                                                         typename Ent<FB>::T* __restrict__ tmp, const uint32_t* __restrict__ woff, int mshift, int w0) {
+                                                         typename Ent<FB>::T* __restrict__ tmp, const uint32_t* __restrict__ woff, int mshift, int w0, int glv) {
   KG_SERVICE_PRIO();
   using E = typename Ent<FB>::T;
   constexpr uint32_t FINE = 1u << FB;
@@ -245,7 +309,7 @@
       key[r] = 0xffffffffu;
       if (i < hi) {
         bool neg;
-        const uint32_t m = window_digit_buf(rkt, n4, i * 4u, w, c, W, neg);
+        const uint32_t m = window_digit_buf(rkt, n4, i * 4u, w, c, W, neg, glv);
         if (m) {
           const uint32_t g = (m - 1) >> FB;
           rec[r] = Ent<FB>::make(i | wtag, (m - 1) & (FINE - 1), neg);
@@ -289,7 +353,7 @@
 template <int FB, int TILE, int NT>
 __global__ void __launch_bounds__(NT) k_group_scatter_big(const uint32_t* __restrict__ kt, size_t n, int c, int W, size_t chunk_len, int G,
                                                              const uint32_t* __restrict__ cnt, const uint32_t* __restrict__ gstart,
-                                                             typename Ent<FB>::T* __restrict__ tmp, const uint32_t* __restrict__ woff, int mshift, int w0) {
+                                                             typename Ent<FB>::T* __restrict__ tmp, const uint32_t* __restrict__ woff, int mshift, int w0, int glv) {
   KG_SERVICE_PRIO();
   using E = typename Ent<FB>::T;
   constexpr uint32_t FINE = 1u << FB;
@@ -345,7 +409,7 @@
       const uint32_t i = tile + (uint32_t)r * NT + (uint32_t)tid;
       if (i < hi) {
         bool neg;
-        const uint32_t m = window_digit_buf(rkt, n4, i * 4u, w, c, W, neg);
+        const uint32_t m = window_digit_buf(rkt, n4, i * 4u, w, c, W, neg, glv);
         if (m) {
           const uint32_t g = (m - 1) >> FB;
           const uint32_t p = atomicAdd(&fill[g], 1u);
@@ -361,22 +425,22 @@
 
 template <int FB, int TILE, int NT>
 static hipError_t launch_gs_big(dim3 grid, hipStream_t st, const uint32_t* kt, size_t n, int c, int W, size_t chunk_len, int G, const uint32_t* cnt,
-                                const uint32_t* gstart, typename Ent<FB>::T* tmp, const uint32_t* woff, int mshift, int w0) {
+                                const uint32_t* gstart, typename Ent<FB>::T* tmp, const uint32_t* woff, int mshift, int w0, int glv) {
   constexpr size_t lds = gs_big_lds<FB, TILE>();
   auto* kern = &k_group_scatter_big<FB, TILE, NT>;
   if (lds + 4 * (3 * GS_MAXG + 40) > 48 * 1024) {
     const hipError_t e = hipFuncSetAttribute((const void*)kern, hipFuncAttributeMaxDynamicSharedMemorySize, (int)lds);
     if (e != hipSuccess) return e;
   }
-  hipLaunchKernelGGL(kern, grid, dim3(NT), lds, st, kt, n, c, W, chunk_len, G, cnt, gstart, tmp, woff, mshift, w0);
+  hipLaunchKernelGGL(kern, grid, dim3(NT), lds, st, kt, n, c, W, chunk_len, G, cnt, gstart, tmp, woff, mshift, w0, glv);
   return hipSuccess;
 }
 
 template <int FB>
 static hipError_t launch_gs_big_any(int tile, int nt, dim3 grid, hipStream_t st, const uint32_t* kt, size_t n, int c, int W, size_t chunk_len, int G,
-                                    const uint32_t* cnt, const uint32_t* gstart, typename Ent<FB>::T* tmp, const uint32_t* woff, int mshift, int w0) {
+                                    const uint32_t* cnt, const uint32_t* gstart, typename Ent<FB>::T* tmp, const uint32_t* woff, int mshift, int w0, int glv) {
 #define KG_GS_CASE(TILE, NT) \
-  if (tile == TILE && nt == NT) return launch_gs_big<FB, TILE, NT>(grid, st, kt, n, c, W, chunk_len, G, cnt, gstart, tmp, woff, mshift, w0);
+  if (tile == TILE && nt == NT) return launch_gs_big<FB, TILE, NT>(grid, st, kt, n, c, W, chunk_len, G, cnt, gstart, tmp, woff, mshift, w0, glv);
   KG_GS_CASE(4096, 256) KG_GS_CASE(4096, 512) KG_GS_CASE(4096, 1024)
   KG_GS_CASE(8192, 256) KG_GS_CASE(8192, 512) KG_GS_CASE(8192, 1024)
 #undef KG_GS_CASE
diff --git a/kogarashi_amd/csrc/sharded.cpp b/kogarashi_amd/csrc/sharded.cpp
--- a/kogarashi_amd/csrc/sharded.cpp
+++ b/kogarashi_amd/csrc/sharded.cpp
@@ -76,6 +76,8 @@
   const int E = words_of(curve) / 2;
   std::vector<uint64_t> xyz((size_t)n_ctx * 3 * E);
   const int rc = for_each_ctx(ctxs, n_ctx, [&](int i) {
+    struct NoSplit { kg_ctx* c; bool old; ~NoSplit() { c->long_glv_off = old; } } no_split{ctxs[i], ctxs[i]->long_glv_off};
+    ctxs[i]->long_glv_off = true;
     return kg_msm(ctxs[i], curve, d_bases[i], d_inf ? d_inf[i] : nullptr, d_scalars[i], n_local[i], xyz.data() + (size_t)i * 3 * E);
   });
   if (rc != KG_OK) return rc;
diff --git a/kogarashi_amd/csrc/tuning.h b/kogarashi_amd/csrc/tuning.h
--- a/kogarashi_amd/csrc/tuning.h
+++ b/kogarashi_amd/csrc/tuning.h
@@ -18,6 +18,7 @@
   X(small_max, "KG_SMALL_MAX", 32768, "longest MSM (pairs) that runs as the short-input kernel (msm_small.hip): 0 = never, at most 32768 (G2: 20480)") \
   X(small_max_flight, "KG_SMALL_MAX_FLIGHT", 8192, "longest MSM begun with kg_msm_begin that runs as the short-input kernel (a call in flight shares the chip with its neighbours, and the kernel's grid fills it at these lengths); G2: half of it") \
   X(small_glv, "KG_SMALL_GLV", 1, "short-input MSMs of up to 16384 pairs split every scalar into two 127-bit halves k1 + k2 lambda against P and (beta x, y): half the windows, half the host chain (0 = off, 1 = where it pays: G1 / Grumpkin up to 6144 pairs, G2 up to 16384, 2 = wherever the index field allows)") \
+  X(long_glv, "KG_LONG_GLV", 1, "the long pipeline of kg_msm / kg_msm_begin / kg_commit splits every scalar into two 127-bit halves k1 + k2 lambda against P and (beta x, y): 2n points over half the windows, half the bucket sets to reduce, half the host chain (0 = off, 1 = where it measured faster: blocking calls of 32769 .. 49151 and of 2^20 .. 1.5 x 2^20 pairs, see long_glv in msm_sort.hip, 2 = wherever legal: G1 / Grumpkin, no window table, 2n below 2^31)") \
   X(small_kt_from, "KG_SMALL_KT_FROM", 2048, "short-input MSMs LONGER than this convert their scalars once, by a launch of their own, instead of in every workgroup (0 = always)") \
   X(small_c, "KG_SMALL_C", 0, "window width of the short-input kernel: 0 = by length, 2..10") \
   X(small_r, "KG_SMALL_R", -1, "log2 of the buckets a workgroup of the short-input kernel owns: -1 = by length, 0..7 (2^(c-1-r) workgroups per window)") \
```
